# OATML-Markslab/ProteinGym

Measured on AMD Instinct MI355X. Metric: mutants scored/sec (ESM-1v 650M masked-marginal), higher is better.
Workload: dtype f16x3 (fp32 operands split into 2 fp16 planes, 3 fp16 MFMAs per product, fp32 accumulate)

## Files before the change

include/pgmi.h:

```cpp
#ifndef PGMI_H
#define PGMI_H

#include <stddef.h>
#include <stdint.h>

#ifdef __cplusplus
extern "C" {
#endif

#define PGMI_ABI_VERSION 4

#define PGMI_OK 0
#define PGMI_EINVAL (-1)
#define PGMI_ENOMEM (-2)
#define PGMI_EHIP (-3)
#define PGMI_ENODEV (-4)
#define PGMI_EPARSE (-5)
#define PGMI_EOVERFLOW (-6)

#define PGMI_ARCH_ESM1B 1
#define PGMI_ARCH_ESM2 2
#define PGMI_ARCH_TRANCEPTION 3
#define PGMI_ARCH_MSA 4
#define PGMI_ARCH_PROGEN2 5
#define PGMI_ARCH_GPT 6
#define PGMI_GPT_POS_ROTARY 0
#define PGMI_GPT_POS_LEARNED 1
#define PGMI_ARCH_ESMC 7

#define PGMI_PREC_FP32 0
#define PGMI_PREC_BF16 1
#define PGMI_PREC_F16X3 2

#define PGMI_TOK_CLS 0
#define PGMI_TOK_PAD 1
#define PGMI_TOK_EOS 2
#define PGMI_TOK_UNK 3
#define PGMI_TOK_MASK 32
#define PGMI_VOCAB 33
#define PGMI_PG2_VOCAB 32
#define PGMI_ESMC_VOCAB 64

typedef struct pgmi_config {
    int32_t abi_version;
    int32_t arch;
    int32_t layers;
    int32_t embed_dim;
    int32_t heads;
    int32_t ffn_dim;
    int32_t vocab;
    int32_t max_positions;
    int32_t token_dropout;
    int32_t emb_layer_norm_before;
    int32_t precision;
    int32_t max_rows;
    float ln_eps;
} pgmi_config;

typedef struct pgmi_model pgmi_model;
typedef struct pgmi_assay pgmi_assay;
typedef struct pgmi_pppl pgmi_pppl;

int pgmi_abi_version(void);
int pgmi_device_count(void);
const char* pgmi_last_error(void);

int64_t pgmi_weight_count(const pgmi_config* cfg);

int pgmi_model_create(const pgmi_config* cfg, const float* weights, int64_t n_weights,
                      int device, pgmi_model** out);
void pgmi_model_destroy(pgmi_model* m);
int pgmi_model_device(const pgmi_model* m);

int pgmi_token_logprobs(pgmi_model* m, const int32_t* tokens, int B, int T, float* out);

int pgmi_masked_logprobs(pgmi_model* m, const int32_t* tokens, const int32_t* mask_pos,
                         int B, int T, float* out);

int pgmi_assay_create(pgmi_model* m, const int32_t* wt_tokens, int n_tok,
                      const int32_t* positions, int P, int window,
                      const int32_t* sub_pos, const int32_t* sub_wt, const int32_t* sub_mt,
                      const int64_t* mut_off, int64_t n_mut, pgmi_assay** out);
int pgmi_assay_run(pgmi_model* m, pgmi_assay* a, double* scores_host, float* table_host,
                   double* scores_dev);
void pgmi_assay_destroy(pgmi_assay* a);

int pgmi_pppl_create(pgmi_model* m, const uint8_t* tokens, const int64_t* seq_off, int64_t n_seq, pgmi_pppl** out);
int pgmi_pppl_run(pgmi_model* m, pgmi_pppl* lib, int64_t first, int64_t count, double* scores_host,
                  float* terms_host, double* scores_dev);
int64_t pgmi_pppl_rows(const pgmi_pppl* lib, int64_t first, int64_t count);
int pgmi_pppl_stats(const pgmi_pppl* lib, int64_t* rows, int64_t* batches, int64_t* tokens, int64_t* padded_tokens);
void pgmi_pppl_destroy(pgmi_pppl* lib);

int pgmi_parse_mutants(const char* text, const int64_t* str_off, int64_t n_mut,
                       const char* sequence, int seq_len, int offset_idx,
                       int32_t* sub_pos, int32_t* sub_wt, int32_t* sub_mt,
                       int64_t* mut_off, int64_t* n_sub);

int pgmi_score_mutants(const float* table, int n_rows, int vocab, const int32_t* sub_pos, const int32_t* sub_wt,
                       const int32_t* sub_mt, const int64_t* mut_off, int64_t n_mut, double* scores);

void pgmi_optimal_window(int position, int seq_len_with_special, int model_window,
                         int* start, int* end);

#define PGMI_K_EMBED 0
#define PGMI_K_LAYERNORM 1
#define PGMI_K_GEMM_QKV 2
#define PGMI_K_ATTENTION 3
#define PGMI_K_GEMM_OUT 4
#define PGMI_K_GEMM_FC1 5
#define PGMI_K_GEMM_FC2 6
#define PGMI_K_HEAD 7
#define PGMI_K_SCORE 8
#define PGMI_K_KEPT_ROWS 9
#define PGMI_K_COUNT 10
int pgmi_profile_enable(pgmi_model* m, int on);
int pgmi_profile_get(pgmi_model* m, int kernel_class, double* ms, int64_t* launches,
                     double* flops, double* bytes);
int pgmi_profile_reset(pgmi_model* m);
int pgmi_synchronize(pgmi_model* m);

int pgmi_set_option(const char* name, int64_t value);

int pgmi_op_layernorm(int device, const float* x, const float* w, const float* b,
                      int rows, int D, float eps, float* y);
int pgmi_op_gemm(int device, int precision, const float* A, const float* W, const float* bias,
                 const float* residual, int M, int N, int K, int epilogue ,
                 float* C);
int pgmi_op_qkln_prep(int device, const float* qkv, const float* q_w, const float* k_w, int B, int T, int H, int iters, float* qk,
                      float* v, double* ms);
int pgmi_op_attention(int device, int precision, const float* qkv, const int32_t* kv_len,
                      int B, int T, int H, int rotary, float* ctx);
int pgmi_op_causal_attention(int device, int lanes, const float* X, const float* W, const float* bias, int K, const float* qkv,
                             const float* conv, const float* rot_cos, const float* rot_sin, const float* slopes, int B, int T,
                             int heads, float* ctx);

int pgmi_tr_token_logprobs(pgmi_model* m, const int32_t* tokens, int B, int T, float* out);
int pgmi_tr_sequence_loglik(pgmi_model* m, const int32_t* tokens, const int32_t* lens, int B, int T,
                            const float* log_prior, int P, const int32_t* prior_a0, const int32_t* prior_row0,
                            const int32_t* prior_n, const int32_t* prior_flip, float alpha, float* out);
int pgmi_tr_sequence_loglik_shared(pgmi_model* m, const int32_t* tokens, const int32_t* ref, int B, int T,
                                   const float* log_prior, int P, const int32_t* prior_a0, const int32_t* prior_row0,
                                   const int32_t* prior_n, const int32_t* prior_flip, float alpha, float* out,
                                   float* token_logprobs, int64_t* rows_forwarded);

int pgmi_bench_gemm(int device, int precision, int M, int N, int K, int epilogue, int split_out,
                    int variant, int iters, double* ms_per_launch);
int pgmi_bench_gemm_ab(int device, int precision, int M, int N, int K, int epilogue, int split_out,
                       const int* variants, int n_variants, int rounds, int iters, double* ms_out);

int pgmi_pg2_model_create(const pgmi_config* cfg, int rotary_dim, const float* weights, int64_t n_weights, int device, pgmi_model** out);
int pgmi_pg2_token_logprobs(pgmi_model* m, const int32_t* tokens, int B, int T, float* out);
int pgmi_pg2_sequence_loglik(pgmi_model* m, const int32_t* tokens, int B, int L, float* out, int32_t* n_kept);

int64_t pgmi_gpt_weight_count(const pgmi_config* cfg, int pos_kind);
int pgmi_gpt_model_create(const pgmi_config* cfg, int pos_kind, const float* weights, int64_t n_weights, int device, pgmi_model** out);
int pgmi_gpt_token_logprobs(pgmi_model* m, const int32_t* tokens, int B, int T, float* out);
int pgmi_gpt_sequence_loglik(pgmi_model* m, const int32_t* tokens, const int32_t* lens, int B, int T, double* sum, int32_t* n_targets);


int pgmi_msa_token_logprobs(pgmi_model* m, const int32_t* tokens, int R, int T, float* out);
int pgmi_msa_masked_logprobs(pgmi_model* m, const int32_t* tokens, int R, int T, int window,
                             const int32_t* positions, const int32_t* starts, int n, float* out);

int pgmi_msa_cluster_counts(int device, const int8_t* matrix, int64_t N, int64_t L, int invalid_value,
                            double identity_threshold, int32_t* counts_out, double* kernel_ms);

#ifdef __cplusplus
}
#endif
#endif
```

proteingym_amd/_lib.py:

```python
from __future__ import annotations

import ctypes as C
import os

import numpy as np

HERE = os.path.dirname(os.path.abspath(__file__))
LIB_PATH = os.path.join(HERE, "libpgmi.so")

ABI_VERSION = 4
ARCH_ESM1B, ARCH_ESM2, ARCH_TRANCEPTION = 1, 2, 3
ARCH_PROGEN2 = 5
ARCH_GPT = 6
ARCH_ESMC = 7
GPT_POS_ROTARY, GPT_POS_LEARNED = 0, 1
PREC_FP32, PREC_BF16, PREC_F16X3 = 0, 1, 2
PRECISIONS = {"fp32": PREC_FP32, "bf16": PREC_BF16, "f16x3": PREC_F16X3}
K_NAMES = ["embed", "layernorm", "gemm_qkv", "attention", "gemm_out", "gemm_fc1", "gemm_fc2",
           "head", "score", "kept_rows"]


EINVAL, ENOMEM, EHIP, ENODEV, EPARSE, EOVERFLOW = -1, -2, -3, -4, -5, -6


class PgmiError(RuntimeError):

    def __init__(self, message, code=None):
        super().__init__(message)
        self.code = code


class Config(C.Structure):
    _fields_ = [(n, C.c_int32) for n in (
        "abi_version", "arch", "layers", "embed_dim", "heads", "ffn_dim", "vocab",
        "max_positions", "token_dropout", "emb_layer_norm_before", "precision", "max_rows")] + [("ln_eps", C.c_float)]


_lib = None

_i32p = C.POINTER(C.c_int32)
_i64p = C.POINTER(C.c_int64)
_f32p = C.POINTER(C.c_float)
_f64p = C.POINTER(C.c_double)

SIGNATURES = [
    ("pgmi_abi_version", C.c_int, []),
    ("pgmi_device_count", C.c_int, []),
    ("pgmi_last_error", C.c_char_p, []),
    ("pgmi_weight_count", C.c_int64, [C.POINTER(Config)]),
    ("pgmi_model_create", C.c_int, [C.POINTER(Config), _f32p, C.c_int64, C.c_int, C.POINTER(C.c_void_p)]),
    ("pgmi_model_destroy", None, [C.c_void_p]),
    ("pgmi_model_device", C.c_int, [C.c_void_p]),
    ("pgmi_token_logprobs", C.c_int, [C.c_void_p, _i32p, C.c_int, C.c_int, _f32p]),
    ("pgmi_masked_logprobs", C.c_int, [C.c_void_p, _i32p, _i32p, C.c_int, C.c_int, _f32p]),
    ("pgmi_assay_create", C.c_int, [C.c_void_p, _i32p, C.c_int, _i32p, C.c_int, C.c_int,
                                    _i32p, _i32p, _i32p, _i64p, C.c_int64, C.POINTER(C.c_void_p)]),
    ("pgmi_assay_run", C.c_int, [C.c_void_p, C.c_void_p, _f64p, _f32p, C.c_void_p]),
    ("pgmi_assay_destroy", None, [C.c_void_p]),
    ("pgmi_pppl_create", C.c_int, [C.c_void_p, C.POINTER(C.c_uint8), _i64p, C.c_int64, C.POINTER(C.c_void_p)]),
    ("pgmi_pppl_run", C.c_int, [C.c_void_p, C.c_void_p, C.c_int64, C.c_int64, _f64p, _f32p, C.c_void_p]),
    ("pgmi_pppl_rows", C.c_int64, [C.c_void_p, C.c_int64, C.c_int64]),
    ("pgmi_pppl_stats", C.c_int, [C.c_void_p, _i64p, _i64p, _i64p, _i64p]),
    ("pgmi_pppl_destroy", None, [C.c_void_p]),
    ("pgmi_parse_mutants", C.c_int, [C.c_char_p, _i64p, C.c_int64, C.c_char_p, C.c_int, C.c_int,
                                     _i32p, _i32p, _i32p, _i64p, _i64p]),
    ("pgmi_score_mutants", C.c_int, [_f32p, C.c_int, C.c_int, _i32p, _i32p, _i32p, _i64p, C.c_int64, _f64p]),
    ("pgmi_optimal_window", None, [C.c_int, C.c_int, C.c_int, _i32p, _i32p]),
    ("pgmi_profile_enable", C.c_int, [C.c_void_p, C.c_int]),
    ("pgmi_profile_get", C.c_int, [C.c_void_p, C.c_int, _f64p, _i64p, _f64p, _f64p]),
    ("pgmi_profile_reset", C.c_int, [C.c_void_p]),
    ("pgmi_synchronize", C.c_int, [C.c_void_p]),
    ("pgmi_set_option", C.c_int, [C.c_char_p, C.c_int64]),
    ("pgmi_op_layernorm", C.c_int, [C.c_int, _f32p, _f32p, _f32p, C.c_int, C.c_int, C.c_float, _f32p]),
    ("pgmi_op_gemm", C.c_int, [C.c_int, C.c_int, _f32p, _f32p, _f32p, _f32p, C.c_int, C.c_int, C.c_int, C.c_int, _f32p]),
    ("pgmi_tr_token_logprobs", C.c_int, [C.c_void_p, _i32p, C.c_int, C.c_int, _f32p]),
    ("pgmi_tr_sequence_loglik", C.c_int, [C.c_void_p, _i32p, _i32p, C.c_int, C.c_int, _f32p, C.c_int,
                                          _i32p, _i32p, _i32p, _i32p, C.c_float, _f32p]),
    ("pgmi_tr_sequence_loglik_shared", C.c_int, [C.c_void_p, _i32p, _i32p, C.c_int, C.c_int, _f32p, C.c_int,
                                                 _i32p, _i32p, _i32p, _i32p, C.c_float, _f32p, _f32p, _i64p]),
    ("pgmi_pg2_model_create", C.c_int, [C.POINTER(Config), C.c_int, _f32p, C.c_int64, C.c_int, C.POINTER(C.c_void_p)]),
    ("pgmi_pg2_token_logprobs", C.c_int, [C.c_void_p, _i32p, C.c_int, C.c_int, _f32p]),
    ("pgmi_pg2_sequence_loglik", C.c_int, [C.c_void_p, _i32p, C.c_int, C.c_int, _f32p, _i32p]),
    ("pgmi_gpt_weight_count", C.c_int64, [C.POINTER(Config), C.c_int]),
    ("pgmi_gpt_model_create", C.c_int, [C.POINTER(Config), C.c_int, _f32p, C.c_int64, C.c_int, C.POINTER(C.c_void_p)]),
    ("pgmi_gpt_token_logprobs", C.c_int, [C.c_void_p, _i32p, C.c_int, C.c_int, _f32p]),
    ("pgmi_gpt_sequence_loglik", C.c_int, [C.c_void_p, _i32p, _i32p, C.c_int, C.c_int, _f64p, _i32p]),
    ("pgmi_bench_gemm", C.c_int, [C.c_int] * 9 + [_f64p]),
    ("pgmi_bench_gemm_ab", C.c_int, [C.c_int] * 7 + [_i32p, C.c_int, C.c_int, C.c_int, _f64p]),
    ("pgmi_op_attention", C.c_int, [C.c_int, C.c_int, _f32p, _i32p, C.c_int, C.c_int, C.c_int, C.c_int, _f32p]),
    ("pgmi_op_qkln_prep", C.c_int, [C.c_int, _f32p, _f32p, _f32p, C.c_int, C.c_int, C.c_int, C.c_int, _f32p, _f32p, _f64p]),
    ("pgmi_op_causal_attention", C.c_int, [C.c_int, C.c_int, _f32p, _f32p, _f32p, C.c_int, _f32p, _f32p, _f32p, _f32p, _f32p,
                                           C.c_int, C.c_int, C.c_int, _f32p]),
    ("pgmi_msa_token_logprobs", C.c_int, [C.c_void_p, _i32p, C.c_int, C.c_int, _f32p]),
    ("pgmi_msa_masked_logprobs", C.c_int, [C.c_void_p, _i32p, C.c_int, C.c_int, C.c_int, _i32p, _i32p, C.c_int, _f32p]),
    ("pgmi_msa_cluster_counts", C.c_int, [C.c_int, C.POINTER(C.c_int8), C.c_int64, C.c_int64, C.c_int, C.c_double, _i32p, _f64p]),
]


def load():
    global _lib
    if _lib is not None:
        return _lib
    if not os.path.exists(LIB_PATH):
        raise PgmiError(f"{LIB_PATH} not found: run `python -m proteingym_amd.build_native` "
                        "(hipcc, gfx950).  There is no CPU fallback.")
    lib = C.CDLL(LIB_PATH)
    for name, res, args in SIGNATURES:
        fn = getattr(lib, name)
        fn.restype = res
        fn.argtypes = args
    if lib.pgmi_abi_version() != ABI_VERSION:
        raise PgmiError("libpgmi ABI version mismatch; rebuild")
    _lib = lib
    return lib


def check(rc: int):
    if rc != 0:
        raise PgmiError(f"libpgmi error {rc}: {load().pgmi_last_error().decode(errors='replace')}", code=int(rc))


def ptr(a: np.ndarray, ty):
    return a.ctypes.data_as(ty) if a is not None else None


def as_i32(a):
    return np.ascontiguousarray(a, dtype=np.int32)


def as_f32(a):
    return np.ascontiguousarray(a, dtype=np.float32)


class ModelHandle:
    CREATE = "pgmi_model_create"

    def __init__(self, cfg: dict, weights: np.ndarray, device: int = 0, max_rows: int = 0, arch_arg=None,
                 precision: int = PREC_F16X3, **fields):
        lib = load()
        self.cfg = dict(cfg)
        self.device = device
        c = Config(abi_version=ABI_VERSION, layers=cfg["layers"], embed_dim=cfg["embed_dim"], heads=cfg["heads"],
                   ffn_dim=cfg["ffn_dim"], precision=precision, max_rows=max_rows, **fields)
        w = as_f32(weights)
        n = self._weight_count(lib, c, arch_arg)
        if w.size != n:
            raise PgmiError(f"weight blob has {w.size} elements, config needs {n}")
        h = C.c_void_p()
        head = (C.byref(c),) if arch_arg is None else (C.byref(c), arch_arg)
        check(getattr(lib, self.CREATE)(*head, ptr(w, _f32p), w.size, device, C.byref(h)))
        self._h = h

    @staticmethod
    def _weight_count(lib, c, arch_arg):
        return lib.pgmi_weight_count(C.byref(c))

    def close(self):
        if getattr(self, "_h", None):
            load().pgmi_model_destroy(self._h)
            self._h = None

    def __del__(self):
        try:
            self.close()
        except Exception:
            pass
```

proteingym_amd/csrc/api_esm.hip:

```cpp
#include "model.h"

namespace pgmi {

int create_esm(pgmi_model* m, const pgmi_config* cfg, const float* w, int64_t n_weights) {
    const size_t D = cfg->embed_dim, F = cfg->ffn_dim, V = cfg->vocab, dh = m->dh, Da = m->Da;
    BlobCursor c(m, w, n_weights);
    c.upload(&m->embed_tokens, V * D);
    if (cfg->arch == PGMI_ARCH_ESM1B) c.upload(&m->embed_positions, (size_t)(cfg->max_positions + 2) * D);
    if (cfg->emb_layer_norm_before) {
        c.upload(&m->lnb_w, D);
        c.upload(&m->lnb_b, D);
    }
    auto slot = [&](size_t col) -> size_t { return rotate_half_slot(col, dh); };
    const float qscale = 1.0f / sqrtf((float)dh);
    m->layers.resize(cfg->layers);
    std::vector<float> wq(3 * Da * D, 0.0f), bq(3 * Da, 0.0f), wo_r(D * Da, 0.0f);
    for (int l = 0; l < cfg->layers; ++l) {
        Layer& L = m->layers[l];
        c.upload(&L.ln1_w, D);
        c.upload(&L.ln1_b, D);
        pack_qkv_slots(c.take(3 * (D * D + D)), D, Da, slot, qscale, wq.data(), bq.data());
        c.linear(&L.wqkv, &L.wqkv16, wq.data(), wq.size(), D);
        c.upload(&L.bqkv, bq.data(), bq.size());
        pack_out_cols(c.take(D * D), D, Da, slot, wo_r.data());
        c.linear(&L.wo, &L.wo16, wo_r.data(), wo_r.size(), Da);
        c.upload(&L.bo, D);
        c.upload(&L.ln2_w, D);
        c.upload(&L.ln2_b, D);
        c.linear(&L.w1, &L.w116, F * D, D);
        c.upload(&L.b1, F);
        c.linear(&L.w2, &L.w216, D * F, F);
        c.upload(&L.b2, D);
    }
    c.upload(&m->lna_w, D);
    c.upload(&m->lna_b, D);
    c.linear(&m->hd_w, &m->hd16, D * D, D);
    c.upload(&m->hd_b, D);
    c.upload(&m->hln_w, D);
    c.upload(&m->hln_b, D);
    c.upload(&m->head_b, V);
    m->head_w = m->embed_tokens;
    return c.finish();
}

int ensure_rotary(pgmi_model* m, int T) {
    if ((m->cfg.arch != PGMI_ARCH_ESM2 && m->cfg.arch != PGMI_ARCH_ESMC) || T <= m->rot_len) return PGMI_OK;
    return upload_rotate_half(m, std::max(T, 1026));
}

int upload_rotate_half(pgmi_model* m, int n) {
    const int rh = m->rot_halves;
    float inv[64];
    const int half = m->dh / 2;
    for (int i = 0; i < half; ++i) inv[i] = 1.0f / powf(10000.0f, (float)(2 * i) / (float)m->dh);
    return upload_rotary(m, n, rh, [&](int t, int g, int i) {
        const int j = (rh == 1) ? i : 32 * g + i;
        return j < half ? (float)t * inv[j] : 0.0f;
    });
}

int run_encoder(pgmi_model* m, int B, int T, const int32_t* keep, int n_keep, bool* compacted) {
    const pgmi_config& c = m->cfg;
    const int M = B * T, D = c.embed_dim, F = c.ffn_dim, N1 = m->fc1_cols, H = c.heads, Da = m->Da;
    hipStream_t s = m->stream;
    if (c.arch == PGMI_ARCH_ESM1B && T > c.max_positions) {
        set_error("Sequence length %d above maximum sequence length of %d", T, c.max_positions);
        return PGMI_EINVAL;
    }
    int rc = ensure_rotary(m, T);
    if (!rc) rc = reset_pad_keys(m, B, T);
    if (rc) return rc;
    {
        ProfScope p(m, PGMI_K_EMBED, 0, (double)M * D * 4);
        launch_seq_stats(m->tokens, B, T, m->embed_gather ? 0 : c.token_dropout, m->denom, m->pos_idx, m->kv_len, s);
        if (m->embed_gather) launch_gather_rows(m->embed_tokens, m->tokens, M, D, m->x, s);
        else launch_embed(m->tokens, m->denom, m->pos_idx, m->embed_tokens, m->embed_positions, c.token_dropout, M, T, D, m->x, s);
        if (m->lnb_w) {
            launch_layernorm(m->x, m->lnb_w, m->lnb_b, M, D, 1e-5f, m->x, s);
            launch_zero_pad_rows(m->tokens, M, D, m->x, s);
        }
    }
    const double ln_bytes = 2.0 * M * D * 4;
    const int prec = c.precision;
    const int mode16 = (prec == PGMI_PREC_F16X3) ? 1 : 2;
    for (int l = 0; l < c.layers; ++l) {
        const Layer& L = m->layers[l];
        { ProfScope p(m, PGMI_K_LAYERNORM, 0, ln_bytes);
          if (prec == PGMI_PREC_FP32) launch_layernorm(m->x, L.ln1_w, L.ln1_b, M, D, 1e-5f, m->h, s);
          else launch_layernorm16(m->x, L.ln1_w, L.ln1_b, M, D, 1e-5f, m->h16, m->h16_plane, mode16, s); }
        const bool fused_qkv = prec != PGMI_PREC_FP32 && !L.q_ln;
        { ProfScope p(m, PGMI_K_GEMM_QKV, 2.0 * M * 3 * D * D, 0);
          if (fused_qkv)
              rc = launch_gemm16_qkv(m->h16, m->h16_plane, L.wqkv16.p, L.wqkv16.plane, L.bqkv, M, Da, D, L.wqkv16.out_scale,
                                     m->qk16, m->qk16_plane, m->vt16, m->vt16_plane, m->rot_cos, m->rot_sin,
                                     c.arch == PGMI_ARCH_ESM2, T, m->Hs, m->gemm_variant, s, m->rot_halves, prec == PGMI_PREC_BF16);
          else
              rc = linear(m, m->h, m->h16, m->h16_plane, L.wqkv, L.wqkv16, L.bqkv, nullptr, m->qkv, nullptr, 0, M, 3 * Da, D, EPI_NONE);
          if (rc) return rc; }
        { ProfScope p(m, PGMI_K_ATTENTION, 4.0 * M * T * D, L.q_ln ? (double)M * D * 20 : 0);
          if (L.q_ln && (rc = launch_qkln_prep(m->qkv, L.q_ln, L.k_ln, 1e-5f, m->rot_cos, m->rot_sin, B, T, H, m->qk16, m->qk16_plane,
                                               m->vt16, m->vt16_plane, s)))
              return rc;
          const bool v2 = prec != PGMI_PREC_FP32;
          if (c.arch == PGMI_ARCH_ESM2 && !v2) launch_rotary(m->qkv, m->rot_cos, m->rot_sin, M, T, m->Hs, s, m->rot_halves);
          if (v2) {
              AttLaunch a;
              a.qk16 = m->qk16, a.qk_plane = m->qk16_plane, a.vt16 = m->vt16, a.vt_plane = m->vt16_plane;
              a.B = B, a.T = T, a.H = H, a.head_dim = m->rot_halves * kHeadDim;
              a.kv_len = m->kv_len;
              a.out = prec == PGMI_PREC_F16X3 ? ATT_OUT_SPLIT : ATT_OUT_BF16;
              a.ctx16 = m->h16;
              a.stream = s;
              rc = launch_attention_f16x3_v2(a);
          } else {
              rc = launch_attention_f32(m->qkv, m->kv_len, B, T, H, m->h, s, m->rot_halves * kHeadDim);
          }
          if (rc) return rc; }
        if (keep && m->keep_rows && l == c.layers - 1) {
            const int R = n_keep;
            ProfScope p(m, PGMI_K_KEPT_ROWS, 2.0 * R * D * (Da + N1 + F), 0);
            launch_gather_rows(m->x, keep, R, D, m->qkv, s);
            if (prec == PGMI_PREC_FP32) launch_gather_rows(m->h, keep, R, Da, m->g, s);
            else
                launch_gather_rows(reinterpret_cast<const float*>(m->h16), keep, R, prec == PGMI_PREC_F16X3 ? Da : Da / 2,
                                   reinterpret_cast<float*>(m->g16), s);
            rc = linear(m, m->g, m->g16, m->g16_plane, L.wo, L.wo16, L.bo, m->qkv, m->x, nullptr, 0, R, D, Da, EPI_NONE);
            if (rc) return rc;
            if (prec == PGMI_PREC_FP32) launch_layernorm(m->x, L.ln2_w, L.ln2_b, R, D, 1e-5f, m->h, s);
            else launch_layernorm16(m->x, L.ln2_w, L.ln2_b, R, D, 1e-5f, m->h16, m->h16_plane, mode16, s);
            rc = linear(m, m->h, m->h16, m->h16_plane, L.w1, L.w116, L.b1, nullptr,
                        prec == PGMI_PREC_FP32 ? m->g : nullptr, prec == PGMI_PREC_FP32 ? nullptr : m->g16, m->g16_plane,
                        R, N1, D, m->fc1_epi);
            if (rc) return rc;
            rc = linear(m, m->g, m->g16, m->g16_plane, L.w2, L.w216, L.b2, m->x, m->x, nullptr, 0, R, D, F, EPI_NONE);
            if (rc) return rc;
            if (compacted) *compacted = true;
            break;
        }
        { ProfScope p(m, PGMI_K_GEMM_OUT, 2.0 * M * D * D, 0);
          rc = linear(m, m->h, m->h16, m->h16_plane, L.wo, L.wo16, L.bo, m->x, m->x, nullptr, 0, M, D, Da, EPI_NONE);
          if (rc) return rc; }
        { ProfScope p(m, PGMI_K_LAYERNORM, 0, ln_bytes);
          if (prec == PGMI_PREC_FP32) launch_layernorm(m->x, L.ln2_w, L.ln2_b, M, D, 1e-5f, m->h, s);
          else launch_layernorm16(m->x, L.ln2_w, L.ln2_b, M, D, 1e-5f, m->h16, m->h16_plane, mode16, s); }
        { ProfScope p(m, PGMI_K_GEMM_FC1, 2.0 * M * N1 * D, 0);
          rc = linear(m, m->h, m->h16, m->h16_plane, L.w1, L.w116, L.b1, nullptr,
                      prec == PGMI_PREC_FP32 ? m->g : nullptr, prec == PGMI_PREC_FP32 ? nullptr : m->g16, m->g16_plane,
                      M, N1, D, m->fc1_epi);
          if (rc) return rc; }
        { ProfScope p(m, PGMI_K_GEMM_FC2, 2.0 * M * F * D, 0);
          rc = linear(m, m->g, m->g16, m->g16_plane, L.w2, L.w216, L.b2, m->x, m->x, nullptr, 0, M, D, F, EPI_NONE);
          if (rc) return rc; }
    }
    PGMI_HIP(hipGetLastError());
    return PGMI_OK;
}

int run_head(pgmi_model* m, int R, const int32_t* row_idx) {
    const pgmi_config& c = m->cfg;
    const int D = c.embed_dim;
    hipStream_t s = m->stream;
    ProfScope p(m, PGMI_K_HEAD, 2.0 * R * D * (D + c.vocab), 0);
    const int prec = c.precision;
    const float* src = m->x;
    if (row_idx) {
        launch_gather_rows(m->x, row_idx, R, D, m->h, s);
        src = m->h;
    }
    if (prec == PGMI_PREC_FP32) launch_layernorm(src, m->lna_w, m->lna_b, R, D, 1e-5f, m->h, s);
    else launch_layernorm16(src, m->lna_w, m->lna_b, R, D, 1e-5f, m->h16, m->h16_plane, prec == PGMI_PREC_F16X3 ? 1 : 2, s);
    int rc = linear(m, m->h, m->h16, m->h16_plane, m->hd_w, m->hd16, m->hd_b, nullptr, m->g, nullptr, 0, R, D, D, EPI_GELU);
    if (rc) return rc;
    launch_layernorm(m->g, m->hln_w, m->hln_b, R, D, 1e-5f, m->g, s);
    launch_vocab_logsoftmax(m->g, m->head_w, m->head_b, R, D, c.vocab, m->lp, m->nonfinite, s);
    PGMI_HIP(hipGetLastError());
    return PGMI_OK;
}


int run_rows(pgmi_model* m, int B, int T, int R, const int32_t* row_idx) {
    bool compacted = false;
    int rc = run_encoder(m, B, T, row_idx, R, &compacted);
    if (rc) return rc;
    return run_head(m, R, compacted ? nullptr : row_idx);
}

}

extern "C" {

int pgmi_token_logprobs(pgmi_model* m, const int32_t* tokens, int B, int T, float* out) {
    if (!m || !tokens || !out || B <= 0 || T <= 0) { set_error("bad argument"); return PGMI_EINVAL; }
    if (T + 31 > m->max_rows) { set_error("T=%d exceeds workspace rows %d", T, m->max_rows); return PGMI_EINVAL; }
    int rc = check_tokens(tokens, B, T);
    if (rc) return rc;
    PGMI_HIP(hipSetDevice(m->device));
    const int V = m->cfg.vocab;
    rc = for_each_chunk(m, B, T, [&](int b0, int bc) {
        PGMI_HIP(hipMemcpyAsync(m->tokens, tokens + (size_t)b0 * T, (size_t)bc * T * 4, hipMemcpyHostToDevice, m->stream));
        int rc = run_rows(m, bc, T, bc * T, nullptr);
        if (rc) return rc;
        PGMI_HIP(hipMemcpyAsync(out + (size_t)b0 * T * V, m->lp, (size_t)bc * T * V * 4, hipMemcpyDeviceToHost, m->stream));
        return PGMI_OK;
    });
    return rc ? rc : check_nonfinite(m);
}

int pgmi_masked_logprobs(pgmi_model* m, const int32_t* tokens, const int32_t* mask_pos, int B, int T, float* out) {
    if (!m || !tokens || !mask_pos || !out || B <= 0 || T <= 0) { set_error("bad argument"); return PGMI_EINVAL; }
    if (m->cfg.arch == PGMI_ARCH_ESMC && T + 31 > m->max_rows) { set_error("T=%d exceeds workspace rows %d", T, m->max_rows); return PGMI_EINVAL; }
    if (T > m->max_rows) { set_error("T=%d exceeds workspace rows %d", T, m->max_rows); return PGMI_EINVAL; }
    int rc = check_tokens(tokens, B, T);
    if (rc) return rc;
    for (int b = 0; b < B; ++b)
        if (mask_pos[b] < 0 || mask_pos[b] >= T) { set_error("mask_pos[%d]=%d out of range", b, mask_pos[b]); return PGMI_EINVAL; }
    PGMI_HIP(hipSetDevice(m->device));
    const int V = m->cfg.vocab;
    std::vector<int32_t> ridx;
    rc = for_each_chunk(m, B, T, [&](int b0, int bc) {
        ridx.resize(bc);
        for (int b = 0; b < bc; ++b) ridx[b] = b * T + mask_pos[b0 + b];
        PGMI_HIP(hipMemcpyAsync(m->tokens, tokens + (size_t)b0 * T, (size_t)bc * T * 4, hipMemcpyHostToDevice, m->stream));
        PGMI_HIP(hipMemcpyAsync(m->aux_i, mask_pos + b0, (size_t)bc * 4, hipMemcpyHostToDevice, m->stream));
        PGMI_HIP(hipMemcpyAsync(m->row_idx, ridx.data(), (size_t)bc * 4, hipMemcpyHostToDevice, m->stream));
        launch_apply_mask(m->tokens, m->aux_i, bc, T, m->stream);
        int rc = run_rows(m, bc, T, bc, m->row_idx);
        if (rc) return rc;
        PGMI_HIP(hipMemcpyAsync(out + (size_t)b0 * V, m->lp, (size_t)bc * V * 4, hipMemcpyDeviceToHost, m->stream));
        return PGMI_OK;
    });
    return rc ? rc : check_nonfinite(m);
}

int pgmi_assay_create(pgmi_model* m, const int32_t* wt_tokens, int n_tok, const int32_t* positions, int P,
                      int window, const int32_t* sub_pos, const int32_t* sub_wt, const int32_t* sub_mt,
                      const int64_t* mut_off, int64_t n_mut, pgmi_assay** out) {
    if (!out) { set_error("null out"); return PGMI_EINVAL; }
    *out = nullptr;
    if (!m || !wt_tokens || n_tok <= 0 || P < 0 || (P > 0 && !positions) || window <= 0 || n_mut < 0) { set_error("bad argument"); return PGMI_EINVAL; }
    if (m->cfg.arch == PGMI_ARCH_ESMC) { set_error("ESM C assays run through pgmi_masked_logprobs (their window rule is not pgmi_optimal_window)"); return PGMI_EINVAL; }
    for (int i = 0; i < n_tok; ++i)
        if (wt_tokens[i] < 0 || wt_tokens[i] >= PGMI_VOCAB || wt_tokens[i] == PGMI_TOK_PAD) { set_error("wt token %d invalid at %d", wt_tokens[i], i); return PGMI_EINVAL; }
    const int T = std::min(n_tok, window);
    if (T > m->max_rows) { set_error("T=%d exceeds workspace rows %d", T, m->max_rows); return PGMI_EINVAL; }
    std::vector<int32_t> ws(P), mr(P);
    for (int i = 0; i < P; ++i) {
        if (positions[i] < 0 || positions[i] >= n_tok) { set_error("position %d out of range", positions[i]); return PGMI_EINVAL; }
        int s, e;
        pgmi_optimal_window(positions[i], n_tok, window, &s, &e);
        if (e - s != T) { set_error("internal: window length %d != %d", e - s, T); return PGMI_EINVAL; }
        ws[i] = s;
        mr[i] = positions[i] - s;
    }
    const int64_t n_sub = n_mut ? mut_off[n_mut] : 0;
    for (int64_t k = 0; k < n_sub; ++k)
        if (sub_pos[k] < 0 || sub_pos[k] >= n_tok || sub_wt[k] < 0 || sub_wt[k] >= PGMI_VOCAB || sub_mt[k] < 0 || sub_mt[k] >= PGMI_VOCAB) {
            set_error("substitution %lld out of range", (long long)k);
            return PGMI_EINVAL;
        }
    PGMI_HIP(hipSetDevice(m->device));
    pgmi_assay* a = new pgmi_assay();
    a->m = m; a->n_tok = n_tok; a->P = P; a->T = T; a->n_mut = n_mut; a->n_sub = n_sub;
    int rc = dev_upload(a->allocs, &a->wt, wt_tokens, (size_t)n_tok);
    if (!rc) rc = dev_upload(a->allocs, &a->positions, positions, (size_t)P);
    if (!rc) rc = dev_upload(a->allocs, &a->win_start, ws.data(), (size_t)P);
    if (!rc) rc = dev_upload(a->allocs, &a->mask_rel, mr.data(), (size_t)P);
    if (!rc) rc = dev_upload(a->allocs, &a->sub_pos, sub_pos, (size_t)n_sub);
    if (!rc) rc = dev_upload(a->allocs, &a->sub_wt, sub_wt, (size_t)n_sub);
    if (!rc) rc = dev_upload(a->allocs, &a->sub_mt, sub_mt, (size_t)n_sub);
    if (!rc) rc = dev_upload(a->allocs, &a->mut_off, mut_off, (size_t)(n_mut + 1));
    if (!rc) rc = dev_alloc(a->allocs, &a->table, (size_t)n_tok * PGMI_VOCAB);
    if (!rc) rc = dev_alloc(a->allocs, &a->scores, (size_t)n_mut);
    if (rc) { pgmi_assay_destroy(a); return rc; }
    m->assays.push_back(a);
    *out = a;
    return PGMI_OK;
}

void pgmi_assay_destroy(pgmi_assay* a) {
    if (!a) return;
    if (a->m) {
        hipSetDevice(a->m->device);
        hipStreamSynchronize(a->m->stream);
        auto& v = a->m->assays;
        v.erase(std::remove(v.begin(), v.end(), a), v.end());
    }
    for (void* p : a->allocs) hipFree(p);
    delete a;
}

int pgmi_assay_run(pgmi_model* m, pgmi_assay* a, double* scores_host, float* table_host, double* scores_dev) {
    if (!m || !a || a->m != m) { set_error("bad model/assay handle (assay belongs to another or a destroyed model)"); return PGMI_EINVAL; }
    PGMI_HIP(hipSetDevice(m->device));
    hipStream_t s = m->stream;
    const int T = a->T, V = m->cfg.vocab;
    const int per = rows_per_chunk(m, T);
    launch_fill_f32(a->table, (int64_t)a->n_tok * V, NAN, s);
    for (int p0 = 0; p0 < a->P; p0 += per) {
        const int bc = std::min(per, a->P - p0);
        launch_make_masked_windows(a->wt, a->win_start + p0, a->mask_rel + p0, bc, T, m->tokens, s);
        launch_row_index(a->mask_rel + p0, bc, T, m->row_idx, s);
        int rc = run_rows(m, bc, T, bc, m->row_idx);
        if (rc) return rc;
        launch_scatter_rows(m->lp, a->positions + p0, bc, V, a->table, s);
    }
    {
        ProfScope p(m, PGMI_K_SCORE, 0, (double)a->n_sub * 20);
        launch_score_mutants(a->table, V, a->sub_pos, a->sub_wt, a->sub_mt, a->mut_off, a->n_mut, a->scores, s);
    }
    PGMI_HIP(hipGetLastError());
    if (scores_dev && a->n_mut) PGMI_HIP(hipMemcpyAsync(scores_dev, a->scores, (size_t)a->n_mut * 8, hipMemcpyDeviceToDevice, s));
    if (scores_host && a->n_mut) PGMI_HIP(hipMemcpyAsync(scores_host, a->scores, (size_t)a->n_mut * 8, hipMemcpyDeviceToHost, s));
    if (table_host) PGMI_HIP(hipMemcpyAsync(table_host, a->table, (size_t)a->n_tok * V * 4, hipMemcpyDeviceToHost, s));
    PGMI_HIP(hipStreamSynchronize(s));
    return check_nonfinite(m);
}

int pgmi_pppl_create(pgmi_model* m, const uint8_t* tokens, const int64_t* seq_off, int64_t n_seq, pgmi_pppl** out) {
    if (!out) { set_error("null out"); return PGMI_EINVAL; }
    *out = nullptr;
    if (!m || !tokens || !seq_off || n_seq <= 0 || n_seq > 0x7fffffff) { set_error("bad argument"); return PGMI_EINVAL; }
    if (m->cfg.arch != PGMI_ARCH_ESM1B && m->cfg.arch != PGMI_ARCH_ESM2) { set_error("pseudo-ppl needs an ESM-1b/1v/ESM2 model"); return PGMI_EINVAL; }
    if (seq_off[0] != 0) { set_error("seq_off[0] must be 0"); return PGMI_EINVAL; }
    for (int64_t n = 0; n < n_seq; ++n) {
        const int64_t len = seq_off[n + 1] - seq_off[n];
        if (len < 2 || len > (1 << 24)) { set_error("sequence %lld has %lld tokens", (long long)n, (long long)len); return PGMI_EINVAL; }
        const uint8_t* t = tokens + seq_off[n];
        for (int64_t i = 0; i < len; ++i)
            if (t[i] >= PGMI_VOCAB || t[i] == PGMI_TOK_PAD) { set_error("token id %d invalid at sequence %lld, position %lld", (int)t[i], (long long)n, (long long)i); return PGMI_EINVAL; }
    }
    PGMI_HIP(hipSetDevice(m->device));
    pgmi_pppl* q = new pgmi_pppl();
    q->m = m;
    q->N = n_seq;
    q->off.assign(seq_off, seq_off + n_seq + 1);
    int rc = dev_upload(q->allocs, &q->tok8, tokens, (size_t)seq_off[n_seq]);
    if (!rc) rc = dev_upload(q->allocs, &q->off_dev, seq_off, (size_t)n_seq + 1);
    if (rc) { for (void* p : q->allocs) hipFree(p); delete q; return rc; }
    m->pppls.push_back(q);
    *out = q;
    return PGMI_OK;
}

void pgmi_pppl_destroy(pgmi_pppl* q) {
    if (!q) return;
    if (q->m) {
        hipSetDevice(q->m->device);
        hipStreamSynchronize(q->m->stream);
        auto& v = q->m->pppls;
        v.erase(std::remove(v.begin(), v.end(), q), v.end());
    }
    for (void* p : q->allocs) hipFree(p);
    delete q;
}

int64_t pgmi_pppl_rows(const pgmi_pppl* q, int64_t first, int64_t count) {
    if (!q || first < 0 || count < 0 || first + count > q->N) return -1;
    int64_t r = 0;
    for (int64_t n = first; n < first + count; ++n) r += std::max<int64_t>(0, q->off[n + 1] - q->off[n] - 4);
    return r;
}

int pgmi_pppl_run(pgmi_model* m, pgmi_pppl* q, int64_t first, int64_t count, double* scores_host, float* terms_host,
                  double* scores_dev) {
    if (!m || !q || q->m != m) { set_error("bad model/library handle (library belongs to another or a destroyed model)"); return PGMI_EINVAL; }
    if (first < 0 || count <= 0 || first + count > q->N) { set_error("sequence range [%lld, %lld) outside the library of %lld", (long long)first, (long long)(first + count), (long long)q->N); return PGMI_EINVAL; }
    PGMI_HIP(hipSetDevice(m->device));
    hipStream_t s = m->stream;
    const int J = (int)count, V = m->cfg.vocab;
    std::vector<int32_t> sid(J);
    for (int j = 0; j < J; ++j) sid[j] = (int32_t)(first + j);
    auto len_of = [&](int32_t n) { return q->off[n + 1] - q->off[n]; };
    std::stable_sort(sid.begin(), sid.end(), [&](int32_t a, int32_t b) { return len_of(a) > len_of(b); });
    std::vector<int64_t> rp((size_t)J + 1);
    rp[0] = 0;
    for (int j = 0; j < J; ++j) rp[j + 1] = rp[j] + std::max<int64_t>(0, len_of(sid[j]) - 4);
    const int64_t R = rp[J];
    const int64_t Tmax = len_of(sid[0]);
    if (R > 0 && Tmax + 31 > m->max_rows) { set_error("T=%lld exceeds workspace rows %d", (long long)Tmax, m->max_rows); return PGMI_EINVAL; }
    if (R > 0 && m->cfg.arch == PGMI_ARCH_ESM1B && Tmax > m->cfg.max_positions) {
        set_error("Sequence length %lld above maximum sequence length of %d", (long long)Tmax, m->cfg.max_positions);
        return PGMI_EINVAL;
    }
    std::vector<void*> pool;
    auto cleanup = [&]() { for (void* p : pool) hipFree(p); };
    int32_t* d_sid = nullptr;
    int64_t* d_rp = nullptr;
    float* d_terms = nullptr;
    double* d_out = nullptr;
    int rc = dev_upload(pool, &d_sid, sid.data(), (size_t)J);
    if (!rc) rc = dev_upload(pool, &d_rp, rp.data(), (size_t)J + 1);
    if (!rc) rc = dev_alloc(pool, &d_terms, (size_t)R);
    if (!rc) rc = dev_alloc(pool, &d_out, (size_t)J);
    if (rc) { cleanup(); return rc; }
    q->last_rows = R; q->last_chunks = 0; q->last_tokens = 0; q->last_padded = 0;
    int j0 = 0;
    for (int64_t g0 = 0; g0 < R;) {
        while (rp[j0 + 1] <= g0) ++j0;
        const int T = (int)len_of(sid[j0]);
        const int bc = (int)std::min<int64_t>(rows_per_chunk(m, T), R - g0);
        launch_make_pppl_rows(q->tok8, q->off_dev, d_sid, d_rp, J, g0, bc, T, m->tokens, m->row_idx, m->aux_i, s);
        rc = run_rows(m, bc, T, bc, m->row_idx);
        if (rc) { hipStreamSynchronize(s); cleanup(); return rc; }
        launch_pppl_pick(m->lp, m->aux_i, bc, V, d_terms + g0, s);
        q->last_chunks += 1;
        q->last_padded += (int64_t)bc * T;
        g0 += bc;
        if ((q->last_chunks & 63) == 0 && g0 < R && (rc = check_nonfinite(m)) != PGMI_OK) { cleanup(); return rc; }
    }
    for (int j = 0; j < J; ++j) q->last_tokens += (rp[j + 1] - rp[j]) * len_of(sid[j]);
    {
        ProfScope p(m, PGMI_K_SCORE, 0, (double)R * 4);
        launch_pppl_sum(d_terms, d_rp, d_sid, J, first, d_out, s);
    }
    hipError_t e = hipGetLastError();
    if (e == hipSuccess && scores_dev) e = hipMemcpyAsync(scores_dev, d_out, (size_t)J * 8, hipMemcpyDeviceToDevice, s);
    if (e == hipSuccess && scores_host) e = hipMemcpyAsync(scores_host, d_out, (size_t)J * 8, hipMemcpyDeviceToHost, s);
    std::vector<float> sorted_terms;
    if (e == hipSuccess && terms_host && R > 0) {
        sorted_terms.resize((size_t)R);
        e = hipMemcpyAsync(sorted_terms.data(), d_terms, (size_t)R * 4, hipMemcpyDeviceToHost, s);
    }
    if (e == hipSuccess) e = hipStreamSynchronize(s);
    cleanup();
    if (e != hipSuccess) { set_error("pseudo-ppl run failed: %s", hipGetErrorString(e)); return PGMI_EHIP; }
    if (terms_host && R > 0) {
        std::vector<int64_t> dst((size_t)J + 1, 0);
        for (int k = 0; k < J; ++k) dst[k + 1] = dst[k] + std::max<int64_t>(0, len_of((int32_t)(first + k)) - 4);
        for (int j = 0; j < J; ++j)
            std::copy(sorted_terms.begin() + rp[j], sorted_terms.begin() + rp[j + 1], terms_host + dst[sid[j] - first]);
    }
    return check_nonfinite(m);
}

int pgmi_pppl_stats(const pgmi_pppl* q, int64_t* rows, int64_t* chunks, int64_t* tokens, int64_t* padded_tokens) {
    if (!q) { set_error("null library"); return PGMI_EINVAL; }
    if (rows) *rows = q->last_rows;
    if (chunks) *chunks = q->last_chunks;
    if (tokens) *tokens = q->last_tokens;
    if (padded_tokens) *padded_tokens = q->last_padded;
    return PGMI_OK;
}

}
```

proteingym_amd/csrc/api_host.hip:

```cpp
#include "model.h"


extern "C" {

int pgmi_score_mutants(const float* table, int n_rows, int vocab, const int32_t* sub_pos, const int32_t* sub_wt, const int32_t* sub_mt,
                       const int64_t* mut_off, int64_t n_mut, double* scores) {
    if (!table || !mut_off || !scores || n_rows <= 0 || vocab <= 0 || n_mut < 0) { set_error("bad argument"); return PGMI_EINVAL; }
    const int64_t n_sub = mut_off[n_mut];
    if (n_sub > 0 && (!sub_pos || !sub_wt || !sub_mt)) { set_error("bad argument"); return PGMI_EINVAL; }
    for (int64_t k = 0; k < n_sub; ++k)
        if (sub_pos[k] < 0 || sub_pos[k] >= n_rows || sub_wt[k] < 0 || sub_wt[k] >= vocab || sub_mt[k] < 0 || sub_mt[k] >= vocab) {
            set_error("substitution %lld reads table[%d][%d / %d] of a [%d][%d] table", (long long)k, sub_pos[k], sub_wt[k], sub_mt[k], n_rows, vocab);
            return PGMI_EINVAL;
        }
    for (int64_t i = 0; i < n_mut; ++i) {
        double sc = 0.0;
        for (int64_t k = mut_off[i]; k < mut_off[i + 1]; ++k) {
            const float* rowp = table + (size_t)sub_pos[k] * vocab;
            const float d = rowp[sub_mt[k]] - rowp[sub_wt[k]];
            sc += (double)d;
        }
        scores[i] = sc;
    }
    return PGMI_OK;
}

void pgmi_optimal_window(int position, int n, int window, int* start, int* end) {
    const int half = window / 2;
    int s, e;
    if (n <= window) { s = 0; e = n; }
    else if (position < half) { s = 0; e = window; }
    else if (position >= n - half) { s = n - window; e = n; }
    else { s = std::max(0, position - half); e = std::min(n, position + half); }
    if (start) *start = s;
    if (end) *end = e;
}

int pgmi_parse_mutants(const char* text, const int64_t* str_off, int64_t n_mut, const char* sequence,
                       int seq_len, int offset_idx, int32_t* sub_pos, int32_t* sub_wt, int32_t* sub_mt,
                       int64_t* mut_off, int64_t* n_sub_out) {
    if (!text || !str_off || !sequence || n_mut < 0 || !n_sub_out) { set_error("bad argument"); return PGMI_EINVAL; }
    static const char* standard = "LAGVSERTIDPKQNFYMHWCXBUZO.-";
    int32_t idx[256];
    for (int i = 0; i < 256; ++i) idx[i] = PGMI_TOK_UNK;
    for (int i = 0; standard[i]; ++i) idx[(unsigned char)standard[i]] = 4 + i;
    const bool fill = sub_pos && sub_wt && sub_mt && mut_off;
    int64_t n = 0;
    for (int64_t i = 0; i < n_mut; ++i) {
        if (fill) mut_off[i] = n;
        const char* p = text + str_off[i];
        const char* end = text + str_off[i + 1];
        while (p < end) {
            const char* q = p;
            while (q < end && *q != ':') ++q;
            const int64_t len = q - p;
            if (len < 3) { set_error("malformed mutation '%.*s' in mutant %lld", (int)len, p, (long long)i); return PGMI_EPARSE; }
            const char wt = p[0], mt = q[-1];
            long pos = 0;
            bool neg = false;
            const char* d = p + 1;
            if (*d == '-') { neg = true; ++d; }
            if (d >= q - 1) { set_error("malformed mutation '%.*s' in mutant %lld", (int)len, p, (long long)i); return PGMI_EPARSE; }
            for (; d < q - 1; ++d) {
                if (*d < '0' || *d > '9') { set_error("malformed mutation '%.*s' in mutant %lld", (int)len, p, (long long)i); return PGMI_EPARSE; }
                pos = pos * 10 + (*d - '0');
                if (pos > 100000000) { set_error("position overflow in mutant %lld", (long long)i); return PGMI_EPARSE; }
            }
            if (neg) pos = -pos;
            const long k = pos - offset_idx;
            if (k < 0 || k >= seq_len) { set_error("mutation '%.*s': position %ld out of range for sequence of length %d", (int)len, p, pos, seq_len); return PGMI_EPARSE; }
            if (sequence[k] != wt) { set_error("The listed wildtype does not match the provided sequence ('%.*s': sequence has %c)", (int)len, p, sequence[k]); return PGMI_EPARSE; }
            if (fill) {
                sub_pos[n] = (int32_t)(1 + k);
                sub_wt[n] = idx[(unsigned char)wt];
                sub_mt[n] = idx[(unsigned char)mt];
            }
            ++n;
            p = (q < end) ? q + 1 : q;
            if (q < end && p == end) { set_error("trailing ':' in mutant %lld", (long long)i); return PGMI_EPARSE; }
        }
        if (str_off[i + 1] == str_off[i]) { set_error("empty mutant string at row %lld", (long long)i); return PGMI_EPARSE; }
    }
    if (fill) mut_off[n_mut] = n;
    *n_sub_out = n;
    return PGMI_OK;
}

}
```

proteingym_amd/csrc/api_model.hip:

```cpp
#include "model.h"

namespace pgmi {

static thread_local char g_err[1024] = "";
void set_error(const char* fmt, ...) {
    va_list ap;
    va_start(ap, fmt);
    vsnprintf(g_err, sizeof(g_err), fmt, ap);
    va_end(ap);
}

int prof_drain(pgmi_model* m) {
    if (m->events_used == 0) return PGMI_OK;
    PGMI_HIP(hipStreamSynchronize(m->stream));
    for (size_t i = 0; i < m->events_used; ++i) {
        float ms = 0.f;
        PGMI_HIP(hipEventElapsedTime(&ms, m->events[i].start, m->events[i].stop));
        m->prof_ms[m->events[i].cls] += ms;
    }
    m->events_used = 0;
    return PGMI_OK;
}

int check_cfg(const pgmi_config* c) {
    if (!c) { set_error("null config"); return PGMI_EINVAL; }
    if (c->abi_version != PGMI_ABI_VERSION) { set_error("ABI version mismatch: got %d, library is %d", c->abi_version, PGMI_ABI_VERSION); return PGMI_EINVAL; }
    if (c->arch != PGMI_ARCH_ESM1B && c->arch != PGMI_ARCH_ESM2 && c->arch != PGMI_ARCH_TRANCEPTION && c->arch != PGMI_ARCH_MSA &&
        c->arch != PGMI_ARCH_PROGEN2 && c->arch != PGMI_ARCH_GPT && c->arch != PGMI_ARCH_ESMC) { set_error("unknown arch %d", c->arch); return PGMI_EINVAL; }
    if (c->layers <= 0 || c->embed_dim <= 0 || c->heads <= 0 || c->ffn_dim <= 0) { set_error("non-positive model dimension"); return PGMI_EINVAL; }
    if (c->arch == PGMI_ARCH_ESMC) {
        if (c->precision != PGMI_PREC_F16X3) { set_error("ESM C is available in precision f16x3 only"); return PGMI_EINVAL; }
        if (c->embed_dim % 32 || c->embed_dim != c->heads * kHeadDim) { set_error("ESM C needs head_dim 64 and d %% 32 == 0 (embed_dim %d, heads %d)", c->embed_dim, c->heads); return PGMI_EINVAL; }
        if (c->embed_dim > 2048) { set_error("ESM C: embed_dim %d above the 2048 this build supports", c->embed_dim); return PGMI_EINVAL; }
        if (c->ffn_dim % 32) { set_error("ESM C: the SwiGLU hidden width %d must be a multiple of 32", c->ffn_dim); return PGMI_EINVAL; }
        if (c->vocab != PGMI_ESMC_VOCAB) { set_error("ESM C vocab must be %d", PGMI_ESMC_VOCAB); return PGMI_EINVAL; }
        return PGMI_OK;
    }
    {
        const int dh = c->embed_dim / c->heads;
        const bool pg2 = c->arch == PGMI_ARCH_PROGEN2;
        const bool esm_layout = c->arch == PGMI_ARCH_ESM1B || c->arch == PGMI_ARCH_ESM2 || c->arch == PGMI_ARCH_GPT;
        const bool ok = c->embed_dim % c->heads == 0 &&
                        (dh == kHeadDim || (dh < kHeadDim && dh % 2 == 0 && esm_layout) || (dh == 2 * kHeadDim && esm_layout) ||
                         (pg2 && dh % 2 == 0 && dh <= 4 * kHeadDim));
        if (pg2 && !ok && c->embed_dim % c->heads == 0 && dh > 4 * kHeadDim) {
            set_error("unsupported head_dim %d (embed_dim %d / heads %d): ProGen2 runs even head dims up to 256", dh, c->embed_dim, c->heads);
            return PGMI_EINVAL;
        }
        if (!ok) { set_error("unsupported head_dim %d (embed_dim %d / heads %d): this build supports head_dim 64, even head dims below 64 and head_dim 128 (ESM)", dh, c->embed_dim, c->heads); return PGMI_EINVAL; }
    }
    if (c->embed_dim % 32 || c->ffn_dim % 32) { set_error("embed_dim and ffn_dim must be multiples of 32"); return PGMI_EINVAL; }
    if (c->arch == PGMI_ARCH_TRANCEPTION) {
        if (c->vocab != 25) { set_error("Tranception vocab must be 25"); return PGMI_EINVAL; }
        if (c->heads % 4) { set_error("Invalid number of heads. Tranception requires the number of heads to be a multiple of 4."); return PGMI_EINVAL; }
        if (c->precision != PGMI_PREC_F16X3) { set_error("Tranception is available in precision f16x3 only"); return PGMI_EINVAL; }
        if (c->max_positions <= 0) { set_error("Tranception needs max_positions = n_ctx"); return PGMI_EINVAL; }
    } else if (c->arch == PGMI_ARCH_PROGEN2) {
        if (c->vocab != PGMI_PG2_VOCAB) { set_error("ProGen2 vocab must be %d", PGMI_PG2_VOCAB); return PGMI_EINVAL; }
        if (c->heads % 8) { set_error("ProGen2 needs the number of heads to be a multiple of 8 (mp_num = 8), got %d", c->heads); return PGMI_EINVAL; }
        if (c->precision != PGMI_PREC_F16X3) { set_error("ProGen2 is available in precision f16x3 only"); return PGMI_EINVAL; }
        if (c->max_positions <= 0) { set_error("ProGen2 needs max_positions = n_positions"); return PGMI_EINVAL; }
    } else if (c->arch == PGMI_ARCH_GPT) {
        if (c->vocab < 2) { set_error("causal decoder vocab must be at least 2, got %d", c->vocab); return PGMI_EINVAL; }
        if (c->precision != PGMI_PREC_F16X3) { set_error("the causal decoder (RITA / ProtGPT2) is available in precision f16x3 only"); return PGMI_EINVAL; }
        if (c->max_positions <= 0) { set_error("the causal decoder needs max_positions = n_positions / max_seq_len"); return PGMI_EINVAL; }
    } else if (c->vocab != PGMI_VOCAB) { set_error("vocab must be %d", PGMI_VOCAB); return PGMI_EINVAL; }
    if (c->arch == PGMI_ARCH_ESM1B && c->max_positions <= 0) { set_error("ESM-1b arch needs max_positions"); return PGMI_EINVAL; }
    if (c->arch == PGMI_ARCH_MSA) {
        if (c->max_positions <= 0) { set_error("MSA Transformer needs max_positions"); return PGMI_EINVAL; }
        if (c->embed_dim != c->heads * kHeadDim) { set_error("MSA Transformer: head_dim must be 64"); return PGMI_EINVAL; }
        if (c->precision != PGMI_PREC_F16X3) { set_error("MSA Transformer is available in precision f16x3 only"); return PGMI_EINVAL; }
    }
    if (c->precision != PGMI_PREC_FP32 && c->precision != PGMI_PREC_F16X3 && c->precision != PGMI_PREC_BF16) { set_error("unknown precision %d", c->precision); return PGMI_EINVAL; }
    if (c->precision == PGMI_PREC_BF16 && (c->embed_dim % 64 || c->ffn_dim % 64)) { set_error("precision bf16 needs embed_dim and ffn_dim to be multiples of 64"); return PGMI_EINVAL; }
    return PGMI_OK;
}

int check_tokens(const int32_t* tokens, int B, int T) {
    for (int b = 0; b < B; ++b) {
        const int32_t* t = tokens + (size_t)b * T;
        bool seen_pad = false;
        if (t[0] == PGMI_TOK_PAD) { set_error("sequence %d is empty (all <pad>)", b); return PGMI_EINVAL; }
        for (int i = 0; i < T; ++i) {
            if (t[i] < 0 || t[i] >= PGMI_VOCAB) { set_error("token id %d out of range at [%d,%d]", t[i], b, i); return PGMI_EINVAL; }
            if (t[i] == PGMI_TOK_PAD) seen_pad = true;
            else if (seen_pad) { set_error("interior <pad> at [%d,%d]: only trailing padding is supported", b, i); return PGMI_EINVAL; }
        }
    }
    return PGMI_OK;
}

int check_vocab(const int32_t* tokens, int B, int T, int V) {
    for (int b = 0; b < B; ++b)
        for (int t = 0; t < T; ++t) {
            const int tk = tokens[(size_t)b * T + t];
            if (tk < 0 || tk >= V) { set_error("token id %d out of range at [%d,%d]", tk, b, t); return PGMI_EINVAL; }
        }
    return PGMI_OK;
}

int env_int(const char* name, int dflt) {
    const char* v = getenv(name);
    return v ? atoi(v) : dflt;
}

int make_w16(std::vector<void*>& pool, const float* host, size_t n, size_t K, int precision, hipStream_t s, W16* out) {
    float mx = 0.f;
    for (size_t i = 0; i < n; ++i) mx = std::max(mx, fabsf(host[i]));
    float scale = 1.0f;
    const int planes = (precision == PGMI_PREC_F16X3) ? 2 : 1;
    if (precision == PGMI_PREC_F16X3 && mx > 0.f && std::isfinite(mx)) scale = exp2f(floorf(log2f(16384.0f / mx)));
    float* tmp = nullptr;
    hipError_t e = hipMalloc(reinterpret_cast<void**>(&tmp), n * sizeof(float));
    if (e != hipSuccess) { set_error("hipMalloc failed: %s", hipGetErrorString(e)); return PGMI_ENOMEM; }
    int rc = dev_alloc(pool, &out->p, n * planes);
    if (rc) { hipFree(tmp); return rc; }
    e = hipMemcpy(tmp, host, n * sizeof(float), hipMemcpyHostToDevice);
    if (e == hipSuccess) {
        launch_split16(tmp, (int64_t)n, scale, precision == PGMI_PREC_BF16 ? 1 : 0, (int)K, out->p, s);
        e = hipStreamSynchronize(s);
    }
    hipFree(tmp);
    if (e != hipSuccess) { set_error("weight split failed: %s", hipGetErrorString(e)); return PGMI_EHIP; }
    out->plane = n;
    out->out_scale = 1.0f / scale;
    return PGMI_OK;
}

int linear(pgmi_model* m, const float* in32, const unsigned short* in16, size_t in_plane, const float* W32,
           const W16& w16, const float* bias, const float* residual, float* out32, unsigned short* out16,
           size_t out_plane, int M, int N, int K, int epi) {
    if (m->cfg.precision == PGMI_PREC_FP32)
        return launch_gemm_f32(in32, W32, bias, residual, out32, M, N, K, epi, m->stream);
    const bool bf = m->cfg.precision == PGMI_PREC_BF16;
    return launch_gemm16(in16, in_plane, w16.p, w16.plane, bias, residual, out32, out16, out_plane, M, N, K, epi,
                         w16.out_scale, bf ? 1 : 2, bf, m->gemm_variant, m->stream);
}

int check_nonfinite(pgmi_model* m) {
    if (m->cfg.precision == PGMI_PREC_FP32) return PGMI_OK;
    int32_t flag = 0;
    PGMI_HIP(hipMemcpyAsync(&flag, m->nonfinite, 4, hipMemcpyDeviceToHost, m->stream));
    PGMI_HIP(hipStreamSynchronize(m->stream));
    if (flag) {
        PGMI_HIP(hipMemsetAsync(m->nonfinite, 0, 4, m->stream));
        set_error("non-finite log-probabilities: an activation left the fp16/bf16 range in precision mode %d; "
                  "re-run with precision fp32", m->cfg.precision);
        return PGMI_EOVERFLOW;
    }
    return PGMI_OK;
}

int reset_pad_keys(pgmi_model* m, int B, int T) {
    if (!m->vt16 || (B == m->last_B && T == m->last_T)) return PGMI_OK;
    PGMI_HIP(hipMemsetAsync(m->vt16, 0, m->vt16_plane * 2 * sizeof(unsigned short), m->stream));
    m->last_B = B;
    m->last_T = T;
    return PGMI_OK;
}

}

extern "C" {

int pgmi_abi_version(void) { return PGMI_ABI_VERSION; }

const char* pgmi_last_error(void) { return g_err; }

int pgmi_device_count(void) {
    int n = 0;
    if (hipGetDeviceCount(&n) != hipSuccess) return 0;
    return n;
}

int64_t pgmi_weight_count(const pgmi_config* c) {
    if (!c || c->layers <= 0 || c->embed_dim <= 0 || c->ffn_dim <= 0) return -1;
    const int64_t D = c->embed_dim, F = c->ffn_dim, V = c->vocab;
    if (c->arch == PGMI_ARCH_TRANCEPTION) {
        const int64_t conv = 3 * ((64 * 3 + 64) + (64 * 5 + 64) + (64 * 7 + 64));
        return V * D + (int64_t)c->layers * (2 * D + (D * 3 * D + 3 * D) + conv + (D * D + D) + 2 * D + (D * F + F) + (F * D + D)) + 2 * D + V * D;
    }
    if (c->arch == PGMI_ARCH_PROGEN2)
        return V * D + (int64_t)c->layers * (2 * D + 3 * D * D + D * D + (F * D + F) + (D * F + D)) + 2 * D + V * D + V;
    if (c->arch == PGMI_ARCH_GPT) return -1;
    if (c->arch == PGMI_ARCH_ESMC) return esmc_weight_count(c);
    if (c->arch == PGMI_ARCH_MSA) {
        const int64_t attn = 2 * D + 4 * (D * D + D);
        return V * D + (int64_t)(c->max_positions + 2) * D + 1024 * D + 2 * D +
               (int64_t)c->layers * (2 * attn + 2 * D + (F * D + F) + (D * F + D)) + 2 * D + (D * D + D) + 2 * D + V;
    }
    int64_t n = V * D;
    if (c->arch == PGMI_ARCH_ESM1B) n += (int64_t)(c->max_positions + 2) * D;
    if (c->emb_layer_norm_before) n += 2 * D;
    n += (int64_t)c->layers * (2 * D + 4 * (D * D + D) + 2 * D + (F * D + F) + (D * F + D));
    n += 2 * D + (D * D + D) + 2 * D + V;
    return n;
}

int pgmi_model_create(const pgmi_config* cfg, const float* w, int64_t n_weights, int device, pgmi_model** out) {
    if (cfg && cfg->arch == PGMI_ARCH_PROGEN2) {
        if (out) *out = nullptr;
        set_error("ProGen2 models are created with pgmi_pg2_model_create (it takes rotary_dim)");
        return PGMI_EINVAL;
    }
    if (cfg && cfg->arch == PGMI_ARCH_GPT) {
        if (out) *out = nullptr;
        set_error("causal decoder models are created with pgmi_gpt_model_create (it takes pos_kind)");
        return PGMI_EINVAL;
    }
    return model_create(cfg, w, n_weights, device, out, 0);
}

}

namespace pgmi {

static int alloc_workspace(pgmi_model* m) {
    const pgmi_config& c = m->cfg;
    const size_t R = m->max_rows, D = c.embed_dim, F = c.ffn_dim, V = c.vocab, Da = m->Da;
    const size_t Dw = std::max(D, Da);
    const bool f32mode = c.precision == PGMI_PREC_FP32;
    int rc = PGMI_OK;
    auto alloc = [&](auto** p, size_t n) { if (!rc) rc = dev_alloc(m->allocs, p, n); };
    alloc(&m->x, R * D);
    alloc(&m->h, R * Dw);
    alloc(&m->qkv, R * 3 * Da);
    alloc(&m->g, R * (f32mode ? std::max(F, D) : D));
    if (!f32mode) {
        const size_t planes = c.precision == PGMI_PREC_F16X3 ? 2 : 1;
        m->h16_plane = R * Dw;
        m->g16_plane = R * F;
        alloc(&m->h16, m->h16_plane * planes);
        alloc(&m->g16, m->g16_plane * planes);
    }
    alloc(&m->nonfinite, (size_t)1);
    if (!f32mode) {
        m->qk16_plane = R * 2 * Da;
        m->vt16_plane = R * Da;
        alloc(&m->qk16, m->qk16_plane * 2);
        alloc(&m->vt16, m->vt16_plane * 2);
    }
    if (c.arch == PGMI_ARCH_MSA) {
        alloc(&m->xt, R * D);
        alloc(&m->msa_kv_len, (size_t)2048);
    }
    alloc(&m->lp, (c.arch == PGMI_ARCH_GPT && V > kWave ? (size_t)m->gpt_head_rows : R) * V);
    alloc(&m->denom, R);
    alloc(&m->tokens, R);
    alloc(&m->pos_idx, R);
    alloc(&m->kv_len, R);
    alloc(&m->row_idx, R);
    alloc(&m->aux_i, R);
    if (rc) return rc;
    PGMI_HIP(hipMemset(m->nonfinite, 0, 4));
    if (m->vt16) PGMI_HIP(hipMemset(m->vt16, 0, m->vt16_plane * 2 * sizeof(unsigned short)));
    return PGMI_OK;
}

int model_create(const pgmi_config* cfg, const float* w, int64_t n_weights, int device, pgmi_model** out, int arch_arg) {
    if (!out) { set_error("null out"); return PGMI_EINVAL; }
    *out = nullptr;
    int rc = check_cfg(cfg);
    if (rc) return rc;
    const int64_t need = cfg->arch == PGMI_ARCH_GPT ? gpt_weight_count(cfg, arch_arg) : pgmi_weight_count(cfg);
    if (need < 0) { set_error("causal decoder pos_kind %d: must be PGMI_GPT_POS_ROTARY or PGMI_GPT_POS_LEARNED", arch_arg); return PGMI_EINVAL; }
    if (!w || n_weights != need) {
        set_error("weight blob has %lld elements, config needs %lld", (long long)n_weights, (long long)need);
        return PGMI_EINVAL;
    }
    const int ndev = pgmi_device_count();
    if (ndev <= 0) { set_error("no HIP device visible (libpgmi has no CPU fallback)"); return PGMI_ENODEV; }
    if (device < 0 || device >= ndev) { set_error("device %d out of range (%d visible)", device, ndev); return PGMI_EINVAL; }
    PGMI_HIP(hipSetDevice(device));
    pgmi_model* m = new pgmi_model();
    m->cfg = *cfg;
    m->device = device;
    if (hipStreamCreateWithFlags(&m->stream, hipStreamNonBlocking) != hipSuccess) { set_error("hipStreamCreate failed"); delete m; return PGMI_EHIP; }
    m->dh = cfg->embed_dim / cfg->heads;
    m->rot_halves = m->dh > 2 * kHeadDim ? 4 : m->dh > kHeadDim ? 2 : 1;
    m->Hs = cfg->heads * m->rot_halves;
    m->Da = m->Hs * kHeadDim;
    m->ln_eps = cfg->ln_eps > 0.f ? cfg->ln_eps : 1e-5f;
    m->max_rows = std::max(cfg->max_rows > 0 ? cfg->max_rows : 98304, 2048);
    const size_t V = cfg->vocab;
    const std::vector<float> zeros(std::max({3 * (size_t)m->Da, (V + 63) / 64 * 64, (size_t)cfg->embed_dim, V, (size_t)cfg->heads}), 0.0f);
    rc = dev_upload(m->allocs, &m->zeros, zeros.data(), zeros.size());
    m->fc1_cols = cfg->ffn_dim;
    if (!rc) switch (cfg->arch) {
        case PGMI_ARCH_TRANCEPTION: rc = create_tranception(m, cfg, w, n_weights); break;
        case PGMI_ARCH_MSA: rc = create_msa(m, cfg, w, n_weights); break;
        case PGMI_ARCH_PROGEN2: rc = create_progen2(m, cfg, w, n_weights, arch_arg); break;
        case PGMI_ARCH_GPT: rc = create_gpt(m, cfg, w, n_weights, arch_arg); break;
        case PGMI_ARCH_ESMC: rc = create_esmc(m, cfg, w, n_weights); break;
        default: rc = create_esm(m, cfg, w, n_weights);
    }
    if (!rc) rc = alloc_workspace(m);
    if (rc) { pgmi_model_destroy(m); return rc; }
    m->keep_rows = env_int("PGMI_KEEP_ROWS", 1);
    gemm_options_from_env();
    m->gemm_variant = env_int("PGMI_GEMM_VARIANT", 0);
    *out = m;
    return PGMI_OK;
}

}

extern "C" {

void pgmi_model_destroy(pgmi_model* m) {
    if (!m) return;
    hipSetDevice(m->device);
    if (m->stream) hipStreamSynchronize(m->stream);
    for (pgmi_assay* a : m->assays) {
        for (void* p : a->allocs) hipFree(p);
        a->allocs.clear();
        a->m = nullptr;
    }
    m->assays.clear();
    for (pgmi_pppl* q : m->pppls) {
        for (void* p : q->allocs) hipFree(p);
        q->allocs.clear();
        q->m = nullptr;
    }
    m->pppls.clear();
    for (auto& e : m->events) { hipEventDestroy(e.start); hipEventDestroy(e.stop); }
    for (void* p : m->allocs) hipFree(p);
    if (m->stream) hipStreamDestroy(m->stream);
    delete m;
}

int pgmi_model_device(const pgmi_model* m) { return m ? m->device : -1; }

int pgmi_set_option(const char* name, int64_t value) {
    if (!name) { set_error("null option name"); return PGMI_EINVAL; }
    int rc = gemm_set_option(name, (long long)value);
    if (rc) rc = att_set_option(name, (long long)value);
    if (rc) set_error("unknown option '%s' (gemm_half_tail, gemm_max_rows, att_xcd_local, att_v3)", name);
    return rc;
}

int pgmi_synchronize(pgmi_model* m) {
    if (!m) { set_error("null model"); return PGMI_EINVAL; }
    PGMI_HIP(hipStreamSynchronize(m->stream));
    return PGMI_OK;
}

int pgmi_profile_enable(pgmi_model* m, int on) {
    if (!m) { set_error("null model"); return PGMI_EINVAL; }
    int rc = prof_drain(m);
    m->prof = on != 0;
    return rc;
}

int pgmi_profile_reset(pgmi_model* m) {
    if (!m) { set_error("null model"); return PGMI_EINVAL; }
    int rc = prof_drain(m);
    for (int i = 0; i < PGMI_K_COUNT; ++i) { m->prof_ms[i] = 0; m->prof_n[i] = 0; m->prof_flops[i] = 0; m->prof_bytes[i] = 0; }
    return rc;
}

int pgmi_profile_get(pgmi_model* m, int k, double* ms, int64_t* launches, double* flops, double* bytes) {
    if (!m || k < 0 || k >= PGMI_K_COUNT) { set_error("bad argument"); return PGMI_EINVAL; }
    int rc = prof_drain(m);
    if (rc) return rc;
    if (ms) *ms = m->prof_ms[k];
    if (launches) *launches = m->prof_n[k];
    if (flops) *flops = m->prof_flops[k];
    if (bytes) *bytes = m->prof_bytes[k];
    return PGMI_OK;
}

}
```

proteingym_amd/csrc/api_ops.hip:

```cpp
#include "model.h"

static inline float rebuild_split(unsigned short h, unsigned short l) {
    _Float16 a, b;
    memcpy(&a, &h, 2); memcpy(&b, &l, 2);
    return (float)a + (float)b * (1.0f / kLoScale);
}

extern "C" {

int pgmi_op_layernorm(int device, const float* x, const float* w, const float* b, int rows, int D, float eps, float* y) {
    if (!x || !w || !b || !y || rows <= 0 || D <= 0 || D % 4) { set_error("bad argument"); return PGMI_EINVAL; }
    if (pgmi_device_count() <= 0) { set_error("no HIP device visible"); return PGMI_ENODEV; }
    PGMI_HIP(hipSetDevice(device));
    std::vector<void*> pool;
    float *dx, *dw, *db, *dy;
    int rc = 0;
    if ((rc = dev_upload(pool, &dx, x, (size_t)rows * D)) || (rc = dev_upload(pool, &dw, w, (size_t)D)) ||
        (rc = dev_upload(pool, &db, b, (size_t)D)) || (rc = dev_alloc(pool, &dy, (size_t)rows * D))) {
        for (void* p : pool) hipFree(p);
        return rc;
    }
    launch_layernorm(dx, dw, db, rows, D, eps, dy, nullptr);
    hipError_t e = hipMemcpy(y, dy, (size_t)rows * D * 4, hipMemcpyDeviceToHost);
    for (void* p : pool) hipFree(p);
    if (e != hipSuccess) { set_error("layernorm op failed: %s", hipGetErrorString(e)); return PGMI_EHIP; }
    return PGMI_OK;
}

int pgmi_op_gemm(int device, int precision, const float* A, const float* W, const float* bias, const float* residual,
                 int M, int N, int K, int epilogue, float* C) {
    if (!A || !W || !C || M <= 0 || N <= 0 || K <= 0) { set_error("bad argument"); return PGMI_EINVAL; }
    if (precision != PGMI_PREC_FP32 && precision != PGMI_PREC_F16X3 && precision != PGMI_PREC_BF16) { set_error("unknown precision %d", precision); return PGMI_EINVAL; }
    if (pgmi_device_count() <= 0) { set_error("no HIP device visible"); return PGMI_ENODEV; }
    PGMI_HIP(hipSetDevice(device));
    gemm_options_from_env();
    std::vector<void*> pool;
    float *dA, *dW = nullptr, *dB = nullptr, *dR = nullptr, *dC;
    int rc = 0;
    if ((rc = dev_upload(pool, &dA, A, (size_t)M * K)) ||
        (precision == PGMI_PREC_FP32 && (rc = dev_upload(pool, &dW, W, (size_t)N * K))) ||
        (bias && (rc = dev_upload(pool, &dB, bias, (size_t)N))) ||
        (residual && (rc = dev_upload(pool, &dR, residual, (size_t)M * N))) ||
        (rc = dev_alloc(pool, &dC, (size_t)M * N))) {
        for (void* p : pool) hipFree(p);
        return rc;
    }
    const int epi = epilogue & 255;
    const bool split_planes = (epilogue & 256) != 0;
    if (epi == EPI_SWIGLU && (!split_planes || precision != PGMI_PREC_F16X3 || (N % 64))) {
        for (void* p : pool) hipFree(p);
        set_error("SwiGLU GEMM op: precision f16x3 with the split-plane output (epilogue 4 + 256), N %% 64 == 0");
        return PGMI_EINVAL;
    }
    if (split_planes && (precision == PGMI_PREC_FP32 || residual || (N % (precision == PGMI_PREC_F16X3 ? 32 : 4)))) {
        for (void* p : pool) hipFree(p);
        set_error("16-bit-plane GEMM op: f16x3 (N %% 32 == 0) or bf16 (N %% 4 == 0), no residual");
        return PGMI_EINVAL;
    }
    if (precision == PGMI_PREC_FP32) {
        rc = launch_gemm_f32(dA, dW, dB, dR, dC, M, N, K, epi, nullptr);
    } else {
        const bool bf = precision == PGMI_PREC_BF16;
        const int planes = bf ? 1 : 2;
        W16 w16;
        unsigned short* a16 = nullptr;
        rc = make_w16(pool, W, (size_t)N * K, (size_t)K, precision, nullptr, &w16);
        if (!rc) rc = dev_alloc(pool, &a16, (size_t)M * K * planes);
        if (!rc) {
            launch_split16(dA, (int64_t)M * K, 1.0f, bf ? 1 : 2, K, a16, nullptr);
            if (split_planes) {
                unsigned short* c16 = nullptr;
                const int No = epi == EPI_SWIGLU ? N / 2 : N;
                rc = dev_alloc(pool, &c16, (size_t)M * N * 2);
                if (!rc) rc = launch_gemm16(a16, (size_t)M * K, w16.p, w16.plane, dB, nullptr, nullptr, c16, (size_t)M * No, M, N, K, epi,
                                            w16.out_scale, planes, bf, env_int("PGMI_GEMM_VARIANT", 0), nullptr);
                if (!rc) {
                    std::vector<unsigned short> h((size_t)M * N * 2);
                    hipError_t e2 = hipMemcpy(h.data(), c16, h.size() * 2, hipMemcpyDeviceToHost);
                    if (e2 != hipSuccess) { set_error("gemm op failed: %s", hipGetErrorString(e2)); rc = PGMI_EHIP; }
                    for (size_t m = 0; m < (size_t)M && !rc && bf; ++m)
                        for (int n = 0; n < N; ++n) {
                            const unsigned int u = (unsigned int)h[m * N + n] << 16;
                            memcpy(&C[m * N + n], &u, 4);
                        }
                    for (size_t m = 0; m < (size_t)M && !rc && !bf; ++m)
                        for (int n = 0; n < No; ++n) {
                            const size_t o = ki_off(m, n, No);
                            C[m * No + n] = rebuild_split(h[o], h[o + 32]);
                        }
                }
                for (void* p : pool) hipFree(p);
                return rc;
            }
            rc = launch_gemm16(a16, (size_t)M * K, w16.p, w16.plane, dB, dR, dC, nullptr, 0, M, N, K, epi,
                               w16.out_scale, planes, bf, env_int("PGMI_GEMM_VARIANT", 0), nullptr);
        }
    }
    hipError_t e = hipMemcpy(C, dC, (size_t)M * N * 4, hipMemcpyDeviceToHost);
    for (void* p : pool) hipFree(p);
    if (rc) return rc;
    if (e != hipSuccess) { set_error("gemm op failed: %s", hipGetErrorString(e)); return PGMI_EHIP; }
    return PGMI_OK;
}

int pgmi_bench_gemm_ab(int device, int precision, int M, int N, int K, int epilogue, int split_out, const int* variants,
                       int n_variants, int rounds, int iters, double* ms_out) {
    if (M <= 0 || N <= 0 || K <= 0 || iters <= 0 || rounds <= 0 || n_variants <= 0 || !variants || !ms_out) { set_error("bad argument"); return PGMI_EINVAL; }
    if (pgmi_device_count() <= 0) { set_error("no HIP device visible"); return PGMI_ENODEV; }
    PGMI_HIP(hipSetDevice(device));
    gemm_options_from_env();
    std::vector<void*> pool;
    auto cleanup = [&]() { for (void* p : pool) hipFree(p); };
    std::vector<float> hA((size_t)M * K), hW((size_t)N * K), hb(N);
    unsigned int st = 12345u;
    auto rnd = [&]() { st = st * 1664525u + 1013904223u; return ((st >> 8) * (1.0f / 8388608.0f)) - 1.0f; };
    for (auto& v : hA) v = rnd();
    for (auto& v : hW) v = rnd() * 0.03f;
    for (auto& v : hb) v = rnd();
    float *dA, *dW = nullptr, *dB, *dC = nullptr;
    unsigned short *a16 = nullptr, *c16 = nullptr;
    int rc = 0;
    if ((rc = dev_upload(pool, &dA, hA.data(), hA.size())) || (rc = dev_upload(pool, &dB, hb.data(), hb.size()))) { cleanup(); return rc; }
    hipEvent_t e0, e1;
    PGMI_HIP(hipEventCreate(&e0));
    PGMI_HIP(hipEventCreate(&e1));
    const bool f32 = precision == PGMI_PREC_FP32;
    const bool bf = precision == PGMI_PREC_BF16;
    const int planes = bf ? 1 : 2;
    W16 w16;
    if (f32) {
        if ((rc = dev_upload(pool, &dW, hW.data(), hW.size())) || (rc = dev_alloc(pool, &dC, (size_t)M * N))) { cleanup(); return rc; }
    } else {
        if ((rc = make_w16(pool, hW.data(), hW.size(), (size_t)K, precision, nullptr, &w16)) ||
            (rc = dev_alloc(pool, &a16, (size_t)M * K * planes))) { cleanup(); return rc; }
        launch_split16(dA, (int64_t)M * K, 1.0f, bf ? 1 : 2, K, a16, nullptr);
        if (split_out == 1) rc = dev_alloc(pool, &c16, (size_t)M * N * planes);
        else if (split_out != 3) rc = dev_alloc(pool, &dC, (size_t)M * N);
        if (rc) { cleanup(); return rc; }
    }
    const bool fused_qkv = split_out == 3 && !f32 && !bf;
    const int Tq = (M % 288 == 0) ? 288 : M;
    unsigned short *qk16 = nullptr, *vt16 = nullptr;
    size_t qk_plane = 0, vt_plane = 0;
    if (fused_qkv) {
        if (N % 3 || (N / 3) % 64) { set_error("fused QKV bench needs N = 3 D, D %% 64 == 0"); cleanup(); return PGMI_EINVAL; }
        const size_t Tp = (size_t)(Tq + 31) / 32 * 32;
        qk_plane = (size_t)M * 2 * (N / 3);
        vt_plane = (size_t)(M / Tq) * (N / 3) * Tp;
        if ((rc = dev_alloc(pool, &qk16, qk_plane * 2)) || (rc = dev_alloc(pool, &vt16, vt_plane * 2))) { cleanup(); return rc; }
    }
    auto run = [&](int var) -> int {
        if (f32) return launch_gemm_f32(dA, dW, dB, split_out == 2 ? dC : nullptr, dC, M, N, K, epilogue, nullptr);
        if (fused_qkv)
            return launch_gemm16_qkv(a16, (size_t)M * K, w16.p, w16.plane, dB, M, N / 3, K, w16.out_scale, qk16, qk_plane, vt16, vt_plane,
                                     nullptr, nullptr, 0, Tq, N / 3 / kHeadDim, var, nullptr);
        const bool planes_out = split_out == 1;
        return launch_gemm16(a16, (size_t)M * K, w16.p, w16.plane, dB, split_out == 2 ? dC : nullptr, planes_out ? nullptr : dC,
                             planes_out ? c16 : nullptr, (size_t)M * N, M, N, K, epilogue, w16.out_scale, planes, bf, var, nullptr);
    };
    std::vector<std::vector<double>> samples(n_variants);
    for (int v = 0; v < n_variants && !rc; ++v) rc = run(variants[v] >= 0 ? variants[v] : env_int("PGMI_GEMM_VARIANT", 0));
    for (int r = 0; r < rounds && !rc; ++r)
        for (int v = 0; v < n_variants && !rc; ++v) {
            const int var = variants[v] >= 0 ? variants[v] : env_int("PGMI_GEMM_VARIANT", 0);
            hipEventRecord(e0, nullptr);
            for (int i = 0; i < iters && !rc; ++i) rc = run(var);
            hipEventRecord(e1, nullptr);
            hipError_t e = hipEventSynchronize(e1);
            float ms = 0.f;
            if (e == hipSuccess) e = hipEventElapsedTime(&ms, e0, e1);
            if (e != hipSuccess) { set_error("bench failed: %s", hipGetErrorString(e)); rc = PGMI_EHIP; }
            samples[v].push_back(ms / iters);
        }
    if (!rc)
        for (int v = 0; v < n_variants; ++v) {
            std::sort(samples[v].begin(), samples[v].end());
            ms_out[v] = samples[v][samples[v].size() / 2];
        }
    hipEventDestroy(e0);
    hipEventDestroy(e1);
    cleanup();
    return rc;
}

int pgmi_bench_gemm(int device, int precision, int M, int N, int K, int epilogue, int split_out, int variant,
                    int iters, double* ms_per_launch) {
    return pgmi_bench_gemm_ab(device, precision, M, N, K, epilogue, split_out, &variant, 1, 1, iters, ms_per_launch);
}

int pgmi_op_qkln_prep(int device, const float* qkv, const float* q_w, const float* k_w, int B, int T, int H, int iters, float* qk,
                      float* v, double* ms) {
    if (!qkv || !q_w || !k_w || B <= 0 || T <= 0 || H <= 0 || H * kHeadDim > 2048 || iters < 0 || (iters > 0 && !ms)) { set_error("bad argument"); return PGMI_EINVAL; }
    if (pgmi_device_count() <= 0) { set_error("no HIP device visible"); return PGMI_ENODEV; }
    PGMI_HIP(hipSetDevice(device));
    const size_t D = (size_t)H * kHeadDim, M = (size_t)B * T, Tp = (size_t)(T + 31) / 32 * 32;
    std::vector<void*> pool;
    auto cleanup = [&]() { for (void* p : pool) hipFree(p); };
    float *dq = nullptr, *dqw = nullptr, *dkw = nullptr;
    unsigned short *qk16 = nullptr, *vt16 = nullptr;
    int rc = 0;
    if ((rc = dev_upload(pool, &dq, qkv, M * 3 * D)) || (rc = dev_upload(pool, &dqw, q_w, D)) || (rc = dev_upload(pool, &dkw, k_w, D)) ||
        (rc = dev_alloc(pool, &qk16, M * 2 * D * 2)) || (rc = dev_alloc(pool, &vt16, (size_t)B * Tp * D * 2))) {
        cleanup();
        return rc;
    }
    pgmi_model tmp;
    rc = upload_rotate_half(&tmp, T);
    auto launch = [&]() {
        return launch_qkln_prep(dq, dqw, dkw, 1e-5f, tmp.rot_cos, tmp.rot_sin, B, T, H, qk16, M * 2 * D, vt16, (size_t)B * Tp * D, nullptr);
    };
    if (!rc) rc = launch();
    if (!rc && iters > 0) {
        hipEvent_t e0, e1;
        PGMI_HIP(hipEventCreate(&e0));
        PGMI_HIP(hipEventCreate(&e1));
        hipEventRecord(e0, nullptr);
        for (int i = 0; i < iters && !rc; ++i) rc = launch();
        hipEventRecord(e1, nullptr);
        hipEventSynchronize(e1);
        float t = 0.f;
        hipEventElapsedTime(&t, e0, e1);
        *ms = (double)t / iters;
        hipEventDestroy(e0);
        hipEventDestroy(e1);
    }
    hipDeviceSynchronize();
    std::vector<unsigned short> hq(qk ? M * 2 * D * 2 : 0), hv(v ? (size_t)B * Tp * D * 2 : 0);
    hipError_t e = hipSuccess;
    if (!rc && qk) e = hipMemcpy(hq.data(), qk16, hq.size() * 2, hipMemcpyDeviceToHost);
    if (!rc && v && e == hipSuccess) e = hipMemcpy(hv.data(), vt16, hv.size() * 2, hipMemcpyDeviceToHost);
    for (void* p : tmp.allocs) hipFree(p);
    cleanup();
    if (rc) return rc;
    if (e != hipSuccess) { set_error("qkln prep op failed: %s", hipGetErrorString(e)); return PGMI_EHIP; }
    if (qk)
        for (size_t i = 0; i < M * 2 * D; ++i) qk[i] = rebuild_split(hq[i], hq[M * 2 * D + i]);
    if (v) {
        const size_t vp = (size_t)B * Tp * D;
        for (int b = 0; b < B; ++b)
            for (int t = 0; t < T; ++t) {
                const int tk = t & 31, pos = (t & ~31) + ((tk & 0x13) | ((tk & 4) << 1) | ((tk & 8) >> 1));
                for (size_t c = 0; c < D; ++c) {
                    const size_t o = ((size_t)b * H * kHeadDim + c) * Tp + pos;
                    v[((size_t)b * T + t) * D + c] = rebuild_split(hv[o], hv[vp + o]);
                }
            }
    }
    return PGMI_OK;
}

int pgmi_op_attention(int device, int precision, const float* qkv, const int32_t* kv_len, int B, int T, int H,
                      int rotary, float* ctx) {
    if (!qkv || !ctx || B <= 0 || T <= 0 || H <= 0) { set_error("bad argument"); return PGMI_EINVAL; }
    if (pgmi_device_count() <= 0) { set_error("no HIP device visible"); return PGMI_ENODEV; }
    PGMI_HIP(hipSetDevice(device));
    std::vector<void*> pool;
    float *dq, *dc;
    int32_t* dl = nullptr;
    const size_t D = (size_t)H * kHeadDim;
    int rc = 0;
    if ((rc = dev_upload(pool, &dq, qkv, (size_t)B * T * 3 * D)) || (kv_len && (rc = dev_upload(pool, &dl, kv_len, (size_t)B))) ||
        (rc = dev_alloc(pool, &dc, (size_t)B * T * D))) {
        for (void* p : pool) hipFree(p);
        return rc;
    }
    pgmi_model tmp;
    tmp.cfg.arch = PGMI_ARCH_ESM2;
    if (rotary) rc = ensure_rotary(&tmp, T);
    if (!rc && precision == PGMI_PREC_F16X3) {
        const size_t Tp = (size_t)(T + 31) / 32 * 32;
        unsigned short *qk = nullptr, *vt = nullptr;
        rc = dev_alloc(pool, &qk, (size_t)B * T * 2 * D * 2);
        if (!rc) rc = dev_alloc(pool, &vt, (size_t)B * Tp * D * 2);
        AttLaunch a;
        a.qk16 = qk, a.qk_plane = (size_t)B * T * 2 * D, a.vt16 = vt, a.vt_plane = (size_t)B * Tp * D;
        a.B = B, a.T = T, a.H = H;
        a.kv_len = dl;
        a.out = ATT_OUT_F32, a.ctx = dc;
        a.qkv = dq, a.cos_t = tmp.rot_cos, a.sin_t = tmp.rot_sin, a.rotary = rotary;
        if (!rc) rc = launch_attention_f16x3_v2(a);
    } else if (!rc) {
        if (rotary) launch_rotary(dq, tmp.rot_cos, tmp.rot_sin, B * T, T, H, nullptr);
        rc = launch_attention_f32(dq, dl, B, T, H, dc, nullptr);
    }
    hipDeviceSynchronize();
    for (void* p : tmp.allocs) hipFree(p);
    hipError_t e = hipMemcpy(ctx, dc, (size_t)B * T * D * 4, hipMemcpyDeviceToHost);
    for (void* p : pool) hipFree(p);
    if (rc) return rc;
    if (e != hipSuccess) { set_error("attention op failed: %s", hipGetErrorString(e)); return PGMI_EHIP; }
    return PGMI_OK;
}

int pgmi_op_causal_attention(int device, int lanes, const float* X, const float* W, const float* bias, int K, const float* qkv,
                             const float* conv, const float* rot_cos, const float* rot_sin, const float* slopes, int B, int T,
                             int heads, float* ctx) {
    const bool fused = X && W && bias && !qkv && !conv, conv_form = qkv && conv && !X && !W && !bias && !rot_cos && !rot_sin;
    if ((!fused && !conv_form) || !slopes || !ctx || B <= 0 || T <= 0 || heads <= 0 || lanes <= 0 || !rot_cos != !rot_sin) { set_error("bad argument"); return PGMI_EINVAL; }
    if (fused && (K <= 0 || K % 32)) { set_error("causal attention op: K = %d is not a positive multiple of 32", K); return PGMI_EINVAL; }
    if (pgmi_device_count() <= 0) { set_error("no HIP device visible"); return PGMI_ENODEV; }
    PGMI_HIP(hipSetDevice(device));
    gemm_options_from_env();
    const size_t M = (size_t)B * T, Da = (size_t)heads * lanes, Tp = (size_t)(T + 31) / 32 * 32, Hs = Da / kHeadDim;
    const int halves = lanes / kHeadDim, rotary = rot_cos != nullptr;
    const size_t qk_plane = M * 2 * Da, vt_plane = (size_t)B * Tp * Da;
    std::vector<void*> pool;
    auto cleanup = [&]() { for (void* p : pool) hipFree(p); };
    float *dx = nullptr, *db = nullptr, *dq = nullptr, *dconv = nullptr, *dcos = nullptr, *dsin = nullptr, *dsl = nullptr;
    unsigned short *a16 = nullptr, *qk16 = nullptr, *vt16 = nullptr, *c16 = nullptr;
    int rc = 0;
    if ((rc = dev_upload(pool, &dsl, slopes, (size_t)heads)) || (rc = dev_alloc(pool, &qk16, qk_plane * 2)) ||
        (rc = dev_alloc(pool, &vt16, vt_plane * 2)) || (rc = dev_alloc(pool, &c16, M * Da * 2)) ||
        (fused && ((rc = dev_upload(pool, &dx, X, M * K)) || (rc = dev_upload(pool, &db, bias, 3 * Da)) || (rc = dev_alloc(pool, &a16, M * K * 2)))) ||
        (rotary && ((rc = dev_upload(pool, &dcos, rot_cos, (size_t)T * std::max(halves, 1) * kHeadDim)) ||
                    (rc = dev_upload(pool, &dsin, rot_sin, (size_t)T * std::max(halves, 1) * kHeadDim)))) ||
        (conv_form && ((rc = dev_upload(pool, &dq, qkv, M * 3 * Da)) || (rc = dev_upload(pool, &dconv, conv, (size_t)3 * 4 * kHeadDim * 8))))) {
        cleanup();
        return rc;
    }
    hipError_t e = hipMemset(vt16, 0, vt_plane * 2 * sizeof(unsigned short));
    if (e != hipSuccess) { cleanup(); set_error("causal attention op failed: %s", hipGetErrorString(e)); return PGMI_EHIP; }
    if (fused) {
        W16 w16;
        rc = make_w16(pool, W, 3 * Da * K, (size_t)K, PGMI_PREC_F16X3, nullptr, &w16);
        if (!rc) {
            launch_split16(dx, (int64_t)(M * K), 1.0f, 2, K, a16, nullptr);
            rc = launch_gemm16_qkv(a16, M * K, w16.p, w16.plane, db, (int)M, (int)Da, K, w16.out_scale, qk16, qk_plane, vt16, vt_plane,
                                   dcos, dsin, rotary, T, (int)Hs, env_int("PGMI_GEMM_VARIANT", 0), nullptr, halves, false);
        }
    }
    AttLaunch a;
    a.qk16 = qk16, a.qk_plane = qk_plane, a.vt16 = vt16, a.vt_plane = vt_plane;
    a.B = B, a.T = T, a.H = heads, a.head_dim = lanes;
    a.slopes = dsl;
    a.out = ATT_OUT_SPLIT, a.ctx16 = c16;
    a.qkv = dq, a.conv = dconv;
    if (!rc) rc = launch_attention_f16x3_v2(a);
    std::vector<unsigned short> h(rc ? 0 : M * Da * 2);
    e = hipDeviceSynchronize();
    if (!rc && e == hipSuccess) e = hipMemcpy(h.data(), c16, h.size() * 2, hipMemcpyDeviceToHost);
    cleanup();
    if (rc) return rc;
    if (e != hipSuccess) { set_error("causal attention op failed: %s", hipGetErrorString(e)); return PGMI_EHIP; }
    for (size_t m = 0; m < M; ++m)
        for (size_t n = 0; n < Da; ++n) {
            const size_t o = ki_off(m, (int)n, (int)Da);
            ctx[m * Da + n] = rebuild_split(h[o], h[o + 32]);
        }
    return PGMI_OK;
}

}
```

proteingym_amd/csrc/attention_f16.hip:

```cpp
#include <stdlib.h>
#include <string.h>
#include <algorithm>

#include "attention_f16_common.h"

namespace pgmi {

template <int WPB, int OUT, int NSTG, int DH = 64, bool RAG = false, int DO = DH>
__global__ __launch_bounds__(WPB * 64) void attention_f16x3_v2_kernel(
    const unsigned short* __restrict__ qk16, size_t qk_plane, const unsigned short* __restrict__ vt16,
    size_t vt_plane, const int32_t* __restrict__ kv_len, const float* __restrict__ slopes, int T, int H,
    int Tp, float* __restrict__ ctx, unsigned short* __restrict__ ctx16, RagMap rag, int dense_nblk, int nseq) {
    constexpr float defer_thr = kAttDefer;
    constexpr int NT = WPB * 64;
    constexpr int KCPR = DH / 8;
    constexpr int KCH = AKT * KCPR, VCH = DO * 4;
    constexpr int NSL = DH / DO;
    static_assert(NSL == 1 || (OUT == ATT_OUT_SPLIT && !RAG), "sliced context: split-plane output of dense launches only");
    constexpr int STG_CH = 2 * KCH + 2 * VCH;
    constexpr int NWI = STG_CH / 64;
    static_assert(NWI % WPB == 0, "the wave-instructions of a stage divide evenly over the waves");
    constexpr int NDMA = NWI / WPB;
    constexpr int NS = DH / 16, ND = DO / 32;
    extern __shared__ __attribute__((aligned(16))) u32x4 lds[];

    int b, h, qblk_dense, hs;
    if (RAG) {
        b = rag.ent_seq[blockIdx.x];
        hs = blockIdx.y;
        qblk_dense = 0;
    } else if (dense_nblk > 0) {
        const int pair = xcd_local_pair(dense_nblk, qblk_dense);
        if (pair >= nseq * H * NSL) return;
        b = pair / (H * NSL);
        hs = pair - b * (H * NSL);
    } else {
        b = blockIdx.z;
        hs = blockIdx.y;
        qblk_dense = blockIdx.x;
    }
    h = hs / NSL;
    const int d0 = (hs - h * NSL) * DO;
    const int tid = threadIdx.x, lane = tid & 63;
    const int wave = __builtin_amdgcn_readfirstlane(tid >> 6);
    const int r = lane & 31, kh = lane >> 5;
    const int D = H * DH;
    const int Tk = (!RAG && kv_len) ? kv_len[b] : T;
    const int p0 = RAG ? rag.seq_p[b] : 0, a0 = p0 & ~(AKT - 1), kt0 = a0 / AKT;
    const int qblk = RAG ? rag.ent_j[blockIdx.x] : qblk_dense;
    const int row0 = RAG ? rag.seq_q[b] : b * T, rrow0 = RAG ? rag.seq_q[rag.seq_root[b]] : 0;
    const int orow0 = RAG ? rag.seq_off[b] - p0 : b * T;
    const int Tpo = RAG ? (T - a0 + 31) / 32 * 32 : Tp;
    const int q0 = a0 + (qblk * WPB + wave) * 32;
    const bool active = q0 < T;

    constexpr bool q_lds = NSTG >= 3;
    u32x4 qh[NS], ql[NS];
    if (!q_lds) {
        const int qrow = min(q0 + r, T - 1);
        const unsigned short* qp = qk16 + ((size_t)row0 + (qrow - a0)) * (2 * D) + h * DH + kh * 8;
#pragma unroll
        for (int s = 0; s < NS; ++s) {
            qh[s] = *reinterpret_cast<const u32x4*>(qp + s * 16);
            ql[s] = *reinterpret_cast<const u32x4*>(qp + qk_plane + s * 16);
        }
    }

    const size_t seq_halfs = (size_t)T * (2 * D), vt_halfs = (size_t)DH * Tp;
    const unsigned long long qk_bytes = std::min<unsigned long long>(0xFFFFFFFFull, (unsigned long long)qk_plane * 2ull + seq_halfs * 2ull);
    const unsigned long long vt_bytes = std::min<unsigned long long>(0xFFFFFFFFull, (unsigned long long)vt_plane * 2ull + vt_halfs * 2ull);
    const __amdgpu_buffer_rsrc_t rsQK = operand_rsrc(qk16 + (size_t)row0 * (2 * D), qk_bytes);
    const __amdgpu_buffer_rsrc_t rsVT = operand_rsrc(vt16 + (RAG ? (size_t)rag.seq_vt[b] + (size_t)h * DH * Tpo : ((size_t)b * H + h) * vt_halfs), vt_bytes);
    const __amdgpu_buffer_rsrc_t rsQKr = operand_rsrc(qk16 + (size_t)rrow0 * (2 * D), qk_bytes);
    const __amdgpu_buffer_rsrc_t rsVTr = operand_rsrc(vt16 + (RAG ? (size_t)rag.seq_vt[rag.seq_root[b]] + (size_t)h * DH * Tp : (size_t)0), vt_bytes);
    const bool causal = slopes != nullptr;
    const int last_q = min(T, a0 + (qblk * WPB + WPB) * 32);
    const int nkt = causal ? (min(Tk, last_q) + AKT - 1) / AKT : (Tk + AKT - 1) / AKT;
    int voff[NDMA], voff_last[NDMA], voff_root[NDMA], sbase[NDMA], sstep[NDMA], slot0[NDMA];
    bool is_k[NDMA];
#pragma unroll
    for (int i = 0; i < NDMA; ++i) {
        int wi = wave + WPB * i;
        if (wi >= NWI) wi -= NWI;
        slot0[i] = wi * 64;
        is_k[i] = wi < 2 * KCH / 64;
        if (is_k[i]) {
            const int p = wi / (KCH / 64), key = ((wi % (KCH / 64)) * 64 + lane) / KCPR;
            const int c = (lane % KCPR) ^ k_swizzle<DH>(key);
            voff[i] = voff_root[i] = key * (2 * D) * 2 + c * 16;
            voff_last[i] = min(key, T - 1 - (nkt - 1) * AKT) * (2 * D) * 2 + c * 16;
            sbase[i] = (int)((unsigned int)p * (unsigned int)qk_plane * 2u + (unsigned int)(D + h * DH) * 2u);
            sstep[i] = AKT * (2 * D) * 2;
        } else {
            const int wv = wi - 2 * KCH / 64, p = wv / (VCH / 64), g = (wv % (VCH / 64)) * 64 + lane;
            const int d = g >> 2, c = (g & 3) ^ ((d >> 2) & 3);
            voff[i] = voff_last[i] = (d0 + d) * Tpo * 2 + c * 16;
            voff_root[i] = (d0 + d) * Tp * 2 + c * 16;
            sbase[i] = (int)((unsigned int)p * (unsigned int)vt_plane * 2u);
            sstep[i] = (AKT / 8) * 16;
        }
    }
    auto issue_tile = [&](int kt, int buf) {
        u32x4* base = lds + buf * STG_CH;
        const bool from_root = RAG && kt < kt0;
#pragma unroll
        for (int i = 0; i < NDMA; ++i) {
            const int vo = from_root ? voff_root[i] : ((kt == nkt - 1) ? voff_last[i] : voff[i]);
            const int so = sbase[i] + (from_root ? kt : kt - kt0) * sstep[i];
            if (is_k[i]) __builtin_amdgcn_raw_ptr_buffer_load_lds(from_root ? rsQKr : rsQK, (__attribute__((address_space(3))) void*)(base + slot0[i]), 16, vo, so, 0, 0);
            else __builtin_amdgcn_raw_ptr_buffer_load_lds(from_root ? rsVTr : rsVT, (__attribute__((address_space(3))) void*)(base + slot0[i]), 16, vo, so, 0, 0);
        }
    };

    constexpr float kLog2e = 1.4426950408889634f;
    const float slope2 = causal ? slopes[h] * kLog2e : 0.0f;
    if (q_lds) {
        issue_tile(0, 0);
        u32x4* qbase = lds + STG_CH + wave * (2 * KCH);
        if (active) {
            constexpr int NQ = 2 * KCH / 64;
#pragma unroll
            for (int i = 0; i < NQ; ++i) {
                const int f = i * 64 + lane, pq = f / KCH, row = (f % KCH) / KCPR;
                const int c = (f % KCPR) ^ k_swizzle<DH>(row);
                const int vo = (int)(((unsigned int)(min(q0 + row, T - 1) - a0) * (unsigned int)(2 * D) + (unsigned int)(h * DH)) * 2u + (unsigned int)c * 16u);
                const int so = (int)((unsigned int)pq * (unsigned int)qk_plane * 2u);
                __builtin_amdgcn_raw_ptr_buffer_load_lds(rsQK, (__attribute__((address_space(3))) void*)(qbase + i * 64), 16, vo, so, 0, 0);
            }
        }
        asm volatile("s_waitcnt vmcnt(0)" ::: "memory");
        if (active) {
#pragma unroll
            for (int s = 0; s < NS; ++s) {
                const int ci = r * KCPR + ((2 * s + kh) ^ k_swizzle<DH>(r));
                qh[s] = qbase[ci];
                ql[s] = qbase[KCH + ci];
            }
        }
        asm volatile("s_waitcnt lgkmcnt(0)" ::: "memory");
        __builtin_amdgcn_s_barrier();
        asm volatile("" ::: "memory");
#pragma unroll
        for (int t = 1; t < NSTG - 1; ++t)
            if (t < nkt) issue_tile(t, t);
    } else {
#pragma unroll
        for (int t = 0; t < NSTG - 1; ++t)
            if (t < nkt) issue_tile(t, t);
    }

    f32x16 om[ND], oc[ND];
#pragma unroll
    for (int dt = 0; dt < ND; ++dt)
#pragma unroll
        for (int v = 0; v < 16; ++v) { om[dt][v] = 0.f; oc[dt][v] = 0.f; }
    float m_run = -INFINITY, l_run = 0.f;
    constexpr float kInvLo = 1.0f / kLoScale;

    const f32x16 zero16 = {0.f, 0.f, 0.f, 0.f, 0.f, 0.f, 0.f, 0.f, 0.f, 0.f, 0.f, 0.f, 0.f, 0.f, 0.f, 0.f};
    auto wanted = [&](int kt) -> bool { return active && !(causal && kt * AKT > q0 + 31); };
    auto scores = [&](int buf, f32x16& sm, f32x16& sc) {
        const u32x4* Kb = lds + buf * STG_CH;
#pragma unroll
        for (int s = 0; s < NS; ++s) {
            const int ci = r * KCPR + ((2 * s + kh) ^ k_swizzle<DH>(r));
            const u32x4 kfh = Kb[ci], kfl = Kb[KCH + ci];
            sc = mfma_h(kfh, ql[s], s == 0 ? zero16 : sc);
            sc = mfma_h(kfl, qh[s], sc);
            sm = mfma_h(kfh, qh[s], s == 0 ? zero16 : sm);
        }
    };
    auto wait_tile = [&](int younger) {
        if (younger >= 2) asm volatile("s_waitcnt vmcnt(%0)" ::"n"(2 * NDMA) : "memory");
        else if (younger == 1) asm volatile("s_waitcnt vmcnt(%0)" ::"n"(NDMA) : "memory");
        else asm volatile("s_waitcnt vmcnt(0)" ::: "memory");
    };
    int cur = 0;
    for (int kt = 0; kt < nkt; ++kt) {
        wait_tile(min(NSTG - 2, nkt - 1 - kt));
        __builtin_amdgcn_s_barrier();
        asm volatile("" ::: "memory");
        if (kt + NSTG - 1 < nkt) issue_tile(kt + NSTG - 1, (cur == 0) ? NSTG - 1 : cur - 1);
        if (wanted(kt)) {
            const u32x4* Vb = lds + cur * STG_CH + 2 * KCH;
            f32x16 sm, sc;
            scores(cur, sm, sc);
            float st[16];
            if (causal) {
                const float kb = (float)(kt * AKT + 4 * kh);
#pragma unroll
                for (int v = 0; v < 16; ++v)
                    st[v] = fmaf(slope2, kb + (float)((v & 3) + 8 * (v >> 2)), fmaf(sc[v], kInvLo, sm[v]));
                if (kt * AKT + AKT - 1 > q0) {
#pragma unroll
                    for (int v = 0; v < 16; ++v) {
                        const int key = kt * AKT + (v & 3) + 8 * (v >> 2) + 4 * kh;
                        if (key > q0 + r) st[v] = -INFINITY;
                    }
                }
            } else {
#pragma unroll
                for (int v = 0; v < 16; ++v) st[v] = fmaf(sc[v], kInvLo, sm[v]);
            }
            if (kt * AKT + AKT > Tk) {
#pragma unroll
                for (int v = 0; v < 16; ++v) {
                    const int key = kt * AKT + (v & 3) + 8 * (v >> 2) + 4 * kh;
                    if (key >= Tk) st[v] = -INFINITY;
                }
            }
            float mloc = st[0];
#pragma unroll
            for (int v = 1; v < 16; ++v) mloc = fmaxf(mloc, st[v]);
            {
                const unsigned int mu = __builtin_bit_cast(unsigned int, mloc);
                const auto sw = __builtin_amdgcn_permlane32_swap(mu, mu, false, false);
                const unsigned int s0 = sw[0], s1 = sw[1];
                mloc = fmaxf(__builtin_bit_cast(float, s0), __builtin_bit_cast(float, s1));
            }
            const float m_new = fmaxf(m_run, mloc);
            if (!__all(m_new <= m_run + defer_thr)) {
                const bool moved = m_new > m_run + defer_thr;
                const float alpha = moved ? __builtin_amdgcn_exp2f(m_run - m_new) : 1.0f;
                l_run *= alpha;
#pragma unroll
                for (int dt = 0; dt < ND; ++dt)
#pragma unroll
                    for (int v = 0; v < 16; ++v) { om[dt][v] *= alpha; oc[dt][v] *= alpha; }
                if (moved) m_run = m_new;
            }
            const float mb = m_run - 10.0f;
            typedef float f32x2 __attribute__((ext_vector_type(2)));
#pragma unroll
            for (int v = 0; v < 16; v += 2) {
                const f32x2 dlt = f32x2{st[v], st[v + 1]} - f32x2{mb, mb};
                st[v] = __builtin_amdgcn_exp2f(dlt[0]);
                st[v + 1] = __builtin_amdgcn_exp2f(dlt[1]);
            }
            l_run += ((st[0] + st[1]) + (st[2] + st[3])) + ((st[4] + st[5]) + (st[6] + st[7])) +
                     (((st[8] + st[9]) + (st[10] + st[11])) + ((st[12] + st[13]) + (st[14] + st[15])));
#pragma unroll
            for (int m = 0; m < 2; ++m) {
                u32x4 ph, pl;
#pragma unroll
                for (int e = 0; e < 4; ++e) {
                    const u32x2 p = split_p(st[8 * m + 2 * e], st[8 * m + 2 * e + 1]);
                    ph[e] = p[0];
                    pl[e] = p[1];
                }
#pragma unroll
                for (int dt = 0; dt < ND; ++dt) {
                    const int ci = v_chunk(dt * 32 + r, m, kh);
                    const u32x4 vfh = Vb[ci], vfl = Vb[VCH + ci];
                    oc[dt] = mfma_h(vfh, pl, oc[dt]);
                    oc[dt] = mfma_h(vfl, ph, oc[dt]);
                    om[dt] = mfma_h(vfh, ph, om[dt]);
                }
            }
        }
        cur = (cur == NSTG - 1) ? 0 : cur + 1;
    }

    if (active) {
        const float l_tot = l_run + __shfl_xor(l_run, 32);
        const float inv = 1.0f / l_tot;
        const bool row_ok = q0 + r < T && q0 + r >= p0;
        const size_t orow = (size_t)(orow0 + max(min(q0 + r, T - 1), p0));
        if (OUT == ATT_OUT_BF16) store_ctx_bf16<ND>(om, oc, inv, kInvLo, row_ok, ctx16 + orow * (size_t)D + (size_t)h * DH, kh);
        else if (OUT == ATT_OUT_SPLIT) store_ctx_split<ND>(om, oc, inv, kInvLo, row_ok, ctx16 + orow * (size_t)(2 * D) + (size_t)((h * DH + d0) / 32) * 64, kh);
        else if (row_ok) store_ctx_f32<ND>(om, oc, inv, kInvLo, ctx + (size_t)(orow0 + q0 + r) * D + (size_t)h * DH + 4 * kh);
    }
}


using Att16v2Kernel = decltype(&attention_f16x3_v2_kernel<4, ATT_OUT_F32, 3, 64, false, 64>);
struct Att16v2Inst { int wpb, out, head_dim; bool rag; Att16v2Kernel fn; size_t lds_bytes; };
template <int WPB, int OUT, int NSTG, int DH, bool RAG = false, int DO = DH>
static constexpr Att16v2Inst att16v2_inst() {
    return {WPB, OUT, DH, RAG, attention_f16x3_v2_kernel<WPB, OUT, NSTG, DH, RAG, DO>, (size_t)NSTG * (8 * DH + 8 * DO) * 16};
}
static const Att16v2Inst kAtt16v2[] = {
    att16v2_inst<1, ATT_OUT_F32, 3, 64>(),   att16v2_inst<2, ATT_OUT_F32, 3, 64>(),   att16v2_inst<4, ATT_OUT_F32, 3, 64>(),
    att16v2_inst<1, ATT_OUT_SPLIT, 3, 64>(), att16v2_inst<2, ATT_OUT_SPLIT, 3, 64>(), att16v2_inst<4, ATT_OUT_SPLIT, 3, 64>(),
    att16v2_inst<1, ATT_OUT_BF16, 3, 64>(),  att16v2_inst<2, ATT_OUT_BF16, 3, 64>(),  att16v2_inst<4, ATT_OUT_BF16, 3, 64>(),
    att16v2_inst<1, ATT_OUT_SPLIT, 3, 64, true>(), att16v2_inst<2, ATT_OUT_SPLIT, 3, 64, true>(), att16v2_inst<4, ATT_OUT_SPLIT, 3, 64, true>(),
    att16v2_inst<4, ATT_OUT_F32, 3, 128>(),  att16v2_inst<4, ATT_OUT_SPLIT, 3, 128>(), att16v2_inst<4, ATT_OUT_BF16, 3, 128>(),
    att16v2_inst<4, ATT_OUT_SPLIT, 2, 256, false, 128>(),
};

static int launch_att16v2(const AttLaunch& a, int wpb, dim3 grid, const RagMap* rag, int dense_nblk) {
    for (const Att16v2Inst& k : kAtt16v2) {
        if (k.wpb != wpb || k.out != a.out || k.head_dim != a.head_dim || k.rag != (rag != nullptr)) continue;
        if (k.lds_bytes > 65536) {
            hipError_t e = hipFuncSetAttribute(reinterpret_cast<const void*>(k.fn), hipFuncAttributeMaxDynamicSharedMemorySize, (int)k.lds_bytes);
            if (e != hipSuccess) { set_error("hipFuncSetAttribute: %s", hipGetErrorString(e)); return PGMI_EHIP; }
        }
        hipLaunchKernelGGL(k.fn, grid, dim3(wpb * 64), k.lds_bytes, a.stream, a.qk16, a.qk_plane, a.vt16, a.vt_plane, a.kv_len, a.slopes,
                           a.T, a.H, (a.T + 31) / 32 * 32, a.ctx, a.ctx16, rag ? *rag : RagMap{}, dense_nblk, a.B);
        PGMI_HIP(hipGetLastError());
        return PGMI_OK;
    }
    set_error("attention_f16x3_v2: no kernel for %d waves, output %d, head_dim %d%s", wpb, (int)a.out, a.head_dim, rag ? ", ragged" : "");
    return PGMI_EINVAL;
}

static int g_att_xcd_local = -1;
int att_set_option(const char* name, long long value) {
    if (!strcmp(name, "att_xcd_local")) { g_att_xcd_local = (int)value; return PGMI_OK; }
    if (!strcmp(name, "att_v3")) { att_v3_set_option((int)value); return PGMI_OK; }
    return PGMI_EINVAL;
}
static dim3 dense_grid(int nblk, int H, int B, int* dense_nblk) {
    if (g_att_xcd_local == 0 || (g_att_xcd_local < 0 && nblk < 2)) { *dense_nblk = 0; return dim3(nblk, H, B); }
    *dense_nblk = nblk;
    const long long pairs = (long long)H * B, groups = (pairs + 7) / 8;
    return dim3((unsigned)(groups * 8 * nblk), 1, 1);
}

int att16_waves_per_block(int T) {
    const int n32 = (T + 31) / 32, nblk = (n32 + 3) / 4;
    const int wpb = (n32 + nblk - 1) / nblk;
    return wpb == 3 ? 4 : wpb;
}

static int check_operand_range(const char* who, const AttLaunch& a) {
    const unsigned long long Tp = (unsigned long long)(a.T + 31) / 32 * 32;
    const unsigned long long seq_bytes = (unsigned long long)a.T * 2ull * (unsigned long long)a.H * (unsigned long long)a.head_dim * 2ull;
    const unsigned long long vt_bytes = (unsigned long long)a.head_dim * Tp * 2ull;
    if ((unsigned long long)a.qk_plane * 2ull + seq_bytes >= (1ull << 32) || (unsigned long long)a.vt_plane * 2ull + vt_bytes >= (1ull << 32)) {
        set_error("%s: operand planes of %zu / %zu halfs exceed the 32-bit offset range of the K / V^T DMA "
                  "(plane stride + one sequence must stay below 4 GiB: create the model with a smaller max_rows)", who, a.qk_plane, a.vt_plane);
        return PGMI_EINVAL;
    }
    return PGMI_OK;
}

int launch_attention_f16x3_v2(const AttLaunch& a) {
    const int B = a.B, T = a.T, H = a.H, head_dim = a.head_dim;
    if (B <= 0 || T <= 0 || H <= 0 || a.out < ATT_OUT_F32 || a.out > ATT_OUT_BF16 || (head_dim != 64 && head_dim != 128 && head_dim != 256)) {
        set_error("attention_f16x3_v2: bad arguments B=%d T=%d H=%d out=%d head_dim=%d", B, T, H, (int)a.out, head_dim);
        return PGMI_EINVAL;
    }
    const int n32 = (T + 31) / 32, Tp = n32 * 32;
    int rc = check_operand_range("attention_f16x3_v2", a);
    if (rc) return rc;
    int dn = 0;
    if (head_dim == 256) {
        if (a.qkv || a.conv || !a.slopes || a.out != ATT_OUT_SPLIT) { set_error("attention_f16x3_v2: head_dim 256 is the causal, fused-QKV, split-plane-output flavour only"); return PGMI_EINVAL; }
        const dim3 grid = dense_grid((n32 + 3) / 4, 2 * H, B, &dn);
        return launch_att16v2(a, 4, grid, nullptr, dn);
    }
    if (head_dim == 128) {
        if (a.qkv || a.conv) { set_error("attention_f16x3_v2: head_dim 128 needs operands from the fused QKV projection"); return PGMI_EINVAL; }
        const dim3 grid = dense_grid((n32 + 3) / 4, H, B, &dn);
        return launch_att16v2(a, 4, grid, nullptr, dn);
    }
    if (a.qkv && a.conv && a.rotary) { set_error("attention_f16x3_v2: depth-wise convolution and rotary together are not a model this library knows"); return PGMI_EINVAL; }
    if (a.qkv && a.conv && H % 4) { set_error("attention_f16x3_v2: the depth-wise convolution has four head groups, H = %d is not a multiple of 4", H); return PGMI_EINVAL; }
    if (a.qkv && a.conv)
        launch_qkv_prep_conv(dim3(n32, H, B), a.stream, a.qkv, a.conv, T, H, Tp, a.qk16, a.qk_plane, a.vt16, a.vt_plane, nullptr);
    else if (a.qkv)
        launch_qkv_prep(dim3(n32, H, B), a.stream, a.qkv, a.cos_t, a.sin_t, a.rotary, T, H, Tp, a.qk16, a.qk_plane, a.vt16, a.vt_plane);
    const int wpb = att16_waves_per_block(T);
    const dim3 grid = dense_grid((n32 + wpb - 1) / wpb, H, B, &dn);
    return att_v3_serves(a) ? launch_att16v3(a, wpb, grid, dn) : launch_att16v2(a, wpb, grid, nullptr, dn);
}

int launch_attention_tr_ragged(const AttLaunch& a, const AttRagged& rg) {
    const int T = a.T, H = a.H;
    if (T <= 0 || H <= 0 || !a.qkv || !a.conv || !a.slopes || a.head_dim != 64 || a.out != ATT_OUT_SPLIT || rg.n_tiles <= 0 || rg.n_blocks <= 0) {
        set_error("attention_tr_ragged: bad arguments T=%d H=%d tiles=%d blocks=%d", T, H, rg.n_tiles, rg.n_blocks);
        return PGMI_EINVAL;
    }
    const int rc = check_operand_range("attention_tr_ragged", a);
    if (rc) return rc;
    const RagMap tiles{rg.seq_off, rg.seq_p, rg.seq_q, rg.seq_root, rg.seq_vt, rg.tile_seq, rg.tile_j};
    launch_qkv_prep_conv(dim3(rg.n_tiles, H, 1), a.stream, a.qkv, a.conv, T, H, (T + 31) / 32 * 32, a.qk16, a.qk_plane, a.vt16, a.vt_plane, &tiles);
    const RagMap rag{rg.seq_off, rg.seq_p, rg.seq_q, rg.seq_root, rg.seq_vt, rg.blk_seq, rg.blk_j};
    return launch_att16v2(a, att16_waves_per_block(T), dim3(rg.n_blocks, H, 1), &rag, 0);
}

}
```

proteingym_amd/csrc/common.h:

```cpp
#pragma once
#include <hip/hip_runtime.h>
#include <stdint.h>
#include <stddef.h>

#include "../../include/pgmi.h"

namespace pgmi {

void set_error(const char* fmt, ...);

#define PGMI_HIP(expr)                                                                   \
    do {                                                                                 \
        hipError_t _e = (expr);                                                          \
        if (_e != hipSuccess) {                                                          \
            pgmi::set_error("%s failed: %s (%s:%d)", #expr, hipGetErrorString(_e),       \
                            __FILE__, __LINE__);                                         \
            return PGMI_EHIP;                                                            \
        }                                                                                \
    } while (0)

typedef float f32x4 __attribute__((ext_vector_type(4)));
typedef float f32x16 __attribute__((ext_vector_type(16)));

constexpr int kWave = 64;
constexpr int kHeadDim = 64;

enum Epilogue { EPI_NONE = 0, EPI_GELU = 1, EPI_SQRELU = 2, EPI_GELU_TANH = 3,
                EPI_SWIGLU = 4 };

constexpr float kLoScale = 2048.0f;
constexpr float kQLog2e = 1.4426950408889634f;

__host__ __device__ __forceinline__ size_t ki_off(size_t row, int k, int K) {
    return row * (size_t)(2 * K) + (size_t)(k >> 5) * 64 + (size_t)(k & 31);
}
#if defined(__HIPCC__)
__device__ __forceinline__ void split_act(float x, _Float16& hi, _Float16& lo) {
    hi = (fabsf(x) < 6.103515625e-05f) ? (_Float16)0.0f : (_Float16)x;
    lo = (_Float16)((x - (float)hi) * kLoScale);
}
#endif

void launch_make_masked_windows(const int32_t* wt, const int32_t* win_start, const int32_t* mask_rel,
                                int B, int T, int32_t* tokens_out, hipStream_t s);
void launch_apply_mask(int32_t* tokens, const int32_t* mask_pos, int B, int T, hipStream_t s);
void launch_seq_stats(const int32_t* tokens, int B, int T, int token_dropout, float* scale,
                      int32_t* pos_idx, int32_t* kv_len, hipStream_t s);
void launch_zero_pad_rows(const int32_t* tokens, int rows, int D, float* x, hipStream_t s);
void launch_embed(const int32_t* tokens, const float* scale, const int32_t* pos_idx,
                  const float* embed_tokens, const float* embed_positions, int token_dropout,
                  int rows, int T, int D, float* x, hipStream_t s);
void launch_layernorm(const float* x, const float* w, const float* b, int rows, int D, float eps,
                      float* y, hipStream_t s);
void launch_gather_rows(const float* x, const int32_t* row_idx, int n, int D, float* y, hipStream_t s);
void launch_strided_index(int first, int stride, int n, int32_t* idx, hipStream_t s);
void launch_vocab_logsoftmax(const float* h, const float* E, const float* bias, int rows, int D,
                             int V, float* out, int32_t* nonfinite, hipStream_t s);
void launch_layernorm16(const float* x, const float* w, const float* b, int rows, int D, float eps,
                        unsigned short* y16, size_t plane, int mode, hipStream_t s);
void launch_scatter_rows(const float* src, const int32_t* dst_row, int n, int V, float* table,
                         hipStream_t s);
void launch_row_index(const int32_t* mask_rel, int B, int T, int32_t* out, hipStream_t s);
void launch_fill_f32(float* p, int64_t n, float v, hipStream_t s);
void launch_seq_loglik(const float* lp, const int32_t* tokens, const int32_t* lens, int B, int T, int V,
                       const float* prior, const int32_t* a0, const int32_t* row0, const int32_t* n,
                       const int32_t* flip, float alpha, float* out, hipStream_t s);
void launch_seq_loglik_ragged(const float* lp, const int32_t* tokens, const int32_t* seq_off, const int32_t* seq_p,
                              const int32_t* seq_root, int B, int T, int V, const float* prior, const int32_t* a0,
                              const int32_t* row0, const int32_t* n, const int32_t* flip, float alpha, float* out, hipStream_t s);
void launch_pg2_seq_loglik(const float* lp, const int32_t* col, const int32_t* n_kept, int B, int T, int V, float* out, hipStream_t s);
void launch_embed_learned(const int32_t* tokens, const float* E, const float* P, int rows, int T, int D, float* x, hipStream_t s);
void launch_wide_logsoftmax(const float* logits, int ldl, int rows, int V, const int32_t* tgt, float* out, int32_t* nonfinite,
                            hipStream_t s);
void launch_seq_sum(const float* terms, const int32_t* off, int B, double* out, hipStream_t s);
void launch_score_mutants(const float* table, int V, const int32_t* sub_pos, const int32_t* sub_wt,
                          const int32_t* sub_mt, const int64_t* mut_off, int64_t n_mut,
                          double* scores, hipStream_t s);
void launch_rotary(float* qkv, const float* cos_t, const float* sin_t, int rows, int T, int H,
                   hipStream_t s, int rot_halves = 1);
void launch_make_pppl_rows(const uint8_t* tok8, const int64_t* seq_off, const int32_t* sid, const int64_t* rp, int J,
                           int64_t g0, int bc, int T, int32_t* tokens, int32_t* row_idx, int32_t* target, hipStream_t s);
void launch_pppl_pick(const float* lp, const int32_t* target, int bc, int V, float* terms, hipStream_t s);
void launch_pppl_sum(const float* terms, const int64_t* rp, const int32_t* sid, int J, int64_t first, double* out, hipStream_t s);

void launch_msa_window_tokens(const int32_t* full, int R, int Tfull, int start, int Tw, int mask_col, int32_t* out, hipStream_t s);
void launch_add_row_embedding(float* x, const float* pe, int R, int C, int D, hipStream_t s);
void launch_permute_rows(const float* src, float* dst, int A, int B, int D, hipStream_t s);
void launch_tied_prep_qk(const float* qkv, int64_t M, int D, unsigned short* q16, unsigned short* k16, hipStream_t s);
void launch_pack_vt16(const float* qkv, int R, int C, int Kp, int H, unsigned short* Vt, hipStream_t s);
int launch_tied_softmax16(const float* part, int H, int S, int C, int Kp, float scale, unsigned short* P, hipStream_t s);
float tied_w_scale();

int launch_gemm_f32(const float* A, const float* W, const float* bias, const float* residual,
                    float* C, int M, int N, int K, int epilogue, hipStream_t s);

void gemm_options_from_env();
int gemm_set_option(const char* name, long long value);
int launch_gemm16(const unsigned short* A, size_t a_plane, const unsigned short* W, size_t w_plane,
                  const float* bias, const float* residual, float* Cf, unsigned short* Ch, size_t c_plane,
                  int M, int N, int K, int epilogue, float out_scale, int planes, bool bf, int variant,
                  hipStream_t s);
int launch_gemm16_qkv(const unsigned short* A, size_t a_plane, const unsigned short* W, size_t w_plane,
                      const float* bias, int M, int D, int K, float out_scale, unsigned short* qk16, size_t qk_plane,
                      unsigned short* vt16, size_t vt_plane, const float* cos_t, const float* sin_t, int rotary,
                      int T, int H, int variant, hipStream_t s, int rot_halves = 1, bool bf = false);
struct XMap;
int launch_gemm16_ex(const unsigned short* A, const unsigned short* W, float* Cf, unsigned short* Ch, int M, int N, int K,
                     float out_scale, XMap xm, int nbatch, hipStream_t s);
void launch_split16(const float* x, int64_t n, float scale, int mode, int K, unsigned short* out, hipStream_t s);

int launch_qkln_prep(const float* qkv, const float* q_w, const float* k_w, float eps, const float* cos_t, const float* sin_t, int B,
                     int T, int H, unsigned short* qk16, size_t qk_plane, unsigned short* vt16, size_t vt_plane, hipStream_t s);

int launch_attention_f32(const float* qkv, const int32_t* kv_len, int B, int T, int H, float* ctx, hipStream_t s,
                         int head_dim = 64);

enum AttOut {
    ATT_OUT_F32 = 0,
    ATT_OUT_SPLIT = 1,
    ATT_OUT_BF16 = 2
};
struct AttLaunch {
    unsigned short* qk16 = nullptr;
    size_t qk_plane = 0;
    unsigned short* vt16 = nullptr;
    size_t vt_plane = 0;
    int B = 1, T = 0, H = 0;
    int head_dim = 64;
    const int32_t* kv_len = nullptr;
    const float* slopes = nullptr;
    AttOut out = ATT_OUT_F32;
    float* ctx = nullptr;
    unsigned short* ctx16 = nullptr;
    hipStream_t stream = nullptr;
    const float* qkv = nullptr;
    const float* conv = nullptr;
    const float* cos_t = nullptr;
    const float* sin_t = nullptr;
    int rotary = 0;
};
int launch_attention_f16x3_v2(const AttLaunch& a);

struct AttRagged {
    const int32_t* seq_off;
    const int32_t* seq_p;
    const int32_t* seq_q;
    const int32_t* seq_root;
    const uint32_t* seq_vt;
    const int32_t* tile_seq;
    const int32_t* tile_j;
    const int32_t* blk_seq;
    const int32_t* blk_j;
    int n_tiles, n_blocks;
};
int att16_waves_per_block(int T);
int att_set_option(const char* name, long long value);
int launch_attention_tr_ragged(const AttLaunch& a, const AttRagged& rg);

}
```

proteingym_amd/csrc/elementwise.hip:

```cpp
#include "common.h"

namespace pgmi {

__device__ __forceinline__ float wave_sum(float v) {
#pragma unroll
    for (int o = 32; o > 0; o >>= 1) v += __shfl_xor(v, o);
    return v;
}
__device__ __forceinline__ float wave_max(float v) {
#pragma unroll
    for (int o = 32; o > 0; o >>= 1) v = fmaxf(v, __shfl_xor(v, o));
    return v;
}
__device__ __forceinline__ double wave_sum_d(double v) {
#pragma unroll
    for (int o = 32; o > 0; o >>= 1) v += __shfl_xor(v, o);
    return v;
}
__device__ __forceinline__ int wave_sum_i(int v) {
#pragma unroll
    for (int o = 32; o > 0; o >>= 1) v += __shfl_xor(v, o);
    return v;
}

__global__ void make_masked_windows_kernel(const int32_t* __restrict__ wt,
                                           const int32_t* __restrict__ win_start,
                                           const int32_t* __restrict__ mask_rel, int B, int T,
                                           int32_t* __restrict__ out) {
    const int64_t i = (int64_t)blockIdx.x * blockDim.x + threadIdx.x;
    if (i >= (int64_t)B * T) return;
    const int b = (int)(i / T), t = (int)(i % T);
    out[i] = (t == mask_rel[b]) ? PGMI_TOK_MASK : wt[win_start[b] + t];
}
void launch_make_masked_windows(const int32_t* wt, const int32_t* win_start, const int32_t* mask_rel,
                                int B, int T, int32_t* out, hipStream_t s) {
    const int64_t n = (int64_t)B * T;
    hipLaunchKernelGGL(make_masked_windows_kernel, dim3((unsigned)((n + 255) / 256)), dim3(256), 0, s,
                       wt, win_start, mask_rel, B, T, out);
}

__global__ void apply_mask_kernel(int32_t* tokens, const int32_t* __restrict__ mask_pos, int B, int T) {
    const int b = blockIdx.x * blockDim.x + threadIdx.x;
    if (b < B) tokens[(int64_t)b * T + mask_pos[b]] = PGMI_TOK_MASK;
}
void launch_apply_mask(int32_t* tokens, const int32_t* mask_pos, int B, int T, hipStream_t s) {
    hipLaunchKernelGGL(apply_mask_kernel, dim3((B + 255) / 256), dim3(256), 0, s, tokens, mask_pos, B, T);
}

__global__ void seq_stats_kernel(const int32_t* __restrict__ tokens, int B, int T, int token_dropout,
                                 float* __restrict__ denom, int32_t* __restrict__ pos_idx,
                                 int32_t* __restrict__ kv_len) {
    const int b = blockIdx.x * (blockDim.x >> 6) + (threadIdx.x >> 6);
    const int lane = threadIdx.x & 63;
    if (b >= B) return;
    const int32_t* tk = tokens + (int64_t)b * T;
    int running = 0, n_mask = 0, last_valid = -1;
    for (int t0 = 0; t0 < T; t0 += 64) {
        const int t = t0 + lane;
        const int tok = (t < T) ? tk[t] : PGMI_TOK_PAD;
        const int valid = (t < T) && (tok != PGMI_TOK_PAD);
        const unsigned long long bal = __ballot(valid);
        const unsigned long long below = bal & ((lane == 63) ? ~0ull : ((1ull << (lane + 1)) - 1ull));
        const int incl = __popcll(below);
        if (t < T) pos_idx[(int64_t)b * T + t] = valid ? (running + incl + PGMI_TOK_PAD) : PGMI_TOK_PAD;
        running += __popcll(bal);
        n_mask += __popcll(__ballot((t < T) && tok == PGMI_TOK_MASK));
        if (bal) last_valid = t0 + 63 - __clzll(bal);
    }
    if (lane == 0) {
        float d = 1.0f;
        if (token_dropout) d = 1.0f - (float)n_mask / (float)running;
        denom[b] = d;
        kv_len[b] = last_valid + 1;
    }
}
void launch_seq_stats(const int32_t* tokens, int B, int T, int token_dropout, float* denom,
                      int32_t* pos_idx, int32_t* kv_len, hipStream_t s) {
    hipLaunchKernelGGL(seq_stats_kernel, dim3((B + 3) / 4), dim3(256), 0, s, tokens, B, T, token_dropout,
                       denom, pos_idx, kv_len);
}

__global__ void embed_kernel(const int32_t* __restrict__ tokens, const float* __restrict__ denom,
                             const int32_t* __restrict__ pos_idx, const float* __restrict__ E,
                             const float* __restrict__ P, int token_dropout, int rows, int T, int D,
                             float* __restrict__ x) {
    const int row = blockIdx.x * (blockDim.x >> 6) + (threadIdx.x >> 6);
    const int lane = threadIdx.x & 63;
    if (row >= rows) return;
    const int tok = tokens[row];
    const int b = row / T;
    const float dn = denom[b];
    const f32x4* e = reinterpret_cast<const f32x4*>(E + (size_t)tok * D);
    const f32x4* p = P ? reinterpret_cast<const f32x4*>(P + (size_t)pos_idx[row] * D) : nullptr;
    f32x4* xo = reinterpret_cast<f32x4*>(x + (size_t)row * D);
    const bool is_pad = tok == PGMI_TOK_PAD;
    const bool zero_emb = token_dropout && tok == PGMI_TOK_MASK;
    for (int i = lane; i < D / 4; i += 64) {
        f32x4 v = zero_emb ? f32x4{0.f, 0.f, 0.f, 0.f} : e[i];
        if (token_dropout) {
#pragma unroll
            for (int c = 0; c < 4; ++c) v[c] = (v[c] * 0.88f) / dn;
        }
        if (p) {
            const f32x4 pv = p[i];
#pragma unroll
            for (int c = 0; c < 4; ++c) v[c] += pv[c];
        }
        if (is_pad) v = f32x4{0.f, 0.f, 0.f, 0.f};
        xo[i] = v;
    }
}
void launch_embed(const int32_t* tokens, const float* denom, const int32_t* pos_idx, const float* E,
                  const float* P, int token_dropout, int rows, int T, int D, float* x, hipStream_t s) {
    hipLaunchKernelGGL(embed_kernel, dim3((rows + 3) / 4), dim3(256), 0, s, tokens, denom, pos_idx, E, P,
                       token_dropout, rows, T, D, x);
}

__global__ void zero_pad_rows_kernel(const int32_t* __restrict__ tokens, int rows, int D, float* __restrict__ x) {
    const int row = blockIdx.x * 4 + (threadIdx.x >> 6);
    const int lane = threadIdx.x & 63;
    if (row >= rows || tokens[row] != PGMI_TOK_PAD) return;
    for (int i = lane; i < D; i += 64) x[(size_t)row * D + i] = 0.f;
}
void launch_zero_pad_rows(const int32_t* tokens, int rows, int D, float* x, hipStream_t s) {
    hipLaunchKernelGGL(zero_pad_rows_kernel, dim3((rows + 3) / 4), dim3(256), 0, s, tokens, rows, D, x);
}

template <int NV, int OUTMODE>
__global__ __launch_bounds__(256) void layernorm_kernel(const float* x,
                                                        const float* __restrict__ w,
                                                        const float* __restrict__ bsh, int rows, int D,
                                                        float eps, float* y, unsigned short* y16,
                                                        size_t plane) {
    const int row = blockIdx.x * 4 + (threadIdx.x >> 6);
    const int lane = threadIdx.x & 63;
    if (row >= rows) return;
    const int nv = D >> 2;
    const f32x4* xr = reinterpret_cast<const f32x4*>(x + (size_t)row * D);
    f32x4 v[NV];
    float s = 0.f;
#pragma unroll
    for (int i = 0; i < NV; ++i) {
        const int c = lane + 64 * i;
        v[i] = (c < nv) ? xr[c] : f32x4{0.f, 0.f, 0.f, 0.f};
        s += (v[i][0] + v[i][1]) + (v[i][2] + v[i][3]);
    }
    const float mean = wave_sum(s) / (float)D;
    float q = 0.f;
#pragma unroll
    for (int i = 0; i < NV; ++i) {
        const int c = lane + 64 * i;
        if (c < nv) {
#pragma unroll
            for (int k = 0; k < 4; ++k) {
                const float d = v[i][k] - mean;
                q += d * d;
            }
        }
    }
    const float rstd = 1.0f / sqrtf(wave_sum(q) / (float)D + eps);
    const f32x4* wr = reinterpret_cast<const f32x4*>(w);
    const f32x4* br = reinterpret_cast<const f32x4*>(bsh);
#pragma unroll
    for (int i = 0; i < NV; ++i) {
        const int c = lane + 64 * i;
        if (c < nv) {
            const f32x4 wv = wr[c], bv = br[c];
            f32x4 o;
#pragma unroll
            for (int k = 0; k < 4; ++k) o[k] = (v[i][k] - mean) * rstd * wv[k] + bv[k];
            if constexpr (OUTMODE == 0) {
                reinterpret_cast<f32x4*>(y + (size_t)row * D)[c] = o;
            } else if constexpr (OUTMODE == 1) {
                typedef _Float16 h4 __attribute__((ext_vector_type(4)));
                h4 hi, lo;
#pragma unroll
                for (int k = 0; k < 4; ++k) {
                    _Float16 a, b2;
                    split_act(o[k], a, b2);
                    hi[k] = a;
                    lo[k] = b2;
                }
                typedef unsigned int u32x2 __attribute__((ext_vector_type(2)));
                typedef unsigned int u32x4 __attribute__((ext_vector_type(4)));
                const u32x2 H = __builtin_bit_cast(u32x2, hi), L = __builtin_bit_cast(u32x2, lo);
                const bool odd = lane & 1;
                const unsigned int s0 = odd ? H[0] : L[0], s1 = odd ? H[1] : L[1];
                const unsigned int r0 = __shfl_xor(s0, 1), r1 = __shfl_xor(s1, 1);
                const u32x4 out = odd ? u32x4{r0, r1, L[0], L[1]} : u32x4{H[0], H[1], r0, r1};
                unsigned short* dst = y16 + ki_off((size_t)row, 4 * (c & ~1), D) + (odd ? 32 : 0);
                *reinterpret_cast<u32x4*>(dst) = out;
            } else {
                typedef unsigned int u32x2 __attribute__((ext_vector_type(2)));
                unsigned short b[4];
#pragma unroll
                for (int k = 0; k < 4; ++k) {
                    const float ok = o[k];
                    unsigned int u = __builtin_bit_cast(unsigned int, ok);
                    u += 0x7fffu + ((u >> 16) & 1u);
                    b[k] = (unsigned short)(u >> 16);
                }
                u32x2 pk;
                pk[0] = b[0] | ((unsigned)b[1] << 16);
                pk[1] = b[2] | ((unsigned)b[3] << 16);
                reinterpret_cast<u32x2*>(y16 + (size_t)row * D)[c] = pk;
            }
        }
    }
}
template <int OUTMODE>
static void launch_ln_mode(const float* x, const float* w, const float* b, int rows, int D, float eps,
                           float* y, unsigned short* y16, size_t plane, hipStream_t s) {
    const dim3 grid((rows + 3) / 4), block(256);
    const int nv = (D / 4 + 63) / 64;
    if (nv <= 1) hipLaunchKernelGGL((layernorm_kernel<1, OUTMODE>), grid, block, 0, s, x, w, b, rows, D, eps, y, y16, plane);
    else if (nv <= 2) hipLaunchKernelGGL((layernorm_kernel<2, OUTMODE>), grid, block, 0, s, x, w, b, rows, D, eps, y, y16, plane);
    else if (nv <= 5) hipLaunchKernelGGL((layernorm_kernel<5, OUTMODE>), grid, block, 0, s, x, w, b, rows, D, eps, y, y16, plane);
    else if (nv <= 10) hipLaunchKernelGGL((layernorm_kernel<10, OUTMODE>), grid, block, 0, s, x, w, b, rows, D, eps, y, y16, plane);
    else hipLaunchKernelGGL((layernorm_kernel<20, OUTMODE>), grid, block, 0, s, x, w, b, rows, D, eps, y, y16, plane);
}
void launch_layernorm(const float* x, const float* w, const float* b, int rows, int D, float eps,
                      float* y, hipStream_t s) {
    launch_ln_mode<0>(x, w, b, rows, D, eps, y, nullptr, 0, s);
}
void launch_layernorm16(const float* x, const float* w, const float* b, int rows, int D, float eps,
                        unsigned short* y16, size_t plane, int mode, hipStream_t s) {
    if (mode == 1) launch_ln_mode<1>(x, w, b, rows, D, eps, nullptr, y16, plane, s);
    else launch_ln_mode<2>(x, w, b, rows, D, eps, nullptr, y16, plane, s);
}

__global__ void rotary_kernel(float* __restrict__ qkv, const float* __restrict__ cos_t,
                              const float* __restrict__ sin_t, int64_t n, int T, int H, int rh) {
    const int64_t i = (int64_t)blockIdx.x * blockDim.x + threadIdx.x;
    if (i >= n) return;
    const int d = (int)(i & 31);
    const int64_t j = i >> 5;
    const int h = (int)(j % H);
    const int64_t k2 = j / H;
    const int which = (int)(k2 & 1);
    const int64_t row = k2 >> 1;
    const int t = (int)(row % T);
    float* p = qkv + row * (size_t)(3 * H * 64) + (size_t)which * H * 64 + h * 64 + d;
    const float x1 = p[0], x2 = p[32];
    const int tr = (t * rh + (h % rh)) * 64;
    const float c1 = cos_t[tr + d], s1 = sin_t[tr + d];
    const float c2 = cos_t[tr + d + 32], s2 = sin_t[tr + d + 32];
    p[0] = x1 * c1 + (-x2) * s1;
    p[32] = x2 * c2 + x1 * s2;
}
void launch_rotary(float* qkv, const float* cos_t, const float* sin_t, int rows, int T, int H, hipStream_t s, int rot_halves) {
    const int64_t n = (int64_t)rows * 2 * H * 32;
    hipLaunchKernelGGL(rotary_kernel, dim3((unsigned)((n + 255) / 256)), dim3(256), 0, s, qkv, cos_t, sin_t, n, T, H, rot_halves);
}

__global__ void gather_rows_kernel(const float* __restrict__ x, const int32_t* __restrict__ idx, int n,
                                   int D, float* __restrict__ y) {
    const int row = blockIdx.x * 4 + (threadIdx.x >> 6);
    const int lane = threadIdx.x & 63;
    if (row >= n) return;
    const f32x4* src = reinterpret_cast<const f32x4*>(x + (size_t)idx[row] * D);
    f32x4* dst = reinterpret_cast<f32x4*>(y + (size_t)row * D);
    for (int i = lane; i < D / 4; i += 64) dst[i] = src[i];
}
void launch_gather_rows(const float* x, const int32_t* idx, int n, int D, float* y, hipStream_t s) {
    hipLaunchKernelGGL(gather_rows_kernel, dim3((n + 3) / 4), dim3(256), 0, s, x, idx, n, D, y);
}

__global__ void strided_index_kernel(int first, int stride, int n, int32_t* __restrict__ idx) {
    const int i = blockIdx.x * blockDim.x + threadIdx.x;
    if (i < n) idx[i] = first + i * stride;
}
void launch_strided_index(int first, int stride, int n, int32_t* idx, hipStream_t s) {
    hipLaunchKernelGGL(strided_index_kernel, dim3((n + 255) / 256), dim3(256), 0, s, first, stride, n, idx);
}

__global__ void scatter_rows_kernel(const float* __restrict__ src, const int32_t* __restrict__ dst_row,
                                    int n, int V, float* __restrict__ table) {
    const int i = blockIdx.x * blockDim.x + threadIdx.x;
    if (i >= n * V) return;
    const int rI = i / V, c = i % V;
    table[(size_t)dst_row[rI] * V + c] = src[i];
}
void launch_scatter_rows(const float* src, const int32_t* dst_row, int n, int V, float* table, hipStream_t s) {
    hipLaunchKernelGGL(scatter_rows_kernel, dim3((n * V + 255) / 256), dim3(256), 0, s, src, dst_row, n, V, table);
}

__global__ void row_index_kernel(const int32_t* __restrict__ mask_rel, int B, int T, int32_t* __restrict__ out) {
    const int b = blockIdx.x * blockDim.x + threadIdx.x;
    if (b < B) out[b] = b * T + mask_rel[b];
}
void launch_row_index(const int32_t* mask_rel, int B, int T, int32_t* out, hipStream_t s) {
    hipLaunchKernelGGL(row_index_kernel, dim3((B + 255) / 256), dim3(256), 0, s, mask_rel, B, T, out);
}

__global__ void fill_f32_kernel(float* p, int64_t n, float v) {
    const int64_t i = (int64_t)blockIdx.x * blockDim.x + threadIdx.x;
    if (i < n) p[i] = v;
}
void launch_fill_f32(float* p, int64_t n, float v, hipStream_t s) {
    hipLaunchKernelGGL(fill_f32_kernel, dim3((unsigned)((n + 255) / 256)), dim3(256), 0, s, p, n, v);
}

__global__ __launch_bounds__(256) void vocab_logsoftmax_kernel(const float* __restrict__ h,
                                                               const float* __restrict__ E,
                                                               const float* __restrict__ bias, int rows,
                                                               int D, int V, float* __restrict__ out,
                                                               int32_t* __restrict__ nonfinite) {
    const int row = blockIdx.x * 4 + (threadIdx.x >> 6);
    const int lane = threadIdx.x & 63;
    if (row >= rows) return;
    const float* hr = h + (size_t)row * D;
    double my_logit = -INFINITY;
    for (int v = 0; v < V; ++v) {
        const float* ev = E + (size_t)v * D;
        double acc = 0.0;
        for (int i = lane; i < D; i += 64) acc = fma((double)hr[i], (double)ev[i], acc);
        acc = wave_sum_d(acc);
        if (lane == v) my_logit = acc + (double)bias[v];
    }
    const float mx = wave_max((float)my_logit);
    const double ex = (lane < V) ? exp(my_logit - (double)mx) : 0.0;
    const double lse = log(wave_sum_d(ex));
    const float res = (float)((my_logit - (double)mx) - lse);
    if (lane < V) {
        out[(size_t)row * V + lane] = res;
        if (nonfinite && !(fabsf(res) <= 3.0e38f)) atomicOr(nonfinite, 1);
    }
}
void launch_vocab_logsoftmax(const float* h, const float* E, const float* bias, int rows, int D, int V,
                             float* out, int32_t* nonfinite, hipStream_t s) {
    hipLaunchKernelGGL(vocab_logsoftmax_kernel, dim3((rows + 3) / 4), dim3(256), 0, s, h, E, bias, rows, D, V, out, nonfinite);
}

__global__ __launch_bounds__(256) void seq_loglik_kernel(const float* __restrict__ lp, const int32_t* __restrict__ tokens,
                                                         const int32_t* __restrict__ lens, int B, int T, int V,
                                                         const float* __restrict__ prior, const int32_t* __restrict__ a0,
                                                         const int32_t* __restrict__ row0, const int32_t* __restrict__ n,
                                                         const int32_t* __restrict__ flip, float alpha,
                                                         float* __restrict__ out) {
    const int b = blockIdx.x * 4 + (threadIdx.x >> 6);
    const int lane = threadIdx.x & 63;
    if (b >= B) return;
    const int len = lens[b];
    float acc = 0.f;
    for (int t = lane; t < len - 1; t += 64) {
        const int tgt = tokens[(size_t)b * T + t + 1];
        float v = lp[((size_t)b * T + t) * V + tgt];
        if (prior && n[b] > 0 && t >= a0[b] && t < a0[b] + n[b]) {
            const int i = t - a0[b];
            const int row = flip[b] ? row0[b] + (n[b] - 1 - i) : row0[b] + i;
            v = (1.0f - alpha) * v + alpha * prior[(size_t)row * V + tgt];
        }
        acc += v;
    }
    acc = wave_sum(acc);
    if (lane == 0) out[b] = acc;
}
__global__ __launch_bounds__(256) void seq_loglik_ragged_kernel(const float* __restrict__ lp, const int32_t* __restrict__ tokens,
                                                                const int32_t* __restrict__ seq_off, const int32_t* __restrict__ seq_p,
                                                                const int32_t* __restrict__ seq_root, int B, int T, int V,
                                                                const float* __restrict__ prior, const int32_t* __restrict__ a0,
                                                                const int32_t* __restrict__ row0, const int32_t* __restrict__ n,
                                                                const int32_t* __restrict__ flip, float alpha,
                                                                float* __restrict__ out) {
    const int b = blockIdx.x * 4 + (threadIdx.x >> 6);
    const int lane = threadIdx.x & 63;
    if (b >= B) return;
    const int a = seq_p[b], own0 = seq_off[b] - a, root0 = seq_off[seq_root[b]];
    float acc = 0.f;
    for (int t = lane; t < T - 1; t += 64) {
        const int tgt = tokens[(t + 1 < a) ? root0 + t + 1 : own0 + t + 1];
        float v = lp[(size_t)((t < a) ? root0 + t : own0 + t) * V + tgt];
        if (prior && n[b] > 0 && t >= a0[b] && t < a0[b] + n[b]) {
            const int i = t - a0[b];
            const int row = flip[b] ? row0[b] + (n[b] - 1 - i) : row0[b] + i;
            v = (1.0f - alpha) * v + alpha * prior[(size_t)row * V + tgt];
        }
        acc += v;
    }
    acc = wave_sum(acc);
    if (lane == 0) out[b] = acc;
}
void launch_seq_loglik_ragged(const float* lp, const int32_t* tokens, const int32_t* seq_off, const int32_t* seq_p,
                              const int32_t* seq_root, int B, int T, int V, const float* prior, const int32_t* a0,
                              const int32_t* row0, const int32_t* n, const int32_t* flip, float alpha, float* out, hipStream_t s) {
    hipLaunchKernelGGL(seq_loglik_ragged_kernel, dim3((B + 3) / 4), dim3(256), 0, s, lp, tokens, seq_off, seq_p, seq_root, B, T, V,
                       prior, a0, row0, n, flip, alpha, out);
}
void launch_seq_loglik(const float* lp, const int32_t* tokens, const int32_t* lens, int B, int T, int V,
                       const float* prior, const int32_t* a0, const int32_t* row0, const int32_t* n,
                       const int32_t* flip, float alpha, float* out, hipStream_t s) {
    hipLaunchKernelGGL(seq_loglik_kernel, dim3((B + 3) / 4), dim3(256), 0, s, lp, tokens, lens, B, T, V, prior, a0, row0, n,
                       flip, alpha, out);
}

__global__ __launch_bounds__(256) void pg2_seq_loglik_kernel(const float* __restrict__ lp, const int32_t* __restrict__ col,
                                                             const int32_t* __restrict__ n_kept, int B, int T, int V,
                                                             float* __restrict__ out) {
    const int b = blockIdx.x * 4 + (threadIdx.x >> 6);
    const int lane = threadIdx.x & 63;
    if (b >= B) return;
    const int n = n_kept[b];
    double acc = 0.0;
    for (int t = lane; t < n; t += 64) acc += (double)lp[((size_t)b * T + t) * V + col[(size_t)b * T + t]];
    acc = wave_sum_d(acc);
    if (lane == 0) out[b] = (float)acc;
}
void launch_pg2_seq_loglik(const float* lp, const int32_t* col, const int32_t* n_kept, int B, int T, int V, float* out, hipStream_t s) {
    hipLaunchKernelGGL(pg2_seq_loglik_kernel, dim3((B + 3) / 4), dim3(256), 0, s, lp, col, n_kept, B, T, V, out);
}

__global__ void score_mutants_kernel(const float* __restrict__ table, int V,
                                     const int32_t* __restrict__ sub_pos,
                                     const int32_t* __restrict__ sub_wt,
                                     const int32_t* __restrict__ sub_mt,
                                     const int64_t* __restrict__ mut_off, int64_t n_mut,
                                     double* __restrict__ scores) {
    const int64_t i = (int64_t)blockIdx.x * blockDim.x + threadIdx.x;
    if (i >= n_mut) return;
    double sc = 0.0;
    for (int64_t k = mut_off[i]; k < mut_off[i + 1]; ++k) {
        const float* rowp = table + (size_t)sub_pos[k] * V;
        const float d = rowp[sub_mt[k]] - rowp[sub_wt[k]];
        sc += (double)d;
    }
    scores[i] = sc;
}
void launch_score_mutants(const float* table, int V, const int32_t* sub_pos, const int32_t* sub_wt,
                          const int32_t* sub_mt, const int64_t* mut_off, int64_t n_mut, double* scores,
                          hipStream_t s) {
    if (n_mut <= 0) return;
    hipLaunchKernelGGL(score_mutants_kernel, dim3((unsigned)((n_mut + 255) / 256)), dim3(256), 0, s, table, V,
                       sub_pos, sub_wt, sub_mt, mut_off, n_mut, scores);
}


__global__ __launch_bounds__(256) void make_pppl_rows_kernel(const uint8_t* __restrict__ tok8, const int64_t* __restrict__ seq_off,
                                                             const int32_t* __restrict__ sid, const int64_t* __restrict__ rp, int J,
                                                             int64_t g0, int bc, int T, int32_t* __restrict__ tokens,
                                                             int32_t* __restrict__ row_idx, int32_t* __restrict__ target) {
    const int b = blockIdx.x * 4 + (threadIdx.x >> 6);
    const int lane = threadIdx.x & 63;
    if (b >= bc) return;
    const int64_t g = g0 + b;
    int lo = 0, hi = J;
    while (hi - lo > 1) {
        const int mid = (lo + hi) >> 1;
        if (rp[mid] <= g) lo = mid; else hi = mid;
    }
    const int n = sid[lo];
    const int i = 1 + (int)(g - rp[lo]);
    const int64_t o = seq_off[n];
    const int len = (int)(seq_off[n + 1] - o);
    int32_t* out = tokens + (int64_t)b * T;
    for (int t = lane; t < T; t += 64) out[t] = (t == i) ? PGMI_TOK_MASK : (t < len ? (int32_t)tok8[o + t] : PGMI_TOK_PAD);
    if (lane == 0) {
        row_idx[b] = b * T + i;
        target[b] = (int32_t)tok8[o + i + 1];
    }
}
void launch_make_pppl_rows(const uint8_t* tok8, const int64_t* seq_off, const int32_t* sid, const int64_t* rp, int J,
                           int64_t g0, int bc, int T, int32_t* tokens, int32_t* row_idx, int32_t* target, hipStream_t s) {
    hipLaunchKernelGGL(make_pppl_rows_kernel, dim3((bc + 3) / 4), dim3(256), 0, s, tok8, seq_off, sid, rp, J, g0, bc, T,
                       tokens, row_idx, target);
}

__global__ void pppl_pick_kernel(const float* __restrict__ lp, const int32_t* __restrict__ target, int bc, int V,
                                 float* __restrict__ terms) {
    const int b = blockIdx.x * blockDim.x + threadIdx.x;
    if (b < bc) terms[b] = lp[(size_t)b * V + target[b]];
}
void launch_pppl_pick(const float* lp, const int32_t* target, int bc, int V, float* terms, hipStream_t s) {
    hipLaunchKernelGGL(pppl_pick_kernel, dim3((bc + 255) / 256), dim3(256), 0, s, lp, target, bc, V, terms);
}

__global__ void pppl_sum_kernel(const float* __restrict__ terms, const int64_t* __restrict__ rp, const int32_t* __restrict__ sid,
                                int J, int64_t first, double* __restrict__ out) {
    const int j = blockIdx.x * blockDim.x + threadIdx.x;
    if (j >= J) return;
    double acc = 0.0;
    for (int64_t g = rp[j]; g < rp[j + 1]; ++g) acc += (double)terms[g];
    out[sid[j] - first] = acc;
}
void launch_pppl_sum(const float* terms, const int64_t* rp, const int32_t* sid, int J, int64_t first, double* out, hipStream_t s) {
    if (J <= 0) return;
    hipLaunchKernelGGL(pppl_sum_kernel, dim3((J + 127) / 128), dim3(128), 0, s, terms, rp, sid, J, first, out);
}


__global__ __launch_bounds__(256) void embed_learned_kernel(const int32_t* __restrict__ tokens, const float* __restrict__ E,
                                                            const float* __restrict__ P, int rows, int T, int D, float* __restrict__ x) {
    const int row = blockIdx.x * 4 + (threadIdx.x >> 6);
    const int lane = threadIdx.x & 63;
    if (row >= rows) return;
    const f32x4* e = reinterpret_cast<const f32x4*>(E + (size_t)tokens[row] * D);
    const f32x4* p = reinterpret_cast<const f32x4*>(P + (size_t)(row % T) * D);
    f32x4* xo = reinterpret_cast<f32x4*>(x + (size_t)row * D);
    for (int i = lane; i < D / 4; i += 64) xo[i] = e[i] + p[i];
}
void launch_embed_learned(const int32_t* tokens, const float* E, const float* P, int rows, int T, int D, float* x, hipStream_t s) {
    hipLaunchKernelGGL(embed_learned_kernel, dim3((rows + 3) / 4), dim3(256), 0, s, tokens, E, P, rows, T, D, x);
}

__device__ __forceinline__ void lse_merge(float& m, double& s, float m2, double s2) {
    const float M = fmaxf(m, m2);
    const double a = s == 0.0 ? 0.0 : s * exp((double)m - (double)M);
    const double b = s2 == 0.0 ? 0.0 : s2 * exp((double)m2 - (double)M);
    m = M;
    s = a + b;
}
__global__ __launch_bounds__(256) void wide_logsoftmax_kernel(const float* __restrict__ logits, int ldl, int V,
                                                              const int32_t* __restrict__ tgt, float* __restrict__ out,
                                                              int32_t* __restrict__ nonfinite) {
    __shared__ float sm[256];
    __shared__ double ss[256];
    const int r = blockIdx.x, tid = threadIdx.x;
    const float* row = logits + (size_t)r * ldl;
    const f32x4* row4 = reinterpret_cast<const f32x4*>(row);
    float m = -INFINITY;
    double s = 0.0;
    for (int i = tid; i < (V + 3) / 4; i += 256) {
        const f32x4 v = row4[i];
        const int c0 = 4 * i;
        float mx = m;
#pragma unroll
        for (int k = 0; k < 4; ++k)
            if (c0 + k < V) mx = fmaxf(mx, v[k]);
        if (mx > m) {
            s = s == 0.0 ? 0.0 : s * (double)__expf(m - mx);
            m = mx;
        }
        float e = 0.0f;
#pragma unroll
        for (int k = 0; k < 4; ++k)
            if (c0 + k < V) e += __expf(v[k] - m);
        s += (double)e;
    }
    sm[tid] = m;
    ss[tid] = s;
    __syncthreads();
    for (int o = 128; o > 0; o >>= 1) {
        if (tid < o) {
            float a = sm[tid];
            double b = ss[tid];
            lse_merge(a, b, sm[tid + o], ss[tid + o]);
            sm[tid] = a;
            ss[tid] = b;
        }
        __syncthreads();
    }
    const double lse = (double)sm[0] + log(ss[0]);
    bool bad = false;
    if (tgt) {
        if (tid == 0) {
            const float res = (float)((double)row[tgt[r]] - lse);
            out[r] = res;
            bad = !(fabsf(res) <= 3.0e38f);
        }
    } else {
        for (int c = tid; c < V; c += 256) {
            const float res = (float)((double)row[c] - lse);
            out[(size_t)r * V + c] = res;
            bad |= !(fabsf(res) <= 3.0e38f);
        }
    }
    if (nonfinite && bad) atomicOr(nonfinite, 1);
}
void launch_wide_logsoftmax(const float* logits, int ldl, int rows, int V, const int32_t* tgt, float* out, int32_t* nonfinite,
                            hipStream_t s) {
    if (rows <= 0) return;
    hipLaunchKernelGGL(wide_logsoftmax_kernel, dim3(rows), dim3(256), 0, s, logits, ldl, V, tgt, out, nonfinite);
}

__global__ void seq_sum_kernel(const float* __restrict__ terms, const int32_t* __restrict__ off, int B, double* __restrict__ out) {
    const int b = blockIdx.x * blockDim.x + threadIdx.x;
    if (b >= B) return;
    double acc = 0.0;
    for (int i = off[b]; i < off[b + 1]; ++i) acc += (double)terms[i];
    out[b] = acc;
}
void launch_seq_sum(const float* terms, const int32_t* off, int B, double* out, hipStream_t s) {
    hipLaunchKernelGGL(seq_sum_kernel, dim3((B + 127) / 128), dim3(128), 0, s, terms, off, B, out);
}

}
```

proteingym_amd/csrc/model.h:

```cpp
#pragma once
#include <math.h>
#include <stdlib.h>
#include <cmath>
#include <algorithm>
#include <stdarg.h>
#include <stdio.h>
#include <string.h>

#include <string>
#include <vector>

#include "common.h"
#include "gemm16x_kernel.h"

namespace pgmi {

struct W16 {
    unsigned short* p = nullptr;
    size_t plane = 0;
    float out_scale = 1.0f;
};

struct Layer {
    float *ln1_w, *ln1_b, *wqkv, *bqkv, *wo, *bo, *ln2_w, *ln2_b, *w1, *b1, *w2, *b2;
    W16 wqkv16, wo16, w116, w216;
    float* conv = nullptr;
    float *c_ln_w = nullptr, *c_ln_b = nullptr, *c_bqkv = nullptr, *c_bo = nullptr;
    W16 c_wqkv16, c_wo16;
    float *q_ln = nullptr, *k_ln = nullptr;
};

struct ProfEvent {
    hipEvent_t start, stop;
    int cls;
};

}

using namespace pgmi;

struct pgmi_assay;
struct pgmi_pppl;

struct pgmi_model {
    pgmi_config cfg;
    int device = 0;
    hipStream_t stream = nullptr;
    std::vector<void*> allocs;
    std::vector<pgmi_assay*> assays;
    std::vector<pgmi_pppl*> pppls;
    float *embed_tokens = nullptr, *embed_positions = nullptr;
    float *lnb_w = nullptr, *lnb_b = nullptr, *lna_w = nullptr, *lna_b = nullptr;
    float *hd_w = nullptr, *hd_b = nullptr, *hln_w = nullptr, *hln_b = nullptr;
    float *head_w = nullptr, *head_b = nullptr;
    std::vector<Layer> layers;
    W16 hd16;
    int fc1_epi = EPI_GELU, fc1_cols = 0;
    bool embed_gather = false;
    float* slopes = nullptr;
    float* tr_prior = nullptr;
    size_t tr_prior_cap = 0;
    int32_t* tr_meta = nullptr;
    size_t tr_meta_cap = 0;
    int pg2_rotary = 0;
    float *pg2_aa_w = nullptr, *pg2_aa_b = nullptr;
    int gpt_Vp = 0, gpt_head_rows = 0;
    bool parallel_residual = false;
    float* gpt_logits = nullptr;
    W16 gpt_head16;
    double* gpt_sum = nullptr;
    float* msa_pe = nullptr;
    float* xt = nullptr;
    int32_t *msa_full = nullptr, *msa_kv_len = nullptr;
    size_t msa_full_cap = 0;
    float *tied_part = nullptr, *tied_p = nullptr, *tied_vt = nullptr;
    size_t tied_part_cap = 0, tied_p_cap = 0, tied_vt_cap = 0;
    int msa_kv_R = 0, msa_kv_C = 0;
    float ln_eps = 1e-5f;
    unsigned short *h16 = nullptr, *g16 = nullptr;
    size_t h16_plane = 0, g16_plane = 0;
    unsigned short *qk16 = nullptr, *vt16 = nullptr;
    size_t qk16_plane = 0, vt16_plane = 0;
    int32_t* nonfinite = nullptr;
    int gemm_variant = 0;
    int keep_rows = 1;
    int last_B = 0, last_T = 0;
    int dh = kHeadDim;
    int rot_halves = 1;
    int Hs = 0;
    int Da = 0;
    float *rot_cos = nullptr, *rot_sin = nullptr;
    int rot_len = 0;
    float* zeros = nullptr;
    int max_rows = 0;
    float *x = nullptr, *h = nullptr, *qkv = nullptr, *g = nullptr, *lp = nullptr, *denom = nullptr;
    int32_t *tokens = nullptr, *pos_idx = nullptr, *kv_len = nullptr, *row_idx = nullptr, *aux_i = nullptr;
    bool prof = false;
    std::vector<ProfEvent> events;
    size_t events_used = 0;
    double prof_ms[PGMI_K_COUNT] = {0};
    int64_t prof_n[PGMI_K_COUNT] = {0};
    double prof_flops[PGMI_K_COUNT] = {0};
    double prof_bytes[PGMI_K_COUNT] = {0};
};

struct pgmi_assay {
    pgmi_model* m = nullptr;
    int n_tok = 0, P = 0, T = 0;
    int64_t n_mut = 0, n_sub = 0;
    std::vector<void*> allocs;
    int32_t *wt = nullptr, *positions = nullptr, *win_start = nullptr, *mask_rel = nullptr;
    int32_t *sub_pos = nullptr, *sub_wt = nullptr, *sub_mt = nullptr;
    int64_t* mut_off = nullptr;
    float* table = nullptr;
    double* scores = nullptr;
};

struct pgmi_pppl {
    pgmi_model* m = nullptr;
    int64_t N = 0;
    std::vector<int64_t> off;
    std::vector<void*> allocs;
    uint8_t* tok8 = nullptr;
    int64_t* off_dev = nullptr;
    int64_t last_rows = 0, last_chunks = 0, last_tokens = 0, last_padded = 0;
};

namespace pgmi {

template <typename T>
int dev_alloc(std::vector<void*>& pool, T** p, size_t n) {
    void* q = nullptr;
    if (n == 0) n = 1;
    hipError_t e = hipMalloc(&q, n * sizeof(T));
    if (e != hipSuccess) {
        set_error("hipMalloc(%zu bytes) failed: %s", n * sizeof(T), hipGetErrorString(e));
        return PGMI_ENOMEM;
    }
    pool.push_back(q);
    *p = static_cast<T*>(q);
    return PGMI_OK;
}

template <typename T>
int dev_upload(std::vector<void*>& pool, T** p, const T* host, size_t n) {
    int rc = dev_alloc(pool, p, n);
    if (rc) return rc;
    if (n) PGMI_HIP(hipMemcpy(*p, host, n * sizeof(T), hipMemcpyHostToDevice));
    return PGMI_OK;
}

struct ProfScope {
    pgmi_model* m;
    ProfEvent* ev = nullptr;
    ProfScope(pgmi_model* m_, int cls, double flops, double bytes) : m(m_) {
        if (!m->prof) return;
        if (m->events_used == m->events.size()) {
            ProfEvent e;
            if (hipEventCreate(&e.start) != hipSuccess || hipEventCreate(&e.stop) != hipSuccess) return;
            m->events.push_back(e);
        }
        ev = &m->events[m->events_used++];
        ev->cls = cls;
        m->prof_n[cls] += 1;
        m->prof_flops[cls] += flops;
        m->prof_bytes[cls] += bytes;
        hipEventRecord(ev->start, m->stream);
    }
    ~ProfScope() {
        if (ev) hipEventRecord(ev->stop, m->stream);
    }
};

template <typename T>
int ensure_cap(pgmi_model* m, T** p, size_t* cap, size_t need) {
    if (need <= *cap) return PGMI_OK;
    T* q = nullptr;
    int rc = dev_alloc(m->allocs, &q, need);
    if (rc) return rc;
    *p = q;
    *cap = need;
    return PGMI_OK;
}

int prof_drain(pgmi_model* m);
int check_cfg(const pgmi_config* c);
int check_tokens(const int32_t* tokens, int B, int T);
int check_vocab(const int32_t* tokens, int B, int T, int V);
int env_int(const char* name, int dflt);
int make_w16(std::vector<void*>& pool, const float* host, size_t n, size_t K, int precision, hipStream_t s, W16* out);
int linear(pgmi_model* m, const float* in32, const unsigned short* in16, size_t in_plane, const float* W32,
           const W16& w16, const float* bias, const float* residual, float* out32, unsigned short* out16,
           size_t out_plane, int M, int N, int K, int epi);
int check_nonfinite(pgmi_model* m);
int reset_pad_keys(pgmi_model* m, int B, int T);
int model_create(const pgmi_config* cfg, const float* w, int64_t n_weights, int device, pgmi_model** out, int arch_arg);
int create_esm(pgmi_model* m, const pgmi_config* cfg, const float* w, int64_t n_weights);
int ensure_rotary(pgmi_model* m, int T);
int upload_rotate_half(pgmi_model* m, int n);
int run_encoder(pgmi_model* m, int B, int T, const int32_t* keep = nullptr, int n_keep = 0, bool* compacted = nullptr);
int run_head(pgmi_model* m, int R, const int32_t* row_idx);
int run_rows(pgmi_model* m, int B, int T, int R, const int32_t* row_idx);
int create_tranception(pgmi_model* m, const pgmi_config* cfg, const float* w, int64_t n_weights);
int create_progen2(pgmi_model* m, const pgmi_config* cfg, const float* w, int64_t n_weights, int rotary_dim);
int create_gpt(pgmi_model* m, const pgmi_config* cfg, const float* w, int64_t n_weights, int pos_kind);
int64_t gpt_weight_count(const pgmi_config* c, int pos_kind);
int decoder_check(pgmi_model* m, int arch, int T);
int run_decoder(pgmi_model* m, int B, int T, const AttRagged* rg = nullptr, int rows = 0, double att_flops = 0);
int narrow_head(pgmi_model* m, int M);
int decoder_token_logprobs(pgmi_model* m, int arch, const int32_t* tokens, int B, int T, float* out);
int64_t esmc_weight_count(const pgmi_config* c);
int create_esmc(pgmi_model* m, const pgmi_config* cfg, const float* w, int64_t n_weights);
int create_msa(pgmi_model* m, const pgmi_config* cfg, const float* w, int64_t n_weights);
int run_msa(pgmi_model* m, int R, int C, int keep_col = -1, bool* compacted = nullptr);

struct BlobCursor {
    pgmi_model* m;
    const float *p, *end;
    int rc = PGMI_OK;
    BlobCursor(pgmi_model* m_, const float* w, int64_t n_weights) : m(m_), p(w), end(w + n_weights) {}
    const float* take(size_t n) { p += n; return p - n; }
    void upload(float** dst, const float* host, size_t n) { if (!rc) rc = dev_upload(m->allocs, dst, host, n); }
    void upload(float** dst, size_t n) { upload(dst, take(n), n); }
    void w16(W16* dst, const float* host, size_t n, size_t K) { if (!rc) rc = make_w16(m->allocs, host, n, K, m->cfg.precision, m->stream, dst); }
    void w16(W16* dst, size_t n, size_t K) { w16(dst, take(n), n, K); }
    void linear(float** w32, W16* w16_, const float* host, size_t n, size_t K) {
        if (m->cfg.precision == PGMI_PREC_FP32) upload(w32, host, n); else w16(w16_, host, n, K);
    }
    void linear(float** w32, W16* w16_, size_t n, size_t K) { linear(w32, w16_, take(n), n, K); }
    int finish() {
        if (!rc && p != end) { set_error("internal: blob walk mismatch"); rc = PGMI_EINVAL; }
        return rc;
    }
};

inline size_t rotate_half_slot(size_t col, size_t dh) {
    const size_t h = col / dh, j = col % dh;
    if (dh > 64) return (2 * h + ((j >> 5) & 1)) * 64 + ((j >> 6) << 5) + (j & 31);
    return h * 64 + (j < dh / 2 ? j : 32 + (j - dh / 2));
}

template <typename Slot>
void pack_qkv_slots(const float* src, size_t D, size_t Da, Slot slot, float qscale, float* wq, float* bq = nullptr) {
    for (size_t k = 0; k < 3; ++k) {
        const float sc = (k == 0) ? qscale : 1.0f;
        for (size_t o = 0; o < D; ++o) {
            float* dst = &wq[(k * Da + slot(o)) * D];
            for (size_t i = 0; i < D; ++i) dst[i] = src[o * D + i] * sc;
        }
        src += D * D;
        if (!bq) continue;
        for (size_t o = 0; o < D; ++o) bq[k * Da + slot(o)] = src[o] * sc;
        src += D;
    }
}

template <typename Slot>
void pack_out_cols(const float* src, size_t D, size_t Da, Slot slot, float* wo) {
    for (size_t o = 0; o < D; ++o)
        for (size_t i = 0; i < D; ++i) wo[o * Da + slot(i)] = src[o * D + i];
}

template <typename Angle>
int upload_rotary(pgmi_model* m, int n, int groups, Angle angle) {
    std::vector<float> c((size_t)n * groups * 64), s((size_t)n * groups * 64);
    for (int t = 0; t < n; ++t)
        for (int g = 0; g < groups; ++g)
            for (int i = 0; i < 32; ++i) {
                const float f = angle(t, g, i);
                const size_t o = ((size_t)t * groups + g) * 64;
                c[o + i] = c[o + 32 + i] = cosf(f);
                s[o + i] = s[o + 32 + i] = sinf(f);
            }
    int rc = dev_upload(m->allocs, &m->rot_cos, c.data(), c.size());
    if (!rc) rc = dev_upload(m->allocs, &m->rot_sin, s.data(), s.size());
    if (!rc) m->rot_len = n;
    return rc;
}

inline int rows_per_chunk(const pgmi_model* m, int T) { return std::max(1, m->max_rows / ((T + 31) / 32 * 32)); }

template <typename Fn>
int for_each_chunk(pgmi_model* m, int B, int T, Fn fn) {
    const int per = rows_per_chunk(m, T);
    for (int b0 = 0; b0 < B; b0 += per) {
        int rc = fn(b0, std::min(per, B - b0));
        if (rc) return rc;
        PGMI_HIP(hipStreamSynchronize(m->stream));
    }
    return PGMI_OK;
}

}
```

Before: 18110.

## Share layer-0 QKV across masked windows and restrict last-layer attention to kept queries

```diff
diff --git a/include/pgmi.h b/include/pgmi.h
--- a/include/pgmi.h
+++ b/include/pgmi.h
@@ -103,6 +103,8 @@
 void pgmi_optimal_window(int position, int seq_len_with_special, int model_window,
                          int* start, int* end);
 
+int pgmi_shared_window(const int32_t* tokens, const int32_t* mask_pos, int B, int T);
+
 #define PGMI_K_EMBED 0
 #define PGMI_K_LAYERNORM 1
 #define PGMI_K_GEMM_QKV 2
@@ -131,6 +133,7 @@
                       float* v, double* ms);
 int pgmi_op_attention(int device, int precision, const float* qkv, const int32_t* kv_len,
                       int B, int T, int H, int rotary, float* ctx);
+int pgmi_op_attention_kept(int device, const float* qkv, const int32_t* keep_t, int B, int T, int H, float* ctx_dense, float* ctx_kept);
 int pgmi_op_causal_attention(int device, int lanes, const float* X, const float* W, const float* bias, int K, const float* qkv,
                              const float* conv, const float* rot_cos, const float* rot_sin, const float* slopes, int B, int T,
                              int heads, float* ctx);
diff --git a/proteingym_amd/_lib.py b/proteingym_amd/_lib.py
--- a/proteingym_amd/_lib.py
+++ b/proteingym_amd/_lib.py
@@ -66,6 +66,7 @@
                                      _i32p, _i32p, _i32p, _i64p, _i64p]),
     ("pgmi_score_mutants", C.c_int, [_f32p, C.c_int, C.c_int, _i32p, _i32p, _i32p, _i64p, C.c_int64, _f64p]),
     ("pgmi_optimal_window", None, [C.c_int, C.c_int, C.c_int, _i32p, _i32p]),
+    ("pgmi_shared_window", C.c_int, [_i32p, _i32p, C.c_int, C.c_int]),
     ("pgmi_profile_enable", C.c_int, [C.c_void_p, C.c_int]),
     ("pgmi_profile_get", C.c_int, [C.c_void_p, C.c_int, _f64p, _i64p, _f64p, _f64p]),
     ("pgmi_profile_reset", C.c_int, [C.c_void_p]),
@@ -88,6 +89,7 @@
     ("pgmi_bench_gemm", C.c_int, [C.c_int] * 9 + [_f64p]),
     ("pgmi_bench_gemm_ab", C.c_int, [C.c_int] * 7 + [_i32p, C.c_int, C.c_int, C.c_int, _f64p]),
     ("pgmi_op_attention", C.c_int, [C.c_int, C.c_int, _f32p, _i32p, C.c_int, C.c_int, C.c_int, C.c_int, _f32p]),
+    ("pgmi_op_attention_kept", C.c_int, [C.c_int, _f32p, _i32p, C.c_int, C.c_int, C.c_int, _f32p, _f32p]),
     ("pgmi_op_qkln_prep", C.c_int, [C.c_int, _f32p, _f32p, _f32p, C.c_int, C.c_int, C.c_int, C.c_int, _f32p, _f32p, _f64p]),
     ("pgmi_op_causal_attention", C.c_int, [C.c_int, C.c_int, _f32p, _f32p, _f32p, C.c_int, _f32p, _f32p, _f32p, _f32p, _f32p,
                                            C.c_int, C.c_int, C.c_int, _f32p]),
diff --git a/proteingym_amd/csrc/api_esm.hip b/proteingym_amd/csrc/api_esm.hip
--- a/proteingym_amd/csrc/api_esm.hip
+++ b/proteingym_amd/csrc/api_esm.hip
@@ -59,7 +59,7 @@
     });
 }
 
-int run_encoder(pgmi_model* m, int B, int T, const int32_t* keep, int n_keep, bool* compacted) {
+int run_encoder(pgmi_model* m, int B, int T, const int32_t* keep, int n_keep, bool* compacted, RowPlan plan) {
     const pgmi_config& c = m->cfg;
     const int M = B * T, D = c.embed_dim, F = c.ffn_dim, N1 = m->fc1_cols, H = c.heads, Da = m->Da;
     hipStream_t s = m->stream;
@@ -83,12 +83,39 @@
     const double ln_bytes = 2.0 * M * D * 4;
     const int prec = c.precision;
     const int mode16 = (prec == PGMI_PREC_F16X3) ? 1 : 2;
+    const bool kept_last = keep && m->keep_rows;
+    const bool share = kept_last && m->share_rows && plan.shared && plan.mask_rel && B > 2 && prec != PGMI_PREC_FP32 && !m->layers[0].q_ln;
     for (int l = 0; l < c.layers; ++l) {
         const Layer& L = m->layers[l];
+        const bool fused_qkv = prec != PGMI_PREC_FP32 && !L.q_ln;
+        if (share && l == 0) {
+            const int Tp = (T + 31) / 32 * 32, M2 = 2 * T;
+            const size_t qs_plane = (size_t)M2 * 2 * Da, vs_plane = (size_t)2 * Da * Tp;
+            const size_t vt_cap = m->shr_vt_cap;
+            auto grown = [](size_t need, size_t cap) { return need <= cap ? need : std::max(need, 2 * cap); };
+            rc = ensure_cap(m, &m->shr_qk, &m->shr_qk_cap, grown(2 * qs_plane, m->shr_qk_cap));
+            if (!rc) rc = ensure_cap(m, &m->shr_vt, &m->shr_vt_cap, grown(2 * vs_plane, m->shr_vt_cap));
+            if (!rc) rc = ensure_cap(m, &m->shr_idx, &m->shr_idx_cap, (size_t)std::max(M2, 5 * B));
+            if (rc) return rc;
+            if (T != m->shr_T || vt_cap != m->shr_vt_cap) {
+                PGMI_HIP(hipMemsetAsync(m->shr_vt, 0, m->shr_vt_cap * sizeof(unsigned short), s));
+                m->shr_T = T;
+            }
+            { ProfScope p(m, PGMI_K_LAYERNORM, 0, (double)M2 * D * 12);
+              launch_shared_rows_index(plan.mask_rel, B, T, m->shr_idx, s);
+              launch_gather_rows(m->x, m->shr_idx, M2, D, m->qkv, s);
+              launch_layernorm16(m->qkv, L.ln1_w, L.ln1_b, M2, D, 1e-5f, m->h16, m->h16_plane, mode16, s); }
+            { ProfScope p(m, PGMI_K_GEMM_QKV, 2.0 * M2 * 3 * D * D, 4.0 * M * 3 * Da);
+              rc = launch_gemm16_qkv(m->h16, m->h16_plane, L.wqkv16.p, L.wqkv16.plane, L.bqkv, M2, Da, D, L.wqkv16.out_scale,
+                                     m->shr_qk, qs_plane, m->shr_vt, vs_plane, m->rot_cos, m->rot_sin,
+                                     c.arch == PGMI_ARCH_ESM2, T, m->Hs, m->gemm_variant, s, m->rot_halves, prec == PGMI_PREC_BF16);
+              if (rc) return rc;
+              launch_broadcast_qk(m->shr_qk, qs_plane, plan.mask_rel, B, T, Da, m->qk16, m->qk16_plane, s);
+              launch_broadcast_vt(m->shr_vt, vs_plane, plan.mask_rel, B, T, Da, m->vt16, m->vt16_plane, s); }
+        } else {
         { ProfScope p(m, PGMI_K_LAYERNORM, 0, ln_bytes);
           if (prec == PGMI_PREC_FP32) launch_layernorm(m->x, L.ln1_w, L.ln1_b, M, D, 1e-5f, m->h, s);
           else launch_layernorm16(m->x, L.ln1_w, L.ln1_b, M, D, 1e-5f, m->h16, m->h16_plane, mode16, s); }
-        const bool fused_qkv = prec != PGMI_PREC_FP32 && !L.q_ln;
         { ProfScope p(m, PGMI_K_GEMM_QKV, 2.0 * M * 3 * D * D, 0);
           if (fused_qkv)
               rc = launch_gemm16_qkv(m->h16, m->h16_plane, L.wqkv16.p, L.wqkv16.plane, L.bqkv, M, Da, D, L.wqkv16.out_scale,
@@ -97,7 +124,11 @@
           else
               rc = linear(m, m->h, m->h16, m->h16_plane, L.wqkv, L.wqkv16, L.bqkv, nullptr, m->qkv, nullptr, 0, M, 3 * Da, D, EPI_NONE);
           if (rc) return rc; }
-        { ProfScope p(m, PGMI_K_ATTENTION, 4.0 * M * T * D, L.q_ln ? (double)M * D * 20 : 0);
+        }
+        const bool kept_tiles = kept_last && l == c.layers - 1 && m->keep_query && plan.mask_rel && n_keep == B && prec == PGMI_PREC_F16X3 &&
+                                m->rot_halves == 1;
+        if (kept_tiles && (rc = ensure_cap(m, &m->shr_idx, &m->shr_idx_cap, (size_t)5 * B))) return rc;
+        { ProfScope p(m, PGMI_K_ATTENTION, 4.0 * (kept_tiles ? B * 32 : M) * T * D, L.q_ln ? (double)M * D * 20 : 0);
           if (L.q_ln && (rc = launch_qkln_prep(m->qkv, L.q_ln, L.k_ln, 1e-5f, m->rot_cos, m->rot_sin, B, T, H, m->qk16, m->qk16_plane,
                                                m->vt16, m->vt16_plane, s)))
               return rc;
@@ -111,12 +142,12 @@
               a.out = prec == PGMI_PREC_F16X3 ? ATT_OUT_SPLIT : ATT_OUT_BF16;
               a.ctx16 = m->h16;
               a.stream = s;
-              rc = launch_attention_f16x3_v2(a);
+              rc = kept_tiles ? launch_attention_kept_tiles(a, keep, m->shr_idx) : launch_attention_f16x3_v2(a);
           } else {
               rc = launch_attention_f32(m->qkv, m->kv_len, B, T, H, m->h, s, m->rot_halves * kHeadDim);
           }
           if (rc) return rc; }
-        if (keep && m->keep_rows && l == c.layers - 1) {
+        if (kept_last && l == c.layers - 1) {
             const int R = n_keep;
             ProfScope p(m, PGMI_K_KEPT_ROWS, 2.0 * R * D * (Da + N1 + F), 0);
             launch_gather_rows(m->x, keep, R, D, m->qkv, s);
@@ -178,9 +209,9 @@
 }
 
 
-int run_rows(pgmi_model* m, int B, int T, int R, const int32_t* row_idx) {
+int run_rows(pgmi_model* m, int B, int T, int R, const int32_t* row_idx, RowPlan plan) {
     bool compacted = false;
-    int rc = run_encoder(m, B, T, row_idx, R, &compacted);
+    int rc = run_encoder(m, B, T, row_idx, R, &compacted, plan);
     if (rc) return rc;
     return run_head(m, R, compacted ? nullptr : row_idx);
 }
@@ -217,14 +248,19 @@
     PGMI_HIP(hipSetDevice(m->device));
     const int V = m->cfg.vocab;
     std::vector<int32_t> ridx;
+    bool no_pad = true;
+    for (size_t i = 0; i < (size_t)B * T && no_pad; ++i) no_pad = tokens[i] != PGMI_TOK_PAD;
     rc = for_each_chunk(m, B, T, [&](int b0, int bc) {
         ridx.resize(bc);
         for (int b = 0; b < bc; ++b) ridx[b] = b * T + mask_pos[b0 + b];
+        RowPlan plan;
+        if (no_pad) plan.mask_rel = m->aux_i;
+        plan.shared = no_pad && m->share_rows && shared_window(tokens + (size_t)b0 * T, mask_pos + b0, bc, T);
         PGMI_HIP(hipMemcpyAsync(m->tokens, tokens + (size_t)b0 * T, (size_t)bc * T * 4, hipMemcpyHostToDevice, m->stream));
         PGMI_HIP(hipMemcpyAsync(m->aux_i, mask_pos + b0, (size_t)bc * 4, hipMemcpyHostToDevice, m->stream));
         PGMI_HIP(hipMemcpyAsync(m->row_idx, ridx.data(), (size_t)bc * 4, hipMemcpyHostToDevice, m->stream));
         launch_apply_mask(m->tokens, m->aux_i, bc, T, m->stream);
-        int rc = run_rows(m, bc, T, bc, m->row_idx);
+        int rc = run_rows(m, bc, T, bc, m->row_idx, plan);
         if (rc) return rc;
         PGMI_HIP(hipMemcpyAsync(out + (size_t)b0 * V, m->lp, (size_t)bc * V * 4, hipMemcpyDeviceToHost, m->stream));
         return PGMI_OK;
@@ -261,6 +297,8 @@
     PGMI_HIP(hipSetDevice(m->device));
     pgmi_assay* a = new pgmi_assay();
     a->m = m; a->n_tok = n_tok; a->P = P; a->T = T; a->n_mut = n_mut; a->n_sub = n_sub;
+    a->win_start_h = ws;
+    a->wt_plain = std::find(wt_tokens, wt_tokens + n_tok, (int32_t)PGMI_TOK_MASK) == wt_tokens + n_tok;
     int rc = dev_upload(a->allocs, &a->wt, wt_tokens, (size_t)n_tok);
     if (!rc) rc = dev_upload(a->allocs, &a->positions, positions, (size_t)P);
     if (!rc) rc = dev_upload(a->allocs, &a->win_start, ws.data(), (size_t)P);
@@ -300,7 +338,11 @@
         const int bc = std::min(per, a->P - p0);
         launch_make_masked_windows(a->wt, a->win_start + p0, a->mask_rel + p0, bc, T, m->tokens, s);
         launch_row_index(a->mask_rel + p0, bc, T, m->row_idx, s);
-        int rc = run_rows(m, bc, T, bc, m->row_idx);
+        RowPlan plan;
+        plan.mask_rel = a->mask_rel + p0;
+        plan.shared = a->wt_plain && std::all_of(a->win_start_h.begin() + p0, a->win_start_h.begin() + p0 + bc,
+                                                 [&](int32_t w) { return w == a->win_start_h[p0]; });
+        int rc = run_rows(m, bc, T, bc, m->row_idx, plan);
         if (rc) return rc;
         launch_scatter_rows(m->lp, a->positions + p0, bc, V, a->table, s);
     }
diff --git a/proteingym_amd/csrc/api_host.hip b/proteingym_amd/csrc/api_host.hip
--- a/proteingym_amd/csrc/api_host.hip
+++ b/proteingym_amd/csrc/api_host.hip
@@ -1,4 +1,25 @@
 #include "model.h"
+
+namespace pgmi {
+
+bool shared_window(const int32_t* tokens, const int32_t* mask_pos, int B, int T) {
+    if (B <= 0 || T <= 0) return false;
+    std::vector<int32_t> win(tokens, tokens + T);
+    const int p0 = mask_pos[0];
+    bool known = false;
+    for (int b = 1; b < B && !known; ++b)
+        if (mask_pos[b] != p0) { win[p0] = tokens[(size_t)b * T + p0]; known = true; }
+    for (int t = 0; t < T; ++t)
+        if ((known || t != p0) && (win[t] == PGMI_TOK_PAD || win[t] == PGMI_TOK_MASK)) return false;
+    for (int b = 0; b < B; ++b) {
+        const int32_t* row = tokens + (size_t)b * T;
+        for (int t = 0; t < T; ++t)
+            if (t != mask_pos[b] && row[t] != win[t]) return false;
+    }
+    return true;
+}
+
+}
 
 
 extern "C" {
@@ -23,6 +44,13 @@
         scores[i] = sc;
     }
     return PGMI_OK;
+}
+
+int pgmi_shared_window(const int32_t* tokens, const int32_t* mask_pos, int B, int T) {
+    if (!tokens || !mask_pos || B <= 0 || T <= 0) { set_error("bad argument"); return PGMI_EINVAL; }
+    for (int b = 0; b < B; ++b)
+        if (mask_pos[b] < 0 || mask_pos[b] >= T) { set_error("mask_pos[%d]=%d out of range", b, mask_pos[b]); return PGMI_EINVAL; }
+    return shared_window(tokens, mask_pos, B, T) ? 1 : 0;
 }
 
 void pgmi_optimal_window(int position, int n, int window, int* start, int* end) {
diff --git a/proteingym_amd/csrc/api_model.hip b/proteingym_amd/csrc/api_model.hip
--- a/proteingym_amd/csrc/api_model.hip
+++ b/proteingym_amd/csrc/api_model.hip
@@ -297,6 +297,8 @@
     if (!rc) rc = alloc_workspace(m);
     if (rc) { pgmi_model_destroy(m); return rc; }
     m->keep_rows = env_int("PGMI_KEEP_ROWS", 1);
+    m->share_rows = env_int("PGMI_SHARE_ROWS", 1);
+    m->keep_query = env_int("PGMI_KEEP_QUERY", 1);
     gemm_options_from_env();
     m->gemm_variant = env_int("PGMI_GEMM_VARIANT", 0);
     *out = m;
diff --git a/proteingym_amd/csrc/api_ops.hip b/proteingym_amd/csrc/api_ops.hip
--- a/proteingym_amd/csrc/api_ops.hip
+++ b/proteingym_amd/csrc/api_ops.hip
@@ -292,6 +292,59 @@
     return PGMI_OK;
 }
 
+int pgmi_op_attention_kept(int device, const float* qkv, const int32_t* keep_t, int B, int T, int H, float* ctx_dense, float* ctx_kept) {
+    if (!qkv || !keep_t || !ctx_dense || !ctx_kept || B <= 0 || T <= 0 || H <= 0) { set_error("bad argument"); return PGMI_EINVAL; }
+    for (int b = 0; b < B; ++b)
+        if (keep_t[b] < 0 || keep_t[b] >= T) { set_error("keep_t[%d]=%d out of range", b, keep_t[b]); return PGMI_EINVAL; }
+    if (pgmi_device_count() <= 0) { set_error("no HIP device visible"); return PGMI_ENODEV; }
+    PGMI_HIP(hipSetDevice(device));
+    const size_t D = (size_t)H * kHeadDim, M = (size_t)B * T, Tp = (size_t)(T + 31) / 32 * 32;
+    std::vector<void*> pool;
+    auto cleanup = [&]() { for (void* p : pool) hipFree(p); };
+    std::vector<int32_t> keep(B);
+    for (int b = 0; b < B; ++b) keep[b] = b * T + keep_t[b];
+    float* dq = nullptr;
+    int32_t *dkeep = nullptr, *dmap = nullptr;
+    unsigned short *qk = nullptr, *vt = nullptr, *c16 = nullptr;
+    int rc = 0;
+    if ((rc = dev_upload(pool, &dq, qkv, M * 3 * D)) || (rc = dev_upload(pool, &dkeep, keep.data(), (size_t)B)) ||
+        (rc = dev_alloc(pool, &dmap, (size_t)5 * B)) || (rc = dev_alloc(pool, &qk, M * 2 * D * 2)) ||
+        (rc = dev_alloc(pool, &vt, (size_t)B * Tp * D * 2)) || (rc = dev_alloc(pool, &c16, M * D * 2))) {
+        cleanup();
+        return rc;
+    }
+    AttLaunch a;
+    a.qk16 = qk, a.qk_plane = M * 2 * D, a.vt16 = vt, a.vt_plane = (size_t)B * Tp * D;
+    a.B = B, a.T = T, a.H = H;
+    a.out = ATT_OUT_SPLIT, a.ctx16 = c16;
+    a.qkv = dq;
+    std::vector<unsigned short> h(M * D * 2);
+    auto kept_rows = [&](float* out) {
+        for (int b = 0; b < B; ++b)
+            for (size_t n = 0; n < D; ++n) {
+                const size_t o = ki_off((size_t)keep[b], (int)n, (int)D);
+                out[(size_t)b * D + n] = rebuild_split(h[o], h[o + 32]);
+            }
+    };
+    hipError_t e = hipMemset(c16, 0, h.size() * 2);
+    if (e == hipSuccess) rc = launch_attention_f16x3_v2(a);
+    if (e == hipSuccess) e = hipDeviceSynchronize();
+    if (!rc && e == hipSuccess) e = hipMemcpy(h.data(), c16, h.size() * 2, hipMemcpyDeviceToHost);
+    if (!rc && e == hipSuccess) {
+        kept_rows(ctx_dense);
+        e = hipMemset(c16, 0, h.size() * 2);
+        a.qkv = nullptr;
+        if (e == hipSuccess) rc = launch_attention_kept_tiles(a, dkeep, dmap);
+        if (e == hipSuccess) e = hipDeviceSynchronize();
+        if (!rc && e == hipSuccess) e = hipMemcpy(h.data(), c16, h.size() * 2, hipMemcpyDeviceToHost);
+        if (!rc && e == hipSuccess) kept_rows(ctx_kept);
+    }
+    cleanup();
+    if (rc) return rc;
+    if (e != hipSuccess) { set_error("kept-tile attention op failed: %s", hipGetErrorString(e)); return PGMI_EHIP; }
+    return PGMI_OK;
+}
+
 int pgmi_op_causal_attention(int device, int lanes, const float* X, const float* W, const float* bias, int K, const float* qkv,
                              const float* conv, const float* rot_cos, const float* rot_sin, const float* slopes, int B, int T,
                              int heads, float* ctx) {
diff --git a/proteingym_amd/csrc/attention_f16.hip b/proteingym_amd/csrc/attention_f16.hip
--- a/proteingym_amd/csrc/attention_f16.hip
+++ b/proteingym_amd/csrc/attention_f16.hip
@@ -380,4 +380,33 @@
     return launch_att16v2(a, att16_waves_per_block(T), dim3(rg.n_blocks, H, 1), &rag, 0);
 }
 
-}
+__global__ void kept_tile_map_kernel(const int32_t* __restrict__ keep, int B, int T, unsigned int vt_seq, int32_t* __restrict__ map) {
+    const int b = blockIdx.x * blockDim.x + threadIdx.x;
+    if (b >= B) return;
+    const int t = min(max(keep[b] - b * T, 0), T - 1);
+    map[b] = b * T;
+    map[B + b] = 0;
+    map[2 * B + b] = b;
+    reinterpret_cast<uint32_t*>(map)[3 * B + b] = (unsigned int)b * vt_seq;
+    map[4 * B + b] = t / AKT;
+}
+
+bool att_kept_tiles_serves(const AttLaunch& a) {
+    return a.head_dim == 64 && a.out == ATT_OUT_SPLIT && !a.slopes && !a.qkv && !a.conv;
+}
+
+int launch_attention_kept_tiles(const AttLaunch& a, const int32_t* keep, int32_t* map) {
+    const int B = a.B, T = a.T, H = a.H;
+    const unsigned long long vt_seq = (unsigned long long)H * kHeadDim * ((T + 31) / 32 * 32);
+    if (B <= 0 || T <= 0 || H <= 0 || !keep || !map || !att_kept_tiles_serves(a) || vt_seq * B >= (1ull << 32)) {
+        set_error("attention_kept_tiles: bad arguments B=%d T=%d H=%d out=%d head_dim=%d", B, T, H, (int)a.out, a.head_dim);
+        return PGMI_EINVAL;
+    }
+    const int rc = check_operand_range("attention_kept_tiles", a);
+    if (rc) return rc;
+    hipLaunchKernelGGL(kept_tile_map_kernel, dim3((B + 255) / 256), dim3(256), 0, a.stream, keep, B, T, (unsigned int)vt_seq, map);
+    const RagMap rag{map, map + B, map, map + 2 * B, reinterpret_cast<const uint32_t*>(map) + 3 * (size_t)B, map + 2 * B, map + 4 * B};
+    return launch_att16v2(a, 1, dim3(B, H, 1), &rag, 0);
+}
+
+}
diff --git a/proteingym_amd/csrc/common.h b/proteingym_amd/csrc/common.h
--- a/proteingym_amd/csrc/common.h
+++ b/proteingym_amd/csrc/common.h
@@ -62,6 +62,11 @@
                          hipStream_t s);
 void launch_row_index(const int32_t* mask_rel, int B, int T, int32_t* out, hipStream_t s);
 void launch_fill_f32(float* p, int64_t n, float v, hipStream_t s);
+void launch_shared_rows_index(const int32_t* mask_rel, int B, int T, int32_t* src, hipStream_t s);
+void launch_broadcast_qk(const unsigned short* qs, size_t qs_plane, const int32_t* mask_rel, int B, int T, int Da,
+                         unsigned short* qk, size_t qk_plane, hipStream_t s);
+void launch_broadcast_vt(const unsigned short* vs, size_t vs_plane, const int32_t* mask_rel, int B, int T, int Da,
+                         unsigned short* vt, size_t vt_plane, hipStream_t s);
 void launch_seq_loglik(const float* lp, const int32_t* tokens, const int32_t* lens, int B, int T, int V,
                        const float* prior, const int32_t* a0, const int32_t* row0, const int32_t* n,
                        const int32_t* flip, float alpha, float* out, hipStream_t s);
@@ -156,5 +161,7 @@
 int att16_waves_per_block(int T);
 int att_set_option(const char* name, long long value);
 int launch_attention_tr_ragged(const AttLaunch& a, const AttRagged& rg);
+bool att_kept_tiles_serves(const AttLaunch& a);
+int launch_attention_kept_tiles(const AttLaunch& a, const int32_t* keep, int32_t* map);
 
 }
diff --git a/proteingym_amd/csrc/elementwise.hip b/proteingym_amd/csrc/elementwise.hip
--- a/proteingym_amd/csrc/elementwise.hip
+++ b/proteingym_amd/csrc/elementwise.hip
@@ -293,6 +293,76 @@
     hipLaunchKernelGGL(row_index_kernel, dim3((B + 255) / 256), dim3(256), 0, s, mask_rel, B, T, out);
 }
 
+__global__ void shared_rows_index_kernel(const int32_t* __restrict__ mask_rel, int B, int T, int32_t* __restrict__ src) {
+    const int t = blockIdx.x * blockDim.x + threadIdx.x;
+    if (t >= T) return;
+    int plain = -1, masked = -1;
+    for (int b = 0; b < B && (plain < 0 || masked < 0); ++b) {
+        if (mask_rel[b] == t) { if (masked < 0) masked = b; }
+        else if (plain < 0) plain = b;
+    }
+    src[t] = max(plain, 0) * T + t;
+    src[T + t] = max(masked, 0) * T + t;
+}
+void launch_shared_rows_index(const int32_t* mask_rel, int B, int T, int32_t* src, hipStream_t s) {
+    hipLaunchKernelGGL(shared_rows_index_kernel, dim3((T + 255) / 256), dim3(256), 0, s, mask_rel, B, T, src);
+}
+
+constexpr int kBcastSeqs = 16;
+typedef unsigned int bc_u32x4 __attribute__((ext_vector_type(4)));
+typedef unsigned short bc_u16x8 __attribute__((ext_vector_type(8)));
+
+__global__ __launch_bounds__(256) void broadcast_qk_kernel(const unsigned short* __restrict__ qs, size_t qs_plane,
+                                                           const int32_t* __restrict__ mask_rel, int B, int n, int row_chunks,
+                                                           unsigned short* __restrict__ qk, size_t qk_plane) {
+    const int i = blockIdx.x * 256 + threadIdx.x;
+    if (i >= n) return;
+    const int t = i / row_chunks;
+    const unsigned short* sp = qs + blockIdx.z * qs_plane + (size_t)i * 8;
+    const bc_u32x4 v0 = *reinterpret_cast<const bc_u32x4*>(sp);
+    const bc_u32x4 v1 = *reinterpret_cast<const bc_u32x4*>(sp + (size_t)n * 8);
+    unsigned short* dp = qk + blockIdx.z * qk_plane + (size_t)i * 8;
+    const int b0 = blockIdx.y * kBcastSeqs, b1 = min(B, b0 + kBcastSeqs);
+    for (int b = b0; b < b1; ++b)
+        *reinterpret_cast<bc_u32x4*>(dp + (size_t)b * n * 8) = (mask_rel[b] == t) ? v1 : v0;
+}
+void launch_broadcast_qk(const unsigned short* qs, size_t qs_plane, const int32_t* mask_rel, int B, int T, int Da,
+                         unsigned short* qk, size_t qk_plane, hipStream_t s) {
+    const int row_chunks = 2 * Da / 8, n = T * row_chunks;
+    hipLaunchKernelGGL(broadcast_qk_kernel, dim3((n + 255) / 256, (B + kBcastSeqs - 1) / kBcastSeqs, 2), dim3(256), 0, s,
+                       qs, qs_plane, mask_rel, B, n, row_chunks, qk, qk_plane);
+}
+
+__global__ __launch_bounds__(256) void broadcast_vt_kernel(const unsigned short* __restrict__ vs, size_t vs_plane,
+                                                           const int32_t* __restrict__ mask_rel, int B, int n, int row_chunks,
+                                                           unsigned short* __restrict__ vt, size_t vt_plane) {
+    const int i = blockIdx.x * 256 + threadIdx.x;
+    if (i >= n) return;
+    const int c = i % row_chunks;
+    const unsigned short* sp = vs + blockIdx.z * vs_plane + (size_t)i * 8;
+    const bc_u16x8 v0 = *reinterpret_cast<const bc_u16x8*>(sp);
+    const bc_u16x8 v1 = *reinterpret_cast<const bc_u16x8*>(sp + (size_t)n * 8);
+    unsigned short* dp = vt + blockIdx.z * vt_plane + (size_t)i * 8;
+    const int b0 = blockIdx.y * kBcastSeqs, b1 = min(B, b0 + kBcastSeqs);
+    for (int b = b0; b < b1; ++b) {
+        const int t = mask_rel[b], tk = t & 31;
+        const int pos = (t & ~31) + ((tk & 0x13) | ((tk & 4) << 1) | ((tk & 8) >> 1));
+        bc_u16x8 v = v0;
+        if ((pos >> 3) == c) {
+#pragma unroll
+            for (int e = 0; e < 8; ++e)
+                if (e == (pos & 7)) v[e] = v1[e];
+        }
+        *reinterpret_cast<bc_u16x8*>(dp + (size_t)b * n * 8) = v;
+    }
+}
+void launch_broadcast_vt(const unsigned short* vs, size_t vs_plane, const int32_t* mask_rel, int B, int T, int Da,
+                         unsigned short* vt, size_t vt_plane, hipStream_t s) {
+    const int row_chunks = (T + 31) / 32 * 32 / 8, n = Da * row_chunks;
+    hipLaunchKernelGGL(broadcast_vt_kernel, dim3((n + 255) / 256, (B + kBcastSeqs - 1) / kBcastSeqs, 2), dim3(256), 0, s,
+                       vs, vs_plane, mask_rel, B, n, row_chunks, vt, vt_plane);
+}
+
 __global__ void fill_f32_kernel(float* p, int64_t n, float v) {
     const int64_t i = (int64_t)blockIdx.x * blockDim.x + threadIdx.x;
     if (i < n) p[i] = v;
diff --git a/proteingym_amd/csrc/model.h b/proteingym_amd/csrc/model.h
--- a/proteingym_amd/csrc/model.h
+++ b/proteingym_amd/csrc/model.h
@@ -85,6 +85,12 @@
     int gemm_variant = 0;
     int keep_rows = 1;
     int last_B = 0, last_T = 0;
+    int share_rows = 1, keep_query = 1;
+    unsigned short *shr_qk = nullptr, *shr_vt = nullptr;
+    size_t shr_qk_cap = 0, shr_vt_cap = 0;
+    int shr_T = 0;
+    int32_t* shr_idx = nullptr;
+    size_t shr_idx_cap = 0;
     int dh = kHeadDim;
     int rot_halves = 1;
     int Hs = 0;
@@ -106,6 +112,8 @@
 
 struct pgmi_assay {
     pgmi_model* m = nullptr;
+    std::vector<int32_t> win_start_h;
+    bool wt_plain = false;
     int n_tok = 0, P = 0, T = 0;
     int64_t n_mut = 0, n_sub = 0;
     std::vector<void*> allocs;
@@ -198,9 +206,15 @@
 int create_esm(pgmi_model* m, const pgmi_config* cfg, const float* w, int64_t n_weights);
 int ensure_rotary(pgmi_model* m, int T);
 int upload_rotate_half(pgmi_model* m, int n);
-int run_encoder(pgmi_model* m, int B, int T, const int32_t* keep = nullptr, int n_keep = 0, bool* compacted = nullptr);
+struct RowPlan {
+    const int32_t* mask_rel = nullptr;
+    bool shared = false;
+};
+int run_encoder(pgmi_model* m, int B, int T, const int32_t* keep = nullptr, int n_keep = 0, bool* compacted = nullptr,
+                RowPlan plan = RowPlan{});
 int run_head(pgmi_model* m, int R, const int32_t* row_idx);
-int run_rows(pgmi_model* m, int B, int T, int R, const int32_t* row_idx);
+int run_rows(pgmi_model* m, int B, int T, int R, const int32_t* row_idx, RowPlan plan = RowPlan{});
+bool shared_window(const int32_t* tokens, const int32_t* mask_pos, int B, int T);
 int create_tranception(pgmi_model* m, const pgmi_config* cfg, const float* w, int64_t n_weights);
 int create_progen2(pgmi_model* m, const pgmi_config* cfg, const float* w, int64_t n_weights, int rotary_dim);
 int create_gpt(pgmi_model* m, const pgmi_config* cfg, const float* w, int64_t n_weights, int pos_kind);
```

After: 18250, median of 6. Within noise of the previous version (+0.8%).
